# kulaginds/lzma

Measured on AMD Instinct MI355X. Metric: decompressed GiB/s (aggregate batch), higher is better.
Workload: dtype u8

## Files before the change

lzma_amd/build.py:

```python
import os
import subprocess
import sys

HERE = os.path.dirname(os.path.abspath(__file__))
CSRC = os.path.join(HERE, "csrc")
SO = os.path.join(HERE, "libxlz.so")
SOURCES = ["xlz_kernel.hip", "xlz_host.hip", "xlz_xz.hip", "xlz_7z.hip", "xlz_check_dev.hip", "xlz_filter_dev.hip", "xlz_sha256_dev.hip"]
HEADERS = ["xlz_format.h", "xlz_check.h", "xlz_check_dev.h", "xlz_check_host.h", "xlz_filter_dev.h", "xlz_sha256_dev.h", "xlz_fastpath.inc", "xlz_fastpath_pb2.inc", "xlz_fastpath_pb2_br.inc", os.path.join("..", "..", "include", "xlz.h")]
ARCH = "gfx950"


KERNEL_FILES = ["xlz_kernel.hip", "xlz_fastpath.inc", "xlz_fastpath_pb2.inc", "xlz_fastpath_pb2_br.inc", "xlz_format.h"]


def source_id(files=None):
    import hashlib
    h = hashlib.sha256()
    for f in sorted(files or (SOURCES + HEADERS)):
        with open(os.path.join(CSRC, f), "rb") as fh:
            h.update(f.encode() + b"\0" + fh.read())
    return h.hexdigest()[:12]


def _stale():
    if not os.path.exists(SO):
        return True
    t = os.path.getmtime(SO)
    deps = [os.path.join(CSRC, f) for f in SOURCES + HEADERS] + [os.path.abspath(__file__)]
    return any(os.path.getmtime(d) > t for d in deps)


def build(force=False, verbose=False, extra_flags=(), out=None):
    if out is None and os.environ.get("XLZ_SO"):
        print("lzma_amd.build: XLZ_SO is set, not building: %s" % os.environ["XLZ_SO"], file=sys.stderr)
        return os.environ["XLZ_SO"]
    if out is None and not force and not _stale():
        return SO
    hipcc = os.environ.get("HIPCC", "/opt/rocm/bin/hipcc")
    cmd = [hipcc, "--offload-arch=" + ARCH, "-O3", "-std=c++17", "-fPIC", "-shared",
           "-fgpu-rdc" if False else "-fno-gpu-rdc", "-Wall", "-Wno-unused-function",
           "-I", os.path.join(HERE, "..", "include"), '-DXLZ_BUILD_ID="%s"' % source_id(), '-DXLZ_KERNEL_ID="%s"' % source_id(KERNEL_FILES)]
    cmd += list(extra_flags)
    cmd += [os.path.join(CSRC, f) for f in SOURCES]
    cmd += ["-o", out or SO]
    if verbose:
        print(" ".join(cmd), file=sys.stderr)
    subprocess.check_call(cmd)
    return out or SO


if __name__ == "__main__":
    build(force="--force" in sys.argv, verbose=True)
    print(SO)
```

lzma_amd/csrc/xlz_host.hip:

```cpp
#include <hip/hip_runtime.h>

#include <algorithm>
#include <atomic>
#include <chrono>
#include <condition_variable>
#include <cstdio>
#include <deque>
#include <functional>
#include <memory>
#include <thread>
#include <cstdlib>
#include <cstring>
#include <mutex>
#include <new>
#include <numeric>
#include <vector>

#include "../../include/xlz.h"
#include "xlz_format.h"
#include "xlz_check.h"
#include "xlz_check_dev.h"
#include "xlz_check_host.h"
#include "xlz_sha256_dev.h"
#include "xlz_filter_dev.h"

using namespace xlz;

namespace {

constexpr uint32_t kLzmaDicMin = 1u << 12;
constexpr uint64_t kUnknownSize = ~(uint64_t)0;
constexpr uint64_t kMaxUnitBytes = 0xFFFF0000ull;
constexpr size_t kArenaAlign = 256;
constexpr size_t kStoredUnitBytes = 256 * 1024;
constexpr size_t kArenaTailPad = 1024;
constexpr size_t kOutTailPad = 64;
constexpr uint32_t kWideGrid = 32;
constexpr int XLZ_ERR_NO_MEMORY_INTERNAL = -1000;
constexpr uint64_t kSlicedCallBytes = 256ull << 20;
constexpr uint64_t kSliceBytes = 128ull << 20;
constexpr uint64_t kMaxSlices = 8;
constexpr uint32_t kCoreOverWave = 16;
static inline uint32_t head_frac_for(uint32_t slices) { return slices >= 2 ? (uint32_t)(65536ull * 3 / (2 * slices)) : 0; }

inline size_t align_up(size_t v, size_t a) { return (v + a - 1) / a * a; }

#define HIP_TRY(expr)                                                                             \
    do {                                                                                          \
        hipError_t e_ = (expr);                                                                   \
        if (e_ != hipSuccess) {                                                                   \
            if (getenv("XLZ_DEBUG"))                                                              \
                fprintf(stderr, "xlz: %s failed: %s\n", #expr, hipGetErrorString(e_));            \
            return XLZ_ERR_DEVICE;                                                                \
        }                                                                                         \
    } while (0)

}

struct xlz_reader;
struct Batcher;
static void batcher_shutdown(Batcher *bt);

struct MemPool {
    struct Blk {
        void *p;
        size_t cap;
        uint64_t gen;
        bool pinned;
    };
    std::mutex mu;
    std::vector<Blk> idle;
    std::vector<Blk> live;
    uint64_t gen = 1;
    void *take(size_t n, bool pinned)
    {
        if (n == 0) n = 1;
        {
            std::lock_guard<std::mutex> lk(mu);
            size_t best = idle.size();
            for (size_t i = 0; i < idle.size(); i++)
                if (idle[i].pinned == pinned && idle[i].cap >= n && idle[i].cap <= n + n / 2 + (1u << 16) &&
                    (best == idle.size() || idle[i].cap < idle[best].cap))
                    best = i;
            if (best != idle.size()) {
                Blk b = idle[best];
                idle.erase(idle.begin() + (long)best);
                b.gen = gen;
                live.push_back(b);
                return b.p;
            }
        }
        void *p = nullptr;
        const hipError_t e = pinned ? hipHostMalloc(&p, n, hipHostMallocDefault) : hipMalloc(&p, n);
        if (e != hipSuccess) {
            (void)hipGetLastError();
            drop_idle();
            if ((pinned ? hipHostMalloc(&p, n, hipHostMallocDefault) : hipMalloc(&p, n)) != hipSuccess) return nullptr;
        }
        std::lock_guard<std::mutex> lk(mu);
        live.push_back(Blk{p, n, gen, pinned});
        return p;
    }
    void give(void *p)
    {
        if (!p) return;
        std::lock_guard<std::mutex> lk(mu);
        for (size_t i = 0; i < live.size(); i++)
            if (live[i].p == p) {
                idle.push_back(live[i]);
                live.erase(live.begin() + (long)i);
                return;
            }
    }
    void end_of_call()
    {
        std::vector<Blk> out;
        {
            std::lock_guard<std::mutex> lk(mu);
            for (size_t i = 0; i < idle.size();)
                if (idle[i].gen + 1 < gen) {
                    out.push_back(idle[i]);
                    idle.erase(idle.begin() + (long)i);
                } else {
                    i++;
                }
            gen++;
        }
        for (const Blk &b : out) (void)(b.pinned ? hipHostFree(b.p) : hipFree(b.p));
    }
    void drop_idle()
    {
        std::vector<Blk> out;
        {
            std::lock_guard<std::mutex> lk(mu);
            out.swap(idle);
        }
        for (const Blk &b : out) (void)(b.pinned ? hipHostFree(b.p) : hipFree(b.p));
    }
    uint64_t idle_bytes()
    {
        std::lock_guard<std::mutex> lk(mu);
        uint64_t t = 0;
        for (const Blk &b : idle) t += b.cap;
        return t;
    }
};

constexpr int kEventSlots = 64;

struct HostPipe {
    static constexpr int kRing = 8;
    static constexpr size_t kRingBytes = 32u << 20;
    std::mutex mu_in;
    std::condition_variable cv_in;
    bool in_busy = false;
    std::mutex mu_out;
    uint8_t *pin_in = nullptr;
    size_t pin_in_cap = 0;
    uint8_t *ring[kRing] = {};
    hipEvent_t ring_ev[kRing] = {};
    hipStream_t copy_stream = nullptr;
    hipStream_t up_stream = nullptr;
};

struct PinLease {
    HostPipe *hp = nullptr;
    void take(HostPipe &h)
    {
        std::unique_lock<std::mutex> lk(h.mu_in);
        h.cv_in.wait(lk, [&] { return !h.in_busy; });
        h.in_busy = true;
        hp = &h;
    }
    void release()
    {
        if (!hp) return;
        {
            std::lock_guard<std::mutex> lk(hp->mu_in);
            hp->in_busy = false;
        }
        hp->cv_in.notify_one();
        hp = nullptr;
    }
    PinLease() = default;
    PinLease(const PinLease &) = delete;
    PinLease &operator=(const PinLease &) = delete;
    ~PinLease() { release(); }
};

struct xlz_ctx {
    Batcher *batcher = nullptr;
    int device = 0;
    int num_cus = 0;
    hipStream_t stream = nullptr;
    uint32_t *queue = nullptr;
    hipStream_t stream2 = nullptr;
    uint32_t *queue2 = nullptr;
    uint32_t *prio_tab = nullptr;
    hipEvent_t ev[kEventSlots] = {};
    std::mutex mu;
    HostPipe pipe;
    MemPool pool;
    xlz_call_stats last_call = {};
    bool have_last_call = false;
    uint64_t sliced_call_bytes = kSlicedCallBytes, slice_bytes = kSliceBytes;
    uint32_t max_slices = kMaxSlices;
    void *chk_tab[2] = {}, *chk_consts[2] = {};
    hipStream_t check_stream = nullptr;
    int check_mode = 0;
    xlz_check_stats last_check = {};
    xlz_sha256_stats last_sha = {};
    int filter_mode = 0;
    xlz_filter_stats last_filter = {};
};

struct StreamPlan {
    int32_t host_status = 1;
    uint64_t host_in_consumed = 0;
    uint32_t header_len = 0;
    uint32_t first_unit = 0, n_units = 0;
    uint64_t out_off = 0;
    uint64_t out_cap = 0;
    uint64_t in_off = 0;
    uint32_t in_len = 0;
    uint32_t dict_size = 0;
    bool lzma2 = false;
    bool slice = false;
    bool oversize = false;
};

struct xlz_batch {
    xlz_ctx *ctx = nullptr;
    size_t n = 0;
    std::vector<StreamPlan> plans;
    std::vector<Unit> units;
    std::vector<uint32_t> order;
    uint8_t *d_in = nullptr;
    uint8_t *d_out = nullptr;
    Unit *d_units = nullptr;
    uint32_t *d_order = nullptr;
    UnitResult *d_results = nullptr;
    size_t in_bytes = 0, out_bytes = 0;
    uint32_t max_pb = 0;
    bool compact = false;
    uint32_t max_lc_lp = 0;
    uint32_t max_lc_lp_big = 0;
    uint32_t n_normal = 0;
    uint16_t *d_scratch = nullptr;
    uint32_t scratch_stride = 0;
    uint16_t *d_mlit = nullptr;
    uint32_t mlit_stride = 0;
    hipEvent_t ev0 = nullptr, ev1 = nullptr;
    hipStream_t run_stream = nullptr;
    uint32_t *queue = nullptr;
    bool pooled = false;
    bool quiet = false;
    uint32_t call_units = 0;
    bool ran = false;
    uint64_t algo_in = 0;
    std::vector<xlz_result> final_results;
    std::vector<UnitResult> unit_results;
    bool collected = false;
    uint64_t sum_in = 0, sum_out = 0;
    std::vector<size_t> rewritten;
    std::vector<char> wants_wide;
    std::vector<uint32_t> slice_fracs;
    std::vector<hipEvent_t> slice_ev;
    uint8_t *d_states = nullptr;
    size_t state_stride = 0;
    std::vector<std::vector<SlicePiece>> slice_pieces;
    std::vector<uint64_t> slice_pack_bytes;
    SlicePiece *d_pieces = nullptr;
    uint8_t *d_pack = nullptr;
    UnitResult *d_res_snap = nullptr;
    UnitResult *pin_res = nullptr;
    uint32_t head_frac = 0;
    uint8_t *d_stage = nullptr;
    SlicePiece *d_up_pieces = nullptr;
    hipEvent_t ev_heads = nullptr, ev_tails = nullptr;
    std::function<int()> upload_tails;
    PinLease in_lease;
    uint8_t *d_chk = nullptr, *pin_chk = nullptr;
    size_t d_chk_cap = 0, pin_chk_cap = 0;
    hipEvent_t chk_ev0 = nullptr, chk_ev1 = nullptr;
    uint8_t *d_sha = nullptr, *pin_sha = nullptr;
    size_t sha_cap = 0;
    uint8_t *d_flt = nullptr, *pin_flt = nullptr;
    size_t d_flt_cap = 0, pin_flt_cap = 0;
    hipEvent_t flt_ev0 = nullptr, flt_ev1 = nullptr;
};

extern "C" const char *xlz_version(void) { return "xlz 0.1 (gfx950)"; }

#ifndef XLZ_BUILD_ID
#define XLZ_BUILD_ID "unknown"
#endif
extern "C" const char *xlz_build_id(void) { return XLZ_BUILD_ID; }
#ifndef XLZ_KERNEL_ID
#define XLZ_KERNEL_ID "unknown"
#endif
extern "C" const char *xlz_kernel_id(void) { return XLZ_KERNEL_ID; }

extern "C" const char *xlz_strerror(int st)
{
    switch (st) {
    case XLZ_OK: return "ok";
    case XLZ_OK_INPUT_EOF: return "ok (input ended; reference reports io.EOF)";
    case XLZ_ERR_RESULT: return "result error";
    case XLZ_ERR_PROPS: return "incorrect LZMA properties";
    case XLZ_ERR_HEADER_EOF: return "EOF";
    case XLZ_ERR_RC_INIT: return "rangeDec.Init: result error";
    case XLZ_ERR_UNEXPECTED_EOF: return "unexpected EOF";
    case XLZ_ERR_OUT_CAP: return "output capacity too small";
    case XLZ_ERR_BAD_ARG: return "bad argument";
    case XLZ_ERR_DEVICE: return "HIP device error";
    case XLZ_ERR_UNSUPPORTED: return "stream not supported by the GPU path";
    case XLZ_ERR_CLOSED: return "lzma: already closed";
    case XLZ_ERR_NEED_ONE_READER: return "lzma: need exactly one reader";
    case XLZ_ERR_INSUFFICIENT_PROPS: return "lzma2: not enough properties";
    case XLZ_EOF: return "EOF";
    }
    return "unknown status";
}

extern "C" int xlz_device_count(void)
{
    int n = 0;
    if (hipGetDeviceCount(&n) != hipSuccess) return 0;
    return n;
}

extern "C" int xlz_decode_prop(uint8_t d, uint8_t *lc, uint8_t *pb, uint8_t *lp)
{
    if (d >= 9 * 5 * 5) return XLZ_ERR_PROPS;
    if (lc) *lc = d % 9;
    d /= 9;
    if (pb) *pb = d / 5;
    if (lp) *lp = d % 5;
    return XLZ_OK;
}

extern "C" uint32_t xlz_decode_dict_size(const uint8_t p[4])
{
    uint32_t d = 0;
    for (int i = 0; i < 4; i++) d |= (uint32_t)p[i] << (8 * i);
    return d < kLzmaDicMin ? kLzmaDicMin : d;
}

extern "C" uint32_t xlz_decode_dict_size2(uint8_t b)
{
    const unsigned sh = (unsigned)(b / 2 + 11);
    return sh >= 32 ? 0u : (uint32_t)(2u | (b & 1u)) << sh;
}

extern "C" uint64_t xlz_decode_unpack_size(const uint8_t h[8])
{
    uint64_t u = 0;
    for (int i = 0; i < 8; i++) u |= (uint64_t)h[i] << (8 * i);
    return u;
}

namespace {

unsigned host_threads(size_t bytes)
{
    unsigned cap = 8;
    const unsigned hw = std::thread::hardware_concurrency();
    if (hw && hw < cap) cap = hw;
    const unsigned want = (unsigned)(bytes / (32u << 20)) + 1;
    return want < cap ? want : cap;
}

template <class F> void run_threads(unsigned n, F &&f)
{
    if (n <= 1) {
        f(0u);
        return;
    }
    std::vector<std::thread> th;
    th.reserve(n - 1);
    for (unsigned t = 1; t < n; t++) th.emplace_back([&f, t] { f(t); });
    f(0u);
    for (auto &x : th) x.join();
}

}

extern "C" int xlz_ctx_create(int device, xlz_ctx **out)
{
    if (!out) return XLZ_ERR_BAD_ARG;
    *out = nullptr;
    int n = 0;
    if (hipGetDeviceCount(&n) != hipSuccess || device < 0 || device >= n) return XLZ_ERR_DEVICE;
    HIP_TRY(hipSetDevice(device));
    hipDeviceProp_t prop;
    HIP_TRY(hipGetDeviceProperties(&prop, device));
    xlz_ctx *c = new (std::nothrow) xlz_ctx;
    if (!c) return XLZ_ERR_BAD_ARG;
    c->device = device;
    c->num_cus = prop.multiProcessorCount;
    if (hipStreamCreateWithFlags(&c->stream, hipStreamNonBlocking) != hipSuccess ||
        hipStreamCreateWithFlags(&c->stream2, hipStreamNonBlocking) != hipSuccess ||
        hipMalloc(&c->queue, 512) != hipSuccess || hipMalloc(&c->queue2, 512) != hipSuccess ||
        hipMalloc(&c->prio_tab, kPrioTabWords * sizeof(uint32_t)) != hipSuccess ||
        hipMemset(c->prio_tab, 0, kPrioTabWords * sizeof(uint32_t)) != hipSuccess) {
        if (c->queue) (void)hipFree(c->queue);
        if (c->queue2) (void)hipFree(c->queue2);
        if (c->stream) (void)hipStreamDestroy(c->stream);
        if (c->stream2) (void)hipStreamDestroy(c->stream2);
        if (c->prio_tab) (void)hipFree(c->prio_tab);
        delete c;
        return XLZ_ERR_DEVICE;
    }
    *out = c;
    return XLZ_OK;
}

extern "C" void xlz_ctx_destroy(xlz_ctx *c)
{
    if (!c) return;
    if (c->batcher) batcher_shutdown(c->batcher);
    (void)hipSetDevice(c->device);
    c->pool.drop_idle();
    if (c->queue) (void)hipFree(c->queue);
    if (c->queue2) (void)hipFree(c->queue2);
    if (c->prio_tab) (void)hipFree(c->prio_tab);
    for (int k = 0; k < 2; k++) {
        if (c->chk_tab[k]) (void)hipFree(c->chk_tab[k]);
        if (c->chk_consts[k]) (void)hipFree(c->chk_consts[k]);
    }
    if (c->check_stream) (void)hipStreamDestroy(c->check_stream);
    if (c->pipe.pin_in) (void)hipHostFree(c->pipe.pin_in);
    for (int i = 0; i < HostPipe::kRing; i++) {
        if (c->pipe.ring[i]) (void)hipHostFree(c->pipe.ring[i]);
        if (c->pipe.ring_ev[i]) (void)hipEventDestroy(c->pipe.ring_ev[i]);
    }
    if (c->pipe.copy_stream) (void)hipStreamDestroy(c->pipe.copy_stream);
    if (c->pipe.up_stream) (void)hipStreamDestroy(c->pipe.up_stream);
    for (hipEvent_t e : c->ev)
        if (e) (void)hipEventDestroy(e);
    if (c->stream) (void)hipStreamDestroy(c->stream);
    if (c->stream2) (void)hipStreamDestroy(c->stream2);
    delete c;
}

extern "C" int xlz_ctx_device(const xlz_ctx *c) { return c ? c->device : -1; }

extern "C" int xlz_ctx_event_record(xlz_ctx *c, int slot)
{
    if (!c || slot < 0 || slot >= kEventSlots) return XLZ_ERR_BAD_ARG;
    std::lock_guard<std::mutex> lock(c->mu);
    HIP_TRY(hipSetDevice(c->device));
    if (!c->ev[slot]) HIP_TRY(hipEventCreate(&c->ev[slot]));
    HIP_TRY(hipEventRecord(c->ev[slot], c->stream));
    return XLZ_OK;
}

extern "C" int xlz_ctx_event_elapsed_ms(xlz_ctx *c, int a, int b, float *ms)
{
    if (!c || !ms || a < 0 || a >= kEventSlots || b < 0 || b >= kEventSlots || !c->ev[a] || !c->ev[b]) return XLZ_ERR_BAD_ARG;
    HIP_TRY(hipSetDevice(c->device));
    HIP_TRY(hipEventSynchronize(c->ev[b]));
    HIP_TRY(hipEventElapsedTime(ms, c->ev[a], c->ev[b]));
    return XLZ_OK;
}

namespace {

void plan_lzma_alone(const xlz_stream_desc &s, StreamPlan &pl, Unit &u, bool &has_unit)
{
    has_unit = false;
    if (s.in_len == 0) {
        pl.host_status = XLZ_ERR_HEADER_EOF;
        pl.host_in_consumed = 0;
        return;
    }
    uint8_t lc, pb, lp;
    if (xlz_decode_prop(s.in[0], &lc, &pb, &lp) != XLZ_OK) {
        pl.host_status = XLZ_ERR_PROPS;
        pl.host_in_consumed = 1;
        return;
    }
    if (s.in_len < 13) {
        pl.host_status = XLZ_ERR_HEADER_EOF;
        pl.host_in_consumed = s.in_len;
        return;
    }
    u.dict_size = xlz_decode_dict_size(s.in + 1);
    u.unpack_size = xlz_decode_unpack_size(s.in + 5);
    u.lc = lc;
    u.lp = lp;
    u.pb = pb;
    u.kind = UNIT_LZMA1;
    pl.header_len = 13;
    has_unit = true;
}

void plan_lzma_raw(const xlz_stream_desc &s, StreamPlan &pl, Unit &u, bool &has_unit)
{
    has_unit = false;
    uint8_t lc, pb, lp;
    if (xlz_decode_prop(s.props, &lc, &pb, &lp) != XLZ_OK) {
        pl.host_status = XLZ_ERR_PROPS;
        pl.host_in_consumed = 0;
        return;
    }
    u.dict_size = s.dict_size < kLzmaDicMin ? kLzmaDicMin : s.dict_size;
    u.unpack_size = s.unpack_size;
    u.lc = lc;
    u.lp = lp;
    u.pb = pb;
    u.kind = UNIT_LZMA1;
    pl.header_len = 0;
    has_unit = true;
}

struct Lz2Unit {
    uint64_t in_start, in_len;
    uint64_t out_start, expect_out;
    bool have_reader;
};

uint64_t stored_unit_bytes()
{
#ifdef XLZ_DEV_KNOBS
    static const uint64_t v = [] {
        const char *e = getenv("XLZ_STORED_UNIT_KIB");
        if (!e) return (uint64_t)kStoredUnitBytes;
        unsigned long long k = strtoull(e, nullptr, 10);
        return (uint64_t)(k > (1u << 20) ? (1u << 20) : k) << 10;
    }();
    return v;
#else
    return kStoredUnitBytes;
#endif
}

void scan_lzma2(const uint8_t *in, size_t len, std::vector<Lz2Unit> &units, uint32_t &max_lc_lp, uint32_t *max_pb = nullptr)
{
    size_t pos = 0, unit_start = 0;
    uint64_t out = 0, unit_out = 0;
    struct Cand {
        size_t pos;
        uint64_t out;
        bool seen_lzma;
    };
    std::vector<Cand> cands;
    struct Mark {
        size_t pos;
        uint64_t out;
    };
    std::vector<Mark> marks;
    const uint64_t stored_unit = stored_unit_bytes();
    bool seen_lzma = false, unit_seen_lzma = false;
    auto cut = [&](size_t at, uint64_t at_out, bool lzma_before) {
        units.push_back({(uint64_t)unit_start, (uint64_t)(at - unit_start), unit_out, at_out - unit_out, unit_seen_lzma});
        unit_start = at;
        unit_out = at_out;
        unit_seen_lzma = lzma_before;
    };
    auto cut_at_candidates = [&](bool last_pure) {
        size_t mi = 0;
        for (size_t i = 0; i < cands.size(); i++) {
            const Cand &c = cands[i];
            if (c.pos != unit_start) cut(c.pos, c.out, c.seen_lzma);
            const size_t region_end = i + 1 < cands.size() ? cands[i + 1].pos : (size_t)-1;
            const bool pure = i + 1 < cands.size() || last_pure;
            for (; mi < marks.size() && marks[mi].pos < region_end; mi++)
                if (pure && stored_unit && marks[mi].pos > c.pos && marks[mi].out - unit_out >= stored_unit)
                    cut(marks[mi].pos, marks[mi].out, c.seen_lzma);
        }
        cands.clear();
        marks.clear();
    };
    bool ended = false;
    while (pos < len) {
        const uint8_t c = in[pos];
        if (c == 0 || (c >= 3 && c < 0x80)) {
            pos++;
            ended = true;
            break;
        }
        const bool stored = c < 3;
        const unsigned sub = c >> 5;
        const size_t hl = stored ? 3 : (sub >= 6 ? 6 : 5);
        if (pos + hl > len) break;
        uint32_t unc = ((uint32_t)in[pos + 1] << 8) | in[pos + 2];
        if (stored) {
            unc += 1;
            if (c == 1 || pos == 0)
                cands.push_back({pos, out, seen_lzma});
            else if (!cands.empty())
                marks.push_back({pos, out});
            const size_t body = std::min<size_t>(unc, len - pos - hl);
            pos += hl + body;
            out += body;
            continue;
        }
        unc = (unc | ((uint32_t)(c & 0x1F) << 16)) + 1;
        const size_t comp = (((size_t)in[pos + 3] << 8) | in[pos + 4]) + 1;
        if (sub >= 6) {
            const uint8_t props = in[pos + 5];
            if (props >= 225) break;
            max_lc_lp = std::max<uint32_t>(max_lc_lp, (props % 9) + (props / 9) % 5);
            if (max_pb) *max_pb = std::max<uint32_t>(*max_pb, props / 45u);
            if (sub == 7 && pos != 0 && pos != unit_start) {
                cut_at_candidates(true);
                if (pos != unit_start) cut(pos, out, seen_lzma);
            } else {
                cut_at_candidates(sub == 7);
            }
        }
        seen_lzma = true;
        cands.clear();
        marks.clear();
        pos += hl + std::min(comp, len - pos - hl);
        out += unc;
    }
    if (ended || pos >= len) cut_at_candidates(true);
    units.push_back({(uint64_t)unit_start, (uint64_t)(len - unit_start), unit_out, out - unit_out, unit_seen_lzma});
}

}

extern "C" int xlz_lzma2_units(const uint8_t *in, size_t len, xlz_lzma2_unit *units, size_t max_units, size_t *n_units)
{
    if ((!in && len) || !n_units || (!units && max_units)) return XLZ_ERR_BAD_ARG;
    std::vector<Lz2Unit> lu;
    uint32_t mx = 0;
    scan_lzma2(in, len, lu, mx);
    *n_units = lu.size();
    for (size_t k = 0; k < lu.size() && k < max_units; k++) {
        units[k].in_off = lu[k].in_start;
        units[k].in_len = lu[k].in_len;
        units[k].out_off = lu[k].out_start;
        units[k].out_len = lu[k].expect_out;
        units[k].have_reader = lu[k].have_reader ? 1u : 0u;
        units[k].reserved = 0;
    }
    return max_units && lu.size() > max_units ? XLZ_ERR_OUT_CAP : XLZ_OK;
}

extern "C" int xlz_batch_advice(const xlz_ctx *ctx, const xlz_stream_desc *streams, size_t n, uint32_t host_threads,
                                xlz_advice *out)
{
    if (!out || (!streams && n)) return XLZ_ERR_BAD_ARG;
    memset(out, 0, sizeof *out);
    uint64_t max_unit = 0, max_stream = 0;
    for (size_t i = 0; i < n; i++) {
        const xlz_stream_desc &s = streams[i];
        if (!s.in && s.in_len) return XLZ_ERR_BAD_ARG;
        out->in_bytes += s.in_len;
        size_t units = 0;
        if (s.format == XLZ_FMT_LZMA2_RAW) {
            std::vector<Lz2Unit> lu;
            uint32_t mx = 0;
            scan_lzma2(s.in, s.in_len, lu, mx);
            units = lu.size();
            for (const Lz2Unit &u : lu) max_unit = std::max<uint64_t>(max_unit, u.in_len);
        } else if (s.format == XLZ_FMT_LZMA_ALONE) {
            units = s.in_len > 13 ? 1 : 0;
            if (units) max_unit = std::max<uint64_t>(max_unit, s.in_len);
        } else {
            units = s.in_len ? 1 : 0;
            if (units) max_unit = std::max<uint64_t>(max_unit, s.in_len);
        }
        out->units += units;
        if (units) max_stream = std::max<uint64_t>(max_stream, s.in_len);
    }
    const uint32_t cus = ctx ? (uint32_t)ctx->num_cus : 256u;
    out->wave_slots = cus * 16u;
    if (!host_threads) host_threads = std::max(1u, std::thread::hardware_concurrency());
    out->break_even_units = kCoreOverWave * host_threads;
    out->fill = out->wave_slots ? std::min(1.0, (double)out->units / out->wave_slots) : 0.0;
    out->cpu_cost = (double)std::max<uint64_t>(max_stream, (out->in_bytes + host_threads - 1) / host_threads) / kCoreOverWave;
    out->gpu_cost = (double)std::max<uint64_t>(max_unit, out->wave_slots ? (out->in_bytes + out->wave_slots - 1) / out->wave_slots : 0);
    out->prefer_cpu = (out->units == 0 || out->cpu_cost < out->gpu_cost) ? 1 : 0;
    return XLZ_OK;
}

namespace {

template <class T> bool batch_alloc(xlz_batch *b, T **p, size_t bytes, bool pinned = false)
{
    if (b->pooled) {
        *p = static_cast<T *>(b->ctx->pool.take(bytes, pinned));
        return *p != nullptr;
    }
    return (pinned ? hipHostMalloc(reinterpret_cast<void **>(p), bytes, hipHostMallocDefault) : hipMalloc(reinterpret_cast<void **>(p), bytes)) ==
           hipSuccess;
}
void batch_release(xlz_batch *b, void *p, bool pinned = false)
{
    if (!p) return;
    if (b->pooled)
        b->ctx->pool.give(p);
    else
        (void)(pinned ? hipHostFree(p) : hipFree(p));
}

int batch_free(xlz_batch *b)
{
    if (!b) return XLZ_OK;
    if (b->ctx) (void)hipSetDevice(b->ctx->device);
    if (b->pooled && !b->quiet) (void)hipDeviceSynchronize();
    batch_release(b, b->d_in);
    batch_release(b, b->d_out);
    batch_release(b, b->d_units);
    batch_release(b, b->d_order);
    batch_release(b, b->d_results);
    batch_release(b, b->d_scratch);
    batch_release(b, b->d_mlit);
    if (b->ev0) (void)hipEventDestroy(b->ev0);
    if (b->ev1) (void)hipEventDestroy(b->ev1);
    for (hipEvent_t e : b->slice_ev)
        if (e) (void)hipEventDestroy(e);
    batch_release(b, b->d_stage);
    batch_release(b, b->d_up_pieces);
    if (b->ev_heads) (void)hipEventDestroy(b->ev_heads);
    if (b->ev_tails) (void)hipEventDestroy(b->ev_tails);
    b->in_lease.release();
    batch_release(b, b->d_states);
    batch_release(b, b->d_pieces);
    batch_release(b, b->d_pack);
    batch_release(b, b->d_res_snap);
    batch_release(b, b->pin_res, true);
    batch_release(b, b->d_chk);
    batch_release(b, b->pin_chk, true);
    if (b->chk_ev0) (void)hipEventDestroy(b->chk_ev0);
    if (b->chk_ev1) (void)hipEventDestroy(b->chk_ev1);
    batch_release(b, b->d_sha);
    batch_release(b, b->pin_sha, true);
    batch_release(b, b->d_flt);
    batch_release(b, b->pin_flt, true);
    if (b->flt_ev0) (void)hipEventDestroy(b->flt_ev0);
    if (b->flt_ev1) (void)hipEventDestroy(b->flt_ev1);
    delete b;
    return XLZ_OK;
}

int take_pin_in(PinLease &lease, HostPipe &hp, size_t bytes)
{
    lease.take(hp);
    if (hp.pin_in_cap < bytes) {
        if (hp.pin_in) (void)hipHostFree(hp.pin_in);
        hp.pin_in = nullptr;
        hp.pin_in_cap = 0;
        const size_t want = bytes + bytes / 4 + (1u << 20);
        if (hipHostMalloc(&hp.pin_in, want, hipHostMallocDefault) != hipSuccess) return XLZ_ERR_DEVICE;
        hp.pin_in_cap = want;
    }
    if (!hp.up_stream && hipStreamCreateWithFlags(&hp.up_stream, hipStreamNonBlocking) != hipSuccess) return XLZ_ERR_DEVICE;
    return XLZ_OK;
}

struct PackPiece {
    uint64_t off;
    const uint8_t *src;
    size_t len;
};

template <class At> int pack_upload(xlz_ctx *ctx, uint8_t *stage, uint8_t *dst, size_t n, uint64_t total, bool zero_gaps, At &&at)
{
    const hipStream_t up = ctx->pipe.up_stream;
    std::atomic<bool> copy_failed{false};
    auto copy = [&](uint64_t from, uint64_t to) {
        if (to > from && hipMemcpyAsync(dst + from, stage + from, (size_t)(to - from), hipMemcpyHostToDevice, up) != hipSuccess)
            copy_failed = true;
    };
    if (!n && zero_gaps) {
        memset(stage, 0, (size_t)total);
        copy(0, total);
    }
    auto end_of = [&](size_t k) {
        if (!zero_gaps) return at(k).off + at(k).len;
        return k + 1 < n ? at(k + 1).off : total;
    };
    const unsigned nth = host_threads((size_t)total);
    run_threads(nth, [&](unsigned t) {
        (void)hipSetDevice(ctx->device);
        const size_t k0 = n * t / nth, k1 = n * (t + 1) / nth;
        if (k0 >= k1) return;
        uint64_t sent = at(k0).off;
        if (zero_gaps && k0 == 0) {
            memset(stage, 0, (size_t)sent);
            sent = 0;
        }
        for (size_t k = k0; k < k1; k++) {
            const PackPiece pc = at(k);
            memcpy(stage + pc.off, pc.src, pc.len);
            const uint64_t end = end_of(k);
            if (end > pc.off + pc.len) memset(stage + pc.off + pc.len, 0, (size_t)(end - pc.off - pc.len));
            if (end - sent >= (16u << 20)) {
                copy(sent, end);
                sent = end;
            }
        }
        copy(sent, end_of(k1 - 1));
    });
    return copy_failed ? XLZ_ERR_DEVICE : XLZ_OK;
}

LaunchParams batch_params(const xlz_batch *b, bool big)
{
    LaunchParams p;
    memset(&p, 0, sizeof p);
    p.in_arena = b->d_in;
    p.out_arena = b->d_out;
    p.units = b->d_units;
    p.order = b->d_order;
    p.results = b->d_results;
    p.queue = b->queue ? b->queue : b->ctx->queue;
    p.prio_tab = b->ctx->prio_tab;
    p.call_units = b->call_units;
    if (big) {
        p.n_units = (uint32_t)b->units.size() - b->n_normal;
        p.order_base = b->n_normal;
        p.max_lc_lp = b->max_lc_lp_big;
        p.scratch = b->d_scratch;
        p.scratch_stride = b->scratch_stride;
    } else {
        p.n_units = b->n_normal;
        p.max_lc_lp = b->max_lc_lp;
        p.mlit = b->d_mlit;
        p.mlit_stride = b->mlit_stride;
        p.compact = b->compact ? 1u : 0u;
    }
    return p;
}

}

struct BatchOpts {
    uint32_t want_slices = 1;
    uint32_t head_frac = 0;
    uint32_t call_units = 0;
    bool pooled = false;
    hipStream_t run_stream = nullptr;
    uint32_t *queue = nullptr;
};
static int batch_create_ex(xlz_ctx *ctx, const xlz_stream_desc *streams, size_t n, xlz_batch **out, const BatchOpts &opts);

extern "C" int xlz_batch_create(xlz_ctx *ctx, const xlz_stream_desc *streams, size_t n, xlz_batch **out)
{
    return batch_create_ex(ctx, streams, n, out, BatchOpts{});
}

static int batch_create_ex(xlz_ctx *ctx, const xlz_stream_desc *streams, size_t n, xlz_batch **out, const BatchOpts &opts)
{
    const uint32_t want_slices = opts.want_slices, head_frac = opts.head_frac;
    if (!ctx || !out || (!streams && n)) return XLZ_ERR_BAD_ARG;
    *out = nullptr;
    for (size_t i = 0; i < n; i++) {
        if (!streams[i].in && streams[i].in_len) return XLZ_ERR_BAD_ARG;
        if ((streams[i].flags & ~XLZ_STREAM_F_LZMA2_SLICE) ||
            ((streams[i].flags & XLZ_STREAM_F_LZMA2_SLICE) && streams[i].format != XLZ_FMT_LZMA2_RAW))
            return XLZ_ERR_BAD_ARG;
        for (size_t k = 0; k < sizeof streams[i].reserved; k++)
            if (streams[i].reserved[k]) return XLZ_ERR_BAD_ARG;
    }
    HIP_TRY(hipSetDevice(ctx->device));

    xlz_batch *b = new (std::nothrow) xlz_batch;
    if (!b) return XLZ_ERR_BAD_ARG;
    b->ctx = ctx;
    b->n = n;
    b->plans.resize(n);
    b->call_units = opts.call_units;
    b->pooled = opts.pooled;
    b->run_stream = opts.run_stream;
    b->queue = opts.queue;

    auto unit_src_off_p = std::make_shared<std::vector<size_t>>();
    std::vector<size_t> &unit_src_off = *unit_src_off_p;
    size_t in_cursor = 0, out_cursor = 0;
    for (size_t i = 0; i < n; i++) {
        const xlz_stream_desc &s = streams[i];
        StreamPlan &pl = b->plans[i];
        Unit u;
        memset(&u, 0, sizeof u);
        bool has_unit = false;
        switch (s.format) {
        case XLZ_FMT_LZMA_ALONE: plan_lzma_alone(s, pl, u, has_unit); break;
        case XLZ_FMT_LZMA_RAW: plan_lzma_raw(s, pl, u, has_unit); break;
        case XLZ_FMT_LZMA2_RAW:
            u.kind = UNIT_LZMA2;
            u.dict_size = s.dict_size < kLzmaDicMin ? 8u * 1024 * 1024 : s.dict_size;
            u.unpack_size = kUnknownSize;
            pl.header_len = 0;
            pl.slice = (s.flags & XLZ_STREAM_F_LZMA2_SLICE) != 0;
            has_unit = true;
            break;
        default: pl.host_status = XLZ_ERR_BAD_ARG; break;
        }
        if (!has_unit) continue;

        if (u.kind == UNIT_LZMA2) {
            if (s.in_len > kMaxUnitBytes || s.out_cap > kMaxUnitBytes) {
                pl.host_status = XLZ_ERR_UNSUPPORTED;
                pl.oversize = !pl.slice;
                continue;
            }
            std::vector<Lz2Unit> lu;
            uint32_t mx = 0, mpb = 0;
            scan_lzma2(s.in, s.in_len, lu, mx, &mpb);
            const bool big = mx > kMaxLcLpLds;
            if (big)
                b->max_lc_lp_big = std::max(b->max_lc_lp_big, mx);
            else
                b->max_lc_lp = std::max(b->max_lc_lp, mx), b->max_pb = std::max(b->max_pb, mpb);
            pl.lzma2 = true;
            pl.in_off = in_cursor;
            pl.in_len = (uint32_t)s.in_len;
            pl.dict_size = u.dict_size;
            pl.first_unit = (uint32_t)b->units.size();
            pl.n_units = (uint32_t)lu.size();
            pl.out_off = out_cursor;
            pl.out_cap = s.out_cap;
            for (size_t k = 0; k < lu.size(); k++) {
                Unit v = u;
                const bool last = k + 1 == lu.size();
                v.in_off = in_cursor + lu[k].in_start;
                v.in_len = (uint32_t)lu[k].in_len;
                v.out_off = out_cursor + std::min<uint64_t>(lu[k].out_start, s.out_cap);
                const uint64_t room = s.out_cap > lu[k].out_start ? s.out_cap - lu[k].out_start : 0;
                v.out_cap = (uint32_t)(last ? room : std::min<uint64_t>(room, lu[k].expect_out));
                v.expect_out = (uint32_t)lu[k].expect_out;
                v.stream = (uint32_t)i;
                v.flags = (last ? UNIT_F_LAST : 0u) | (lu[k].have_reader ? UNIT_F_HAVE_READER : 0u) |
                          ((k || pl.slice) ? UNIT_F_NOT_FIRST : 0u) | (big ? UNIT_F_BIG_MODEL : 0u);
                v.lc = (uint8_t)mx;
                b->units.push_back(v);
                unit_src_off.push_back(lu[k].in_start);
            }
            b->algo_in += s.in_len;
            in_cursor += align_up(s.in_len + 16, kArenaAlign);
            out_cursor += align_up((size_t)s.out_cap + kOutTailPad, kArenaAlign);
            continue;
        }

        const size_t payload = s.in_len - pl.header_len;
        uint64_t cap = s.out_cap;
        if (u.unpack_size != kUnknownSize && u.unpack_size < cap)
            cap = u.unpack_size;
        const bool size_too_big = u.unpack_size != kUnknownSize && u.unpack_size > kMaxUnitBytes;
        if (payload > kMaxUnitBytes || cap > kMaxUnitBytes || size_too_big) {
            pl.host_status = XLZ_ERR_UNSUPPORTED;
            pl.oversize = true;
            continue;
        }
        const bool big = (uint32_t)u.lc + u.lp > kMaxLcLpLds;
        u.in_off = in_cursor;
        u.in_len = (uint32_t)payload;
        u.out_off = out_cursor;
        u.out_cap = (uint32_t)cap;
        u.stream = (uint32_t)i;
        u.flags = UNIT_F_LAST | (big ? UNIT_F_BIG_MODEL : 0u);
        pl.first_unit = (uint32_t)b->units.size();
        pl.n_units = 1;
        pl.out_off = out_cursor;
        pl.out_cap = cap;
        b->units.push_back(u);
        unit_src_off.push_back(pl.header_len);
        if (big)
            b->max_lc_lp_big = std::max(b->max_lc_lp_big, (uint32_t)u.lc + u.lp);
        else
            b->max_lc_lp = std::max(b->max_lc_lp, (uint32_t)u.lc + u.lp), b->max_pb = std::max<uint32_t>(b->max_pb, u.pb);
        b->algo_in += payload;
        in_cursor += align_up(payload + 16, kArenaAlign);
        out_cursor += align_up((size_t)cap + kOutTailPad, kArenaAlign);
    }
    b->in_bytes = in_cursor + kArenaTailPad;
    b->out_bytes = out_cursor + kArenaTailPad;

    b->order.resize(b->units.size());
    std::iota(b->order.begin(), b->order.end(), 0u);
    std::stable_sort(b->order.begin(), b->order.end(), [&](uint32_t a, uint32_t c) {
        const bool ba = b->units[a].flags & UNIT_F_BIG_MODEL, bc = b->units[c].flags & UNIT_F_BIG_MODEL;
        if (ba != bc) return !ba;
        return b->units[a].in_len > b->units[c].in_len;
    });
    for (uint32_t idx : b->order)
        if (!(b->units[idx].flags & UNIT_F_BIG_MODEL)) b->n_normal++;

    b->compact = b->max_pb <= kCompactPosBits && !getenv("XLZ_NO_COMPACT");

    const size_t nu = b->units.size();
    auto fail = [&](int st) {
        batch_free(b);
        return st;
    };
    if (!batch_alloc(b, &b->d_in, b->in_bytes)) return fail(XLZ_ERR_DEVICE);
    if (!batch_alloc(b, &b->d_out, b->out_bytes)) return fail(XLZ_ERR_DEVICE);
    if (nu) {
        if (!batch_alloc(b, &b->d_units, nu * sizeof(Unit))) return fail(XLZ_ERR_DEVICE);
        if (!batch_alloc(b, &b->d_order, nu * sizeof(uint32_t))) return fail(XLZ_ERR_DEVICE);
        if (!batch_alloc(b, &b->d_results, nu * sizeof(UnitResult))) return fail(XLZ_ERR_DEVICE);
    }
    if (hipEventCreate(&b->ev0) != hipSuccess || hipEventCreate(&b->ev1) != hipSuccess)
        return fail(XLZ_ERR_DEVICE);
    if (b->n_normal < nu) {
        b->scratch_stride = num_probs(b->max_lc_lp_big) + num_matched_probs(b->max_lc_lp_big);
        if (!batch_alloc(b, &b->d_scratch, (size_t)big_model_grid(ctx->num_cus) * b->scratch_stride * sizeof(uint16_t)))
            return fail(XLZ_ERR_DEVICE);
    }
    if (b->n_normal) {
        b->mlit_stride = num_matched_probs(b->max_lc_lp);
        const size_t slots = std::min<size_t>(b->n_normal, decode_grid(b->max_lc_lp, ctx->num_cus, ~0u, b->compact));
        if (!batch_alloc(b, &b->d_mlit, slots * b->mlit_stride * sizeof(uint16_t))) return fail(XLZ_ERR_DEVICE);
    }
    if (want_slices > 1 && b->n_normal && b->n_normal <= decode_grid(b->max_lc_lp, ctx->num_cus, b->call_units ? b->call_units : b->n_normal, b->compact)) {
        const uint32_t K0 = std::min<uint32_t>(want_slices, 63);
        for (uint32_t k = 1; k < K0; k++) b->slice_fracs.push_back((uint32_t)((uint64_t)kSliceOne * k / K0));
        if (K0 >= 4) b->slice_fracs.push_back((uint32_t)((uint64_t)kSliceOne * (2 * K0 - 1) / (2 * K0)));
        b->slice_fracs.push_back(kSliceOne);
        const uint32_t K = (uint32_t)b->slice_fracs.size();
        b->state_stride = align_up(state_bytes(b->max_lc_lp), kArenaAlign);
        if (!batch_alloc(b, &b->d_states, nu * b->state_stride)) return fail(XLZ_ERR_DEVICE);
        for (size_t k = 0; k < nu; k++)
            if (!(b->units[k].flags & UNIT_F_BIG_MODEL)) b->units[k].state = (uint64_t)(uintptr_t)(b->d_states + k * b->state_stride);
        b->slice_pieces.resize(K);
        b->slice_pack_bytes.assign(K, 0);
        size_t total_pieces = 0;
        uint64_t max_pack = 0;
        for (uint32_t k = 0; k < K; k++) {
            uint64_t cursor = 0;
            for (size_t ui = 0; ui < nu; ui++) {
                const Unit &u = b->units[ui];
                if (u.flags & UNIT_F_BIG_MODEL) continue;
                const uint32_t lo = k == 0 ? 0u : std::min(slice_bound(u.out_cap, b->slice_fracs[k - 1]), u.out_cap);
                const uint32_t hi = std::min(slice_bound(u.out_cap, b->slice_fracs[k]), u.out_cap);
                if (hi <= lo) continue;
                const uint64_t po = align_up(cursor, kArenaAlign) + ((u.out_off + lo) & (kArenaAlign - 1));
                b->slice_pieces[k].push_back(SlicePiece{u.out_off + lo, po, hi - lo, (uint32_t)ui});
                cursor = po + (hi - lo);
            }
            b->slice_pack_bytes[k] = cursor;
            max_pack = std::max(max_pack, cursor);
            total_pieces += b->slice_pieces[k].size();
        }
        b->slice_ev.assign(K, nullptr);
        for (uint32_t k = 0; k < K; k++)
            if (hipEventCreateWithFlags(&b->slice_ev[k], hipEventDisableTiming) != hipSuccess) return fail(XLZ_ERR_DEVICE);
        if (!batch_alloc(b, &b->d_pieces, std::max<size_t>(total_pieces, 1) * sizeof(SlicePiece)) ||
            !batch_alloc(b, &b->d_pack, (size_t)max_pack + kArenaAlign) ||
            !batch_alloc(b, &b->d_res_snap, (size_t)K * nu * sizeof(UnitResult)) ||
            !batch_alloc(b, &b->pin_res, (size_t)K * nu * sizeof(UnitResult), true))
            return fail(XLZ_ERR_DEVICE);
        size_t at = 0;
        for (uint32_t k = 0; k < K; k++) {
            const std::vector<SlicePiece> &pv = b->slice_pieces[k];
            if (!pv.empty() &&
                hipMemcpy(b->d_pieces + at, pv.data(), pv.size() * sizeof(SlicePiece), hipMemcpyHostToDevice) != hipSuccess)
                return fail(XLZ_ERR_DEVICE);
            at += pv.size();
        }
    }
    if (!b->slice_fracs.empty() && head_frac && head_frac < kSliceOne) {
        HostPipe &hp = ctx->pipe;
        b->head_frac = head_frac;
        auto heads = std::make_shared<std::vector<SlicePiece>>(), tails = std::make_shared<std::vector<SlicePiece>>();
        uint64_t A = 0, B = 0;
        auto place = [](std::vector<SlicePiece> &v, uint64_t &cur, uint64_t src, uint32_t len, uint32_t ui) {
            if (!len) return;
            const uint64_t po = align_up(cur, kArenaAlign) + (src & (kArenaAlign - 1));
            v.push_back(SlicePiece{src, po, len, ui});
            cur = po + len;
        };
        for (size_t ui = 0; ui < nu; ui++) {
            const Unit &u = b->units[ui];
            const uint32_t h = (u.flags & UNIT_F_BIG_MODEL) ? 0u : slice_head(u.in_len, head_frac, u.kind == UNIT_LZMA2);
            place(*heads, A, u.in_off, h, (uint32_t)ui);
            place(*tails, B, u.in_off + h, u.in_len - h, (uint32_t)ui);
        }
        A = align_up(A, kArenaAlign);
        B = align_up(B, kArenaAlign);
        if (!batch_alloc(b, &b->d_stage, A + B + kArenaAlign) ||
            !batch_alloc(b, &b->d_up_pieces, std::max<size_t>(heads->size() + tails->size(), 1) * sizeof(SlicePiece)) ||
            hipEventCreateWithFlags(&b->ev_heads, hipEventDisableTiming) != hipSuccess ||
            hipEventCreateWithFlags(&b->ev_tails, hipEventDisableTiming) != hipSuccess)
            return fail(XLZ_ERR_DEVICE);
        if ((!heads->empty() && hipMemcpy(b->d_up_pieces, heads->data(), heads->size() * sizeof(SlicePiece), hipMemcpyHostToDevice) != hipSuccess) ||
            (!tails->empty() && hipMemcpy(b->d_up_pieces + heads->size(), tails->data(), tails->size() * sizeof(SlicePiece),
                                          hipMemcpyHostToDevice) != hipSuccess))
            return fail(XLZ_ERR_DEVICE);
        if (take_pin_in(b->in_lease, hp, (size_t)(A + B)) != XLZ_OK) return fail(XLZ_ERR_DEVICE);
        auto upload_part = [b, ctx, streams, unit_src_off_p](const std::vector<SlicePiece> &pv, size_t table_at, uint64_t zone,
                                                             uint64_t zone_bytes, hipEvent_t done) -> int {
            HostPipe &hp = ctx->pipe;
            const int st = pack_upload(ctx, hp.pin_in + zone, b->d_stage + zone, pv.size(), zone_bytes, false, [&](size_t k) {
                const SlicePiece &pc = pv[k];
                const Unit &u = b->units[pc.unit];
                return PackPiece{pc.pack_off, streams[u.stream].in + (*unit_src_off_p)[pc.unit] + (pc.src_off - u.in_off), pc.len};
            });
            if (st != XLZ_OK) return st;
            if (launch_gather(b->d_up_pieces + table_at, (uint32_t)pv.size(), b->d_in, b->d_stage + zone, zone_bytes, ctx->num_cus,
                              hp.up_stream, true) != 0)
                return XLZ_ERR_DEVICE;
            return hipEventRecord(done, hp.up_stream) == hipSuccess ? XLZ_OK : XLZ_ERR_DEVICE;
        };
        if (hipMemsetAsync(b->d_in, 0, b->in_bytes, hp.up_stream) != hipSuccess) return fail(XLZ_ERR_DEVICE);
        const int st_heads = upload_part(*heads, 0, 0, A, b->ev_heads);
        if (st_heads != XLZ_OK) return fail(st_heads);
        const size_t n_heads = heads->size();
        b->upload_tails = [upload_part, tails, n_heads, A, B, b]() { return upload_part(*tails, n_heads, A, B, b->ev_tails); };
    } else {
        HostPipe &hp = ctx->pipe;
        PinLease lease;
        if (take_pin_in(lease, hp, b->in_bytes) != XLZ_OK) return fail(XLZ_ERR_DEVICE);
        const int st = pack_upload(ctx, hp.pin_in, b->d_in, nu, b->in_bytes, true, [&](size_t k) {
            const Unit &u = b->units[k];
            return PackPiece{u.in_off, streams[u.stream].in + unit_src_off[k], u.in_len};
        });
        if (hipStreamSynchronize(hp.up_stream) != hipSuccess || st != XLZ_OK) return fail(XLZ_ERR_DEVICE);
    }
    if (nu) {
        if (hipMemcpy(b->d_units, b->units.data(), nu * sizeof(Unit), hipMemcpyHostToDevice) != hipSuccess ||
            hipMemcpy(b->d_order, b->order.data(), nu * sizeof(uint32_t), hipMemcpyHostToDevice) != hipSuccess)
            return fail(XLZ_ERR_DEVICE);
    }
    *out = b;
    return XLZ_OK;
}


extern "C" int xlz_batch_run(xlz_batch *b)
{
    if (!b) return XLZ_ERR_BAD_ARG;
    xlz_ctx *ctx = b->ctx;
    std::lock_guard<std::mutex> lock(ctx->mu);
    HIP_TRY(hipSetDevice(ctx->device));
    const hipStream_t rs = b->run_stream ? b->run_stream : ctx->stream;
    uint32_t *const rq = b->queue ? b->queue : ctx->queue;
    HIP_TRY(hipMemsetAsync(rq, 0, 256, rs));
    HIP_TRY(hipEventRecord(b->ev0, rs));
    if (b->n_normal) {
        LaunchParams p = batch_params(b, false);
        if (b->slice_fracs.empty()) {
            if (launch_decode(p, ctx->num_cus, rs) != 0) return XLZ_ERR_DEVICE;
        } else {
            for (size_t k = 0; k < b->slice_fracs.size(); k++) {
                if (k) HIP_TRY(hipMemsetAsync(rq, 0, 256, rs));
                if (k == 0 && b->upload_tails) HIP_TRY(hipStreamWaitEvent(rs, b->ev_heads, 0));
                if (k == 1 && b->upload_tails) {
                    const int st = b->upload_tails();
                    b->upload_tails = nullptr;
                    if (st != XLZ_OK) return st;
                    HIP_TRY(hipStreamWaitEvent(rs, b->ev_tails, 0));
                }
                p.slice_frac = b->slice_fracs[k];
                p.slice_k = (uint32_t)k;
                p.head_frac = k == 0 ? b->head_frac : 0;
                if (launch_decode(p, ctx->num_cus, rs) != 0) return XLZ_ERR_DEVICE;
                HIP_TRY(hipMemcpyAsync(b->d_res_snap + k * b->units.size(), b->d_results, b->units.size() * sizeof(UnitResult),
                                       hipMemcpyDeviceToDevice, rs));
                HIP_TRY(hipEventRecord(b->slice_ev[k], rs));
            }
            if (b->head_frac) {
                HIP_TRY(hipEventSynchronize(b->ev_tails));
                b->in_lease.release();
                b->head_frac = 0;
            }
        }
    }
    if (b->units.size() > b->n_normal) {
        HIP_TRY(hipMemsetAsync(rq, 0, 256, rs));
        if (launch_decode(batch_params(b, true), ctx->num_cus, rs) != 0) return XLZ_ERR_DEVICE;
    }
    HIP_TRY(hipEventRecord(b->ev1, rs));
    b->ran = true;
    b->collected = false;
    return XLZ_OK;
}

extern "C" int xlz_batch_sync(xlz_batch *b)
{
    if (!b) return XLZ_ERR_BAD_ARG;
    HIP_TRY(hipSetDevice(b->ctx->device));
    HIP_TRY(hipStreamSynchronize(b->run_stream ? b->run_stream : b->ctx->stream));
    return XLZ_OK;
}

extern "C" int xlz_batch_last_kernel_ms(xlz_batch *b, float *ms)
{
    if (!b || !ms || !b->ran) return XLZ_ERR_BAD_ARG;
    HIP_TRY(hipSetDevice(b->ctx->device));
    HIP_TRY(hipEventSynchronize(b->ev1));
    HIP_TRY(hipEventElapsedTime(ms, b->ev0, b->ev1));
    return XLZ_OK;
}

namespace {

int run_units(xlz_batch *b, const std::vector<Unit> &units, std::vector<UnitResult> &res, bool big, uint32_t wide_lc_lp = 0)
{
    xlz_ctx *ctx = b->ctx;
    const size_t n = units.size();
    res.resize(n);
    if (!n) return XLZ_OK;
    Unit *d_units = nullptr;
    uint32_t *d_order = nullptr;
    UnitResult *d_res = nullptr;
    Epoch *d_epochs = nullptr;
    std::vector<uint32_t> order(n);
    std::iota(order.begin(), order.end(), 0u);
    uint32_t grid = std::min<uint32_t>((uint32_t)n, big ? big_model_grid(ctx->num_cus)
                                                        : decode_grid(b->max_lc_lp, ctx->num_cus, (uint32_t)n, b->compact));
    if (wide_lc_lp) grid = std::min(grid, kWideGrid);
    int st = XLZ_ERR_DEVICE;
    uint16_t *d_wide = nullptr;
    const uint32_t wide_stride = wide_lc_lp ? num_probs(wide_lc_lp) + num_matched_probs(wide_lc_lp) : 0;
    if (wide_lc_lp && hipMalloc(&d_wide, (size_t)grid * wide_stride * sizeof(uint16_t)) != hipSuccess) {
        (void)hipGetLastError();
        return XLZ_ERR_NO_MEMORY_INTERNAL;
    }
    if (hipMalloc(&d_units, n * sizeof(Unit)) == hipSuccess && hipMalloc(&d_order, n * sizeof(uint32_t)) == hipSuccess &&
        hipMalloc(&d_res, n * sizeof(UnitResult)) == hipSuccess &&
        hipMalloc(&d_epochs, (size_t)grid * kMaxEpochs * sizeof(Epoch)) == hipSuccess &&
        hipMemcpy(d_units, units.data(), n * sizeof(Unit), hipMemcpyHostToDevice) == hipSuccess &&
        hipMemcpy(d_order, order.data(), n * sizeof(uint32_t), hipMemcpyHostToDevice) == hipSuccess &&
        hipMemsetAsync(ctx->queue, 0, 256, ctx->stream) == hipSuccess) {
        LaunchParams p = batch_params(b, big);
        p.units = d_units;
        p.order = d_order;
        p.results = d_res;
        p.queue = ctx->queue;
        p.n_units = (uint32_t)n;
        p.order_base = 0;
        p.call_units = 0;
        p.epochs = d_epochs;
        if (wide_lc_lp) {
            p.max_lc_lp = wide_lc_lp;
            p.scratch = d_wide;
            p.scratch_stride = wide_stride;
        }
        if (launch_decode(p, ctx->num_cus, ctx->stream, wide_lc_lp ? grid : 0) == 0 && hipStreamSynchronize(ctx->stream) == hipSuccess &&
            hipMemcpy(res.data(), d_res, n * sizeof(UnitResult), hipMemcpyDeviceToHost) == hipSuccess)
            st = XLZ_OK;
    }
    if (d_units) (void)hipFree(d_units);
    if (d_order) (void)hipFree(d_order);
    if (d_res) (void)hipFree(d_res);
    if (d_epochs) (void)hipFree(d_epochs);
    if (d_wide) (void)hipFree(d_wide);
    return st;
}

void fold_streams(xlz_batch *b, std::vector<size_t> &redo)
{
    const std::vector<UnitResult> &ur = b->unit_results;
    for (size_t i = 0; i < b->n; i++) {
        const StreamPlan &pl = b->plans[i];
        xlz_result &r = b->final_results[i];
        if (pl.host_status != 1) {
            r.status = pl.host_status;
            r.in_consumed = pl.host_in_consumed;
            continue;
        }
        if (!pl.lzma2) {
            const UnitResult &u = ur[pl.first_unit];
            r.status = u.status;
            r.out_len = u.out_len;
            r.in_consumed = (uint64_t)pl.header_len + u.in_consumed;
            continue;
        }
        uint64_t out = 0, in_base = 0;
        bool settled = false;
        auto again = [&] {
            if (pl.slice) {
                r.status = XLZ_ERR_UNSUPPORTED;
                r.out_len = 0;
                r.in_consumed = 0;
            } else {
                redo.push_back(i);
            }
        };
        for (uint32_t k = 0; k < pl.n_units && !settled; k++)
            if (ur[pl.first_unit + k].aux & AUX_STALE) {
                again();
                settled = true;
            }
        for (uint32_t k = 0; k < pl.n_units && !settled; k++) {
            const Unit &un = b->units[pl.first_unit + k];
            const UnitResult &u = ur[pl.first_unit + k];
            const bool last = k + 1 == pl.n_units;
            if (u.status == ST_ERR_UNSUPPORTED && (u.aux & AUX_GROW)) b->wants_wide[i] = 1;
            if (last) {
                r.status = u.status;
                r.out_len = out + u.out_len;
                r.in_consumed = in_base + u.in_consumed;
                settled = true;
            } else if (u.status == ST_OK && !(u.aux & AUX_END_MARK) && u.out_len == un.expect_out && u.in_consumed == un.in_len) {
                out += u.out_len;
                in_base += u.in_consumed;
            } else if (u.status < 0 && u.status != ST_ERR_OUT_CAP) {
                r.status = u.status;
                r.out_len = out + u.out_len;
                r.in_consumed = in_base + u.in_consumed;
                settled = true;
            } else {
                again();
                settled = true;
            }
        }
    }
}

Unit whole_stream_unit(const xlz_batch *b, size_t i, uint32_t lc_lp, bool big)
{
    const StreamPlan &pl = b->plans[i];
    Unit u;
    memset(&u, 0, sizeof u);
    u.kind = UNIT_LZMA2;
    u.in_off = pl.in_off;
    u.in_len = pl.in_len;
    u.out_off = pl.out_off;
    u.out_cap = (uint32_t)pl.out_cap;
    u.dict_size = pl.dict_size;
    u.unpack_size = kUnknownSize;
    u.stream = (uint32_t)i;
    u.lc = (uint8_t)lc_lp;
    u.flags = UNIT_F_LAST | (big ? UNIT_F_BIG_MODEL : 0u);
    return u;
}

int rerun_streams(xlz_batch *b, const std::vector<size_t> &idx, bool big, uint32_t wide_lc_lp = 0)
{
    std::vector<Unit> units;
    for (size_t i : idx) units.push_back(whole_stream_unit(b, i, wide_lc_lp ? wide_lc_lp : b->units[b->plans[i].first_unit].lc, big));
    std::vector<UnitResult> res;
    const int st = run_units(b, units, res, big, wide_lc_lp);
    if (st != XLZ_OK) return st;
    for (size_t k = 0; k < idx.size(); k++) {
        xlz_result &r = b->final_results[idx[k]];
        r.status = res[k].status;
        r.out_len = res[k].out_len;
        r.in_consumed = res[k].in_consumed;
        b->rewritten.push_back(idx[k]);
        b->wants_wide[idx[k]] = (res[k].status == ST_ERR_UNSUPPORTED && (res[k].aux & AUX_GROW)) ? 1 : 0;
    }
    return XLZ_OK;
}

int collect(xlz_batch *b)
{
    if (b->collected) return XLZ_OK;
    xlz_ctx *ctx = b->ctx;
    std::lock_guard<std::mutex> lock(ctx->mu);
    HIP_TRY(hipSetDevice(ctx->device));
    HIP_TRY(hipEventSynchronize(b->ev1));
    std::vector<UnitResult> &ur = b->unit_results;
    ur.resize(b->units.size());
    if (!ur.empty())
        HIP_TRY(hipMemcpy(ur.data(), b->d_results, ur.size() * sizeof(UnitResult), hipMemcpyDeviceToHost));
    b->final_results.assign(b->n, xlz_result{});
    b->rewritten.clear();
    b->wants_wide.assign(b->n, 0);
    std::vector<size_t> redo;
    fold_streams(b, redo);
    for (int pass = 0; pass < 2 && !redo.empty(); pass++) {
        const bool big = pass == 1;
        std::vector<size_t> idx;
        for (size_t i : redo)
            if (((b->units[b->plans[i].first_unit].flags & UNIT_F_BIG_MODEL) != 0) == big) idx.push_back(i);
        const int st = rerun_streams(b, idx, big);
        if (st != XLZ_OK) return st;
    }
    std::vector<size_t> wide;
    for (size_t i = 0; i < b->n; i++) {
        const StreamPlan &pl = b->plans[i];
        if (pl.host_status == 1 && pl.lzma2 && !pl.slice && b->final_results[i].status == XLZ_ERR_UNSUPPORTED && b->wants_wide[i])
            wide.push_back(i);
    }
    const int st = rerun_streams(b, wide, true, kMaxLcLp);
    if (st != XLZ_OK && st != XLZ_ERR_NO_MEMORY_INTERNAL) return st;
    std::sort(b->rewritten.begin(), b->rewritten.end());
    b->rewritten.erase(std::unique(b->rewritten.begin(), b->rewritten.end()), b->rewritten.end());
    b->sum_in = b->sum_out = 0;
    for (size_t i = 0; i < b->n; i++) {
        const StreamPlan &pl = b->plans[i];
        if (pl.host_status != 1) continue;
        b->sum_out += b->final_results[i].out_len;
        b->sum_in += b->final_results[i].in_consumed - pl.header_len;
    }
    b->collected = true;
    return XLZ_OK;
}

}

extern "C" int xlz_batch_results(xlz_batch *b, xlz_result *results)
{
    if (!b || (!results && b->n) || !b->ran) return XLZ_ERR_BAD_ARG;
    int st = collect(b);
    if (st != XLZ_OK) return st;
    for (size_t i = 0; i < b->n; i++) results[i] = b->final_results[i];
    return XLZ_OK;
}

extern "C" int xlz_batch_stats(xlz_batch *b, uint64_t *in_bytes, uint64_t *out_bytes, uint64_t *units)
{
    if (!b || !b->ran) return XLZ_ERR_BAD_ARG;
    int st = collect(b);
    if (st != XLZ_OK) return st;
    if (in_bytes) *in_bytes = b->sum_in;
    if (out_bytes) *out_bytes = b->sum_out;
    if (units) *units = b->units.size();
    return XLZ_OK;
}

extern "C" int xlz_batch_unit_trace(xlz_batch *b, uint32_t *t_start, uint32_t *t_end, uint32_t *in_len, size_t cap,
                                    size_t *n_units)
{
    if (!b || !b->ran || !n_units) return XLZ_ERR_BAD_ARG;
    int st = collect(b);
    if (st != XLZ_OK) return st;
    *n_units = b->unit_results.size();
    uint32_t t0 = 0;
    bool first = true;
    for (const UnitResult &u : b->unit_results)
        if (first || (int32_t)(u.t_start - t0) < 0) {
            t0 = u.t_start;
            first = false;
        }
    for (size_t k = 0; k < b->unit_results.size() && k < cap; k++) {
        if (t_start) t_start[k] = b->unit_results[k].t_start - t0;
        if (t_end) t_end[k] = b->unit_results[k].t_end - t0;
        if (in_len) in_len[k] = b->units[k].in_len;
    }
    return XLZ_OK;
}

extern "C" int xlz_batch_launch_info(xlz_batch *b, uint32_t *workgroups, uint32_t *lds_bytes)
{
    if (!b) return XLZ_ERR_BAD_ARG;
    const uint32_t grid = std::min<uint32_t>(b->n_normal, decode_grid(b->max_lc_lp, b->ctx->num_cus, b->call_units ? b->call_units : b->n_normal, b->compact));
    if (workgroups) *workgroups = grid;
    if (lds_bytes) *lds_bytes = decode_lds_bytes(b->max_lc_lp, b->compact);
    return XLZ_OK;
}

extern "C" const char *xlz_batch_kernel_name(xlz_batch *b)
{
    if (!b) return "";
    if (!b->n_normal) return "xlz::xlz_decode_kernel_hbm_model";
    if (decode_branchy(b->max_lc_lp, b->ctx->num_cus, b->call_units ? b->call_units : b->n_normal, b->compact)) return "xlz::xlz_decode_kernel_pb2_br";
    return b->compact ? "xlz::xlz_decode_kernel_pb2" : "xlz::xlz_decode_kernel";
}

extern "C" int xlz_batch_device_output(xlz_batch *b, size_t i, void **dptr, size_t *cap)
{
    if (!b || i >= b->n || !dptr) return XLZ_ERR_BAD_ARG;
    const StreamPlan &pl = b->plans[i];
    *dptr = pl.host_status == 1 ? b->d_out + pl.out_off : nullptr;
    if (cap) *cap = pl.host_status == 1 ? (size_t)pl.out_cap : 0;
    return XLZ_OK;
}

extern "C" int xlz_batch_download(xlz_batch *b, size_t i, uint8_t *dst, size_t len)
{
    if (!b || i >= b->n || (!dst && len)) return XLZ_ERR_BAD_ARG;
    const StreamPlan &pl = b->plans[i];
    if (pl.host_status != 1 || len == 0) return XLZ_OK;
    if (len > pl.out_cap) len = (size_t)pl.out_cap;
    HIP_TRY(hipSetDevice(b->ctx->device));
    HIP_TRY(hipStreamSynchronize(b->run_stream ? b->run_stream : b->ctx->stream));
    HIP_TRY(hipMemcpy(dst, b->d_out + pl.out_off, len, hipMemcpyDeviceToHost));
    return XLZ_OK;
}

extern "C" void xlz_batch_destroy(xlz_batch *b) { batch_free(b); }

namespace xlz {
int check_launch(int width, const uint8_t *arena, const xlzchk::DevRange *ranges, uint32_t n_ranges, uint32_t total_segs,
                 const void *tab, const void *consts, uint64_t *seg_vals, uint64_t *digests, int num_cus, hipStream_t stream);
int sha256_launch(const uint8_t *arena, uint64_t arena_bytes, const xlzsha::DevRange *ranges, uint32_t n_ranges, uint32_t *digests,
                  hipStream_t stream);
}

namespace {

struct CheckHost {
    xlzchk::Consts<32> c32;
    xlzchk::Consts<64> c64;
    CheckHost()
    {
        xlzchk::build_consts<32>(c32);
        xlzchk::build_consts<64>(c64);
    }
};
const CheckHost &check_host()
{
    static const CheckHost h;
    return h;
}

int check_tables(xlz_ctx *ctx)
{
    if (ctx->chk_tab[0]) return XLZ_OK;
    const CheckHost &h = check_host();
    std::vector<uint32_t> t32(xlzchk::kTabEntries);
    std::vector<uint64_t> t64(xlzchk::kTabEntries);
    xlzchk::build_tables<32>(h.c32, t32.data());
    xlzchk::build_tables<64>(h.c64, t64.data());
    void *p[4] = {};
    const void *src[4] = {t32.data(), t64.data(), &h.c32, &h.c64};
    const size_t bytes[4] = {t32.size() * 4, t64.size() * 8, sizeof h.c32, sizeof h.c64};
    bool ok = true;
    for (int k = 0; k < 4 && ok; k++)
        ok = hipMalloc(&p[k], bytes[k]) == hipSuccess && hipMemcpy(p[k], src[k], bytes[k], hipMemcpyHostToDevice) == hipSuccess;
    if (!ok) {
        (void)hipGetLastError();
        for (void *q : p)
            if (q) (void)hipFree(q);
        return XLZ_ERR_DEVICE;
    }
    ctx->chk_tab[0] = p[0], ctx->chk_tab[1] = p[1], ctx->chk_consts[0] = p[2], ctx->chk_consts[1] = p[3];
    return XLZ_OK;
}

int check_args(const xlz_check_range *ranges, size_t n_ranges, size_t n_streams, const void *digests, bool sha_too = false)
{
    if ((!ranges || !digests) && n_ranges) return XLZ_ERR_BAD_ARG;
    for (size_t q = 0; q < n_ranges; q++)
        if (ranges[q].stream >= n_streams ||
            (ranges[q].kind != XLZ_CHECK_CRC32 && ranges[q].kind != XLZ_CHECK_CRC64 && !(sha_too && ranges[q].kind == XLZ_CHECK_SHA256)) ||
            ranges[q].reserved)
            return XLZ_ERR_BAD_ARG;
    return XLZ_OK;
}

uint64_t host_digest(uint32_t kind, const uint8_t *p, uint64_t n)
{
    return kind == XLZ_CHECK_CRC32 ? (uint64_t)xlzcheck::crc32(p, (size_t)n) : xlzcheck::crc64(p, (size_t)n);
}

int batch_checks_run(xlz_batch *b, const xlz_check_range *ranges, const size_t *idx, size_t n_idx, size_t stream_base, uint64_t *digests,
                     hipStream_t stream, const xlz_stream_desc *streams, xlz_check_stats &acc)
{
    using xlzchk::DevRange;
    if (!n_idx) return XLZ_OK;
    std::vector<DevRange> dev[2];
    std::vector<size_t> where[2];
    uint64_t segs[2] = {0, 0}, dev_bytes = 0;
    for (size_t q = 0; q < n_idx; q++) {
        const size_t ri = idx ? idx[q] : q;
        const xlz_check_range &r = ranges[ri];
        const size_t s = (size_t)(r.stream - stream_base);
        const StreamPlan &pl = b->plans[s];
        if (pl.oversize || r.kind == XLZ_CHECK_SHA256) continue;
        const bool in_arena = pl.host_status == 1;
        const uint64_t produced = in_arena ? std::min<uint64_t>(b->final_results[s].out_len, pl.out_cap) : b->final_results[s].out_len;
        const uint64_t lo = std::min(r.off, produced), hi = r.len > produced - lo ? produced : lo + r.len;
        digests[ri] = 0;
        if (hi == lo) {
            acc.empty_ranges++;
        } else if (!in_arena) {
            if (streams && streams[s].out && hi <= streams[s].out_cap) {
                digests[ri] = host_digest(r.kind, streams[s].out + lo, hi - lo);
                acc.host_ranges++, acc.host_bytes += hi - lo;
            } else {
                acc.empty_ranges++;
            }
        } else {
            const int k = r.kind == XLZ_CHECK_CRC64;
            DevRange d;
            d.off = pl.out_off + lo, d.len = hi - lo;
            const uint64_t ns = xlzchk::range_segments(d.off, d.len);
            if (d.off + d.len > b->out_bytes || segs[k] + ns > 0xFFFFFFFFull) return XLZ_ERR_UNSUPPORTED;
            d.seg_first = (uint32_t)segs[k], d.n_segs = (uint32_t)ns, d.out_index = (uint32_t)where[0].size() + (uint32_t)where[1].size(), d.reserved = 0;
            segs[k] += ns;
            dev[k].push_back(d);
            where[k].push_back(ri);
            dev_bytes += d.len;
        }
    }
    const size_t n_dev = dev[0].size() + dev[1].size();
    if (!n_dev) return XLZ_OK;
    if (n_dev > 0xFFFFFFFFull) return XLZ_ERR_UNSUPPORTED;
    xlz_ctx *ctx = b->ctx;
    std::lock_guard<std::mutex> lock(ctx->mu);
    HIP_TRY(hipSetDevice(ctx->device));
    int st = check_tables(ctx);
    if (st != XLZ_OK) return st;
    const size_t tab_bytes = n_dev * sizeof(DevRange), seg_bytes = (size_t)(segs[0] + segs[1]) * 8, dig_bytes = n_dev * 8;
    if (b->d_chk_cap < tab_bytes + seg_bytes + dig_bytes) {
        batch_release(b, b->d_chk);
        b->d_chk = nullptr, b->d_chk_cap = 0;
        const size_t want = tab_bytes + seg_bytes + dig_bytes;
        if (!batch_alloc(b, &b->d_chk, want)) return XLZ_ERR_DEVICE;
        b->d_chk_cap = want;
    }
    if (b->pin_chk_cap < tab_bytes + dig_bytes) {
        batch_release(b, b->pin_chk, true);
        b->pin_chk = nullptr, b->pin_chk_cap = 0;
        if (!batch_alloc(b, &b->pin_chk, tab_bytes + dig_bytes, true)) return XLZ_ERR_DEVICE;
        b->pin_chk_cap = tab_bytes + dig_bytes;
    }
    if (!b->chk_ev0) HIP_TRY(hipEventCreate(&b->chk_ev0));
    if (!b->chk_ev1) HIP_TRY(hipEventCreate(&b->chk_ev1));
    DevRange *h_tab = reinterpret_cast<DevRange *>(b->pin_chk);
    uint64_t *h_dig = reinterpret_cast<uint64_t *>(b->pin_chk + tab_bytes);
    if (!dev[0].empty()) memcpy(h_tab, dev[0].data(), dev[0].size() * sizeof(DevRange));
    if (!dev[1].empty()) memcpy(h_tab + dev[0].size(), dev[1].data(), dev[1].size() * sizeof(DevRange));
    DevRange *d_tab = reinterpret_cast<DevRange *>(b->d_chk);
    uint64_t *d_seg = reinterpret_cast<uint64_t *>(b->d_chk + tab_bytes);
    uint64_t *d_dig = reinterpret_cast<uint64_t *>(b->d_chk + tab_bytes + seg_bytes);
    HIP_TRY(hipMemcpyAsync(d_tab, h_tab, tab_bytes, hipMemcpyHostToDevice, stream));
    HIP_TRY(hipEventRecord(b->chk_ev0, stream));
    if (xlz::check_launch(32, b->d_out, d_tab, (uint32_t)dev[0].size(), (uint32_t)segs[0], ctx->chk_tab[0], ctx->chk_consts[0], d_seg, d_dig,
                          ctx->num_cus, stream) != 0 ||
        xlz::check_launch(64, b->d_out, d_tab + dev[0].size(), (uint32_t)dev[1].size(), (uint32_t)segs[1], ctx->chk_tab[1], ctx->chk_consts[1],
                          d_seg + segs[0], d_dig, ctx->num_cus, stream) != 0) {
        if (getenv("XLZ_DEBUG")) fprintf(stderr, "xlz: launching the check kernels failed\n");
        (void)hipStreamSynchronize(stream);
        return XLZ_ERR_DEVICE;
    }
    HIP_TRY(hipEventRecord(b->chk_ev1, stream));
    HIP_TRY(hipMemcpyAsync(h_dig, d_dig, dig_bytes, hipMemcpyDeviceToHost, stream));
    HIP_TRY(hipStreamSynchronize(stream));
    float ms = 0;
    HIP_TRY(hipEventElapsedTime(&ms, b->chk_ev0, b->chk_ev1));
    for (int k = 0; k < 2; k++)
        for (size_t j = 0; j < dev[k].size(); j++) digests[where[k][j]] = h_dig[dev[k][j].out_index];
    acc.device_ranges += n_dev, acc.device_bytes += dev_bytes, acc.kernel_ms += ms, acc.launches++;
    return XLZ_OK;
}

void sha256_plan(const uint64_t *lens, size_t n, uint32_t host_threads, double lane_rate, double host_rate, uint8_t *on_device,
                 uint64_t *thr_out)
{
    if (!host_threads) host_threads = xlzsha::kHostThreads;
    if (!(lane_rate > 0)) lane_rate = xlzsha::kLaneBytesPerS;
    if (!(host_rate > 0)) host_rate = xlzsha::kHostBytesPerSPerThread;
    std::vector<uint64_t> s(lens, lens + n);
    std::sort(s.begin(), s.end());
    double total = 0;
    for (uint64_t v : s) total += (double)v;
    double best = total / ((double)host_threads * host_rate), dev_bytes = 0;
    uint64_t thr = 0;
    for (size_t k = 1; k <= n; k++) {
        if (s[k - 1] > xlzsha::kMaxDeviceLen) break;
        dev_bytes += (double)s[k - 1];
        if (k < n && s[k] == s[k - 1]) continue;
        const double rounds = (double)((k + xlzsha::kRoundLanes - 1) / xlzsha::kRoundLanes);
        const double dev_t = (double)s[k - 1] / lane_rate * rounds, host_t = (total - dev_bytes) / ((double)host_threads * host_rate);
        const double t = std::max(dev_t, host_t);
        if (t < best) best = t, thr = s[k - 1];
    }
    for (size_t i = 0; i < n; i++) on_device[i] = thr && lens[i] <= thr;
    if (thr_out) *thr_out = thr;
}

struct ShaHostJob {
    const uint8_t *p;
    uint64_t n;
    xlz_digest *out;
};
void sha256_host_jobs(const std::vector<ShaHostJob> &jobs)
{
    if (jobs.empty()) return;
    const unsigned hw = std::thread::hardware_concurrency();
    const unsigned nth = (unsigned)std::min<size_t>(std::max(1u, std::min(hw ? hw : 1u, xlzsha::kHostThreads)), jobs.size());
    std::atomic<size_t> next{0};
    auto work = [&] {
        for (size_t i; (i = next.fetch_add(1)) < jobs.size();) xlzcheck::sha256(jobs[i].p, (size_t)jobs[i].n, jobs[i].out->b);
    };
    std::vector<std::thread> th;
    try {
        for (unsigned t = 1; t < nth; t++) th.emplace_back(work);
    } catch (...) {
    }
    work();
    for (auto &x : th) x.join();
}
void sha256_of_nothing(xlz_digest *out) { xlzcheck::sha256(out->b, 0, out->b); }
void sha_stats_add(xlz_sha256_stats &t, const xlz_sha256_stats &a)
{
    t.device_ranges += a.device_ranges, t.device_bytes += a.device_bytes, t.host_ranges += a.host_ranges, t.host_bytes += a.host_bytes;
    t.empty_ranges += a.empty_ranges, t.kernel_ms += a.kernel_ms, t.launches += a.launches;
    t.threshold = std::max(t.threshold, a.threshold);
}
void check_stats_add_sha(xlz_check_stats &t, const xlz_sha256_stats &a)
{
    t.device_ranges += a.device_ranges, t.device_bytes += a.device_bytes, t.host_ranges += a.host_ranges, t.host_bytes += a.host_bytes;
    t.empty_ranges += a.empty_ranges, t.kernel_ms += a.kernel_ms, t.launches += a.launches;
}

int batch_sha256_run(xlz_batch *b, const xlz_check_range *ranges, const size_t *idx, size_t n_idx, size_t stream_base, xlz_digest *out,
                     hipStream_t stream, const xlz_stream_desc *streams, std::vector<ShaHostJob> *later, xlz_sha256_stats &acc,
                     bool all_on_device = false)
{
    using xlzsha::DevRange;
    struct InArena {
        size_t ri;
        uint64_t off, len;
    };
    std::vector<InArena> cand;
    for (size_t q = 0; q < n_idx; q++) {
        const size_t ri = idx ? idx[q] : q;
        const xlz_check_range &r = ranges[ri];
        if (r.kind != XLZ_CHECK_SHA256) continue;
        const size_t s = (size_t)(r.stream - stream_base);
        const StreamPlan &pl = b->plans[s];
        if (pl.oversize) continue;
        const bool in_arena = pl.host_status == 1;
        const uint64_t produced = in_arena ? std::min<uint64_t>(b->final_results[s].out_len, pl.out_cap) : b->final_results[s].out_len;
        const uint64_t lo = std::min(r.off, produced), hi = r.len > produced - lo ? produced : lo + r.len;
        if (hi == lo) {
            sha256_of_nothing(&out[ri]);
            acc.empty_ranges++;
        } else if (!in_arena) {
            if (later && streams && streams[s].out && hi <= streams[s].out_cap) {
                later->push_back(ShaHostJob{streams[s].out + lo, hi - lo, &out[ri]});
                acc.host_ranges++, acc.host_bytes += hi - lo;
            } else {
                sha256_of_nothing(&out[ri]);
                acc.empty_ranges++;
            }
        } else {
            if (pl.out_off + hi > b->out_bytes) return XLZ_ERR_UNSUPPORTED;
            cand.push_back(InArena{ri, pl.out_off + lo, hi - lo});
        }
    }
    if (cand.empty()) return XLZ_OK;
    std::vector<uint64_t> lens(cand.size());
    std::vector<uint8_t> on_dev(cand.size());
    for (size_t i = 0; i < cand.size(); i++) lens[i] = cand[i].len;
    uint64_t thr = 0;
    if (all_on_device)
        std::fill(on_dev.begin(), on_dev.end(), (uint8_t)1);
    else
        sha256_plan(lens.data(), lens.size(), 0, 0, 0, on_dev.data(), &thr);
    acc.threshold = std::max(acc.threshold, thr);
    std::vector<InArena> dev, host;
    for (size_t i = 0; i < cand.size(); i++) (on_dev[i] ? dev : host).push_back(cand[i]);
    std::stable_sort(dev.begin(), dev.end(), [](const InArena &x, const InArena &y) { return x.len > y.len; });
    if (dev.size() > 0xFFFFFFFFull) return XLZ_ERR_UNSUPPORTED;
    xlz_ctx *ctx = b->ctx;
    std::vector<std::vector<uint8_t>> fetched;
    {
        std::lock_guard<std::mutex> lock(ctx->mu);
        HIP_TRY(hipSetDevice(ctx->device));
        if (!dev.empty()) {
            const size_t dig_bytes = dev.size() * 32, tab_bytes = dev.size() * sizeof(DevRange);
            if (b->sha_cap < dig_bytes + tab_bytes) {
                batch_release(b, b->d_sha);
                batch_release(b, b->pin_sha, true);
                b->d_sha = b->pin_sha = nullptr, b->sha_cap = 0;
                if (!batch_alloc(b, &b->d_sha, dig_bytes + tab_bytes) || !batch_alloc(b, &b->pin_sha, dig_bytes + tab_bytes, true))
                    return XLZ_ERR_DEVICE;
                b->sha_cap = dig_bytes + tab_bytes;
            }
            if (!b->chk_ev0) HIP_TRY(hipEventCreate(&b->chk_ev0));
            if (!b->chk_ev1) HIP_TRY(hipEventCreate(&b->chk_ev1));
            DevRange *h_tab = reinterpret_cast<DevRange *>(b->pin_sha + dig_bytes);
            for (size_t i = 0; i < dev.size(); i++)
                h_tab[i].off = dev[i].off, h_tab[i].len = dev[i].len, h_tab[i].out_index = (uint32_t)i, h_tab[i].reserved = 0;
            DevRange *d_tab = reinterpret_cast<DevRange *>(b->d_sha + dig_bytes);
            uint32_t *d_dig = reinterpret_cast<uint32_t *>(b->d_sha);
            HIP_TRY(hipMemcpyAsync(d_tab, h_tab, tab_bytes, hipMemcpyHostToDevice, stream));
            HIP_TRY(hipEventRecord(b->chk_ev0, stream));
            uint32_t launches = 0;
            for (size_t at = 0; at < dev.size(); at += xlzsha::kRoundLanes, launches++) {
                const uint32_t m = (uint32_t)std::min<size_t>(xlzsha::kRoundLanes, dev.size() - at);
                if (xlz::sha256_launch(b->d_out, b->out_bytes, d_tab + at, m, d_dig, stream) != 0) {
                    if (getenv("XLZ_DEBUG")) fprintf(stderr, "xlz: launching the SHA-256 kernel failed\n");
                    (void)hipStreamSynchronize(stream);
                    return XLZ_ERR_DEVICE;
                }
            }
            HIP_TRY(hipEventRecord(b->chk_ev1, stream));
            HIP_TRY(hipMemcpyAsync(b->pin_sha, d_dig, dig_bytes, hipMemcpyDeviceToHost, stream));
            HIP_TRY(hipStreamSynchronize(stream));
            float ms = 0;
            HIP_TRY(hipEventElapsedTime(&ms, b->chk_ev0, b->chk_ev1));
            for (size_t i = 0; i < dev.size(); i++) {
                memcpy(out[dev[i].ri].b, b->pin_sha + 32 * i, 32);
                acc.device_bytes += dev[i].len;
            }
            acc.device_ranges += dev.size(), acc.kernel_ms += ms, acc.launches += launches;
        }
        if (!later && !host.empty()) {
            fetched.resize(host.size());
            for (size_t i = 0; i < host.size(); i++) {
                fetched[i].resize((size_t)host[i].len);
                HIP_TRY(hipMemcpyAsync(fetched[i].data(), b->d_out + host[i].off, (size_t)host[i].len, hipMemcpyDeviceToHost, stream));
            }
            HIP_TRY(hipStreamSynchronize(stream));
        }
    }
    std::vector<ShaHostJob> now;
    for (size_t i = 0; i < host.size(); i++) {
        const size_t s = (size_t)(ranges[host[i].ri].stream - stream_base);
        if (later && !(streams && streams[s].out)) {
            sha256_of_nothing(&out[host[i].ri]);
            acc.empty_ranges++;
            continue;
        }
        acc.host_ranges++, acc.host_bytes += host[i].len;
        if (later)
            later->push_back(ShaHostJob{streams[s].out + (host[i].off - b->plans[s].out_off), host[i].len, &out[host[i].ri]});
        else
            now.push_back(ShaHostJob{fetched[i].data(), host[i].len, &out[host[i].ri]});
    }
    sha256_host_jobs(now);
    return XLZ_OK;
}

void crc_digest(uint64_t v, xlz_digest *out)
{
    memset(out->b, 0, sizeof out->b);
    for (int k = 0; k < 8; k++) out->b[k] = (uint8_t)(v >> (8 * k));
}

}

extern "C" int xlz_sha256_plan(const uint64_t *lens, size_t n, uint32_t host_threads, double lane_bytes_per_s,
                               double host_bytes_per_s_per_thread, uint8_t *on_device)
{
    if ((!lens || !on_device) && n) return XLZ_ERR_BAD_ARG;
    if (n) sha256_plan(lens, n, host_threads, lane_bytes_per_s, host_bytes_per_s_per_thread, on_device, nullptr);
    return XLZ_OK;
}

extern "C" int xlz_batch_digests(xlz_batch *b, const xlz_check_range *ranges, size_t n, xlz_digest *out)
{
    if (!b || !b->ran) return XLZ_ERR_BAD_ARG;
    int st = check_args(ranges, n, b->n, out, true);
    if (st != XLZ_OK) return st;
    st = collect(b);
    if (st != XLZ_OK) return st;
    xlz_check_stats acc;
    xlz_sha256_stats sha;
    memset(&acc, 0, sizeof acc);
    memset(&sha, 0, sizeof sha);
    hipStream_t stream = b->run_stream ? b->run_stream : b->ctx->stream;
    std::vector<uint64_t> crc(n);
    st = batch_checks_run(b, ranges, nullptr, n, 0, crc.data(), stream, nullptr, acc);
    if (st == XLZ_OK) st = batch_sha256_run(b, ranges, nullptr, n, 0, out, stream, nullptr, nullptr, sha);
    if (st != XLZ_OK) return st;
    for (size_t q = 0; q < n; q++)
        if (ranges[q].kind != XLZ_CHECK_SHA256) crc_digest(crc[q], &out[q]);
    check_stats_add_sha(acc, sha);
    std::lock_guard<std::mutex> lock(b->ctx->mu);
    b->ctx->last_check = acc;
    b->ctx->last_sha = sha;
    return XLZ_OK;
}

extern "C" int xlz_ctx_last_sha256_stats(xlz_ctx *ctx, xlz_sha256_stats *out)
{
    if (!ctx || !out) return XLZ_ERR_BAD_ARG;
    std::lock_guard<std::mutex> lock(ctx->mu);
    *out = ctx->last_sha;
    return XLZ_OK;
}
extern "C" int xlz_internal_batch_sha256_device(xlz_batch *b, const xlz_check_range *ranges, size_t n, xlz_digest *out, double *kernel_ms)
{
    if (!b || !b->ran || !kernel_ms) return XLZ_ERR_BAD_ARG;
    int st = check_args(ranges, n, b->n, out, true);
    if (st == XLZ_OK) st = collect(b);
    if (st != XLZ_OK) return st;
    xlz_sha256_stats sha;
    memset(&sha, 0, sizeof sha);
    st = batch_sha256_run(b, ranges, nullptr, n, 0, out, b->run_stream ? b->run_stream : b->ctx->stream, nullptr, nullptr, sha, true);
    *kernel_ms = sha.kernel_ms;
    return st;
}
extern "C" double xlz_internal_sha256_host_bench(const uint8_t *p, size_t n, size_t reps, uint32_t threads)
{
    std::vector<xlz_digest> out(reps);
    std::atomic<size_t> next{0};
    auto work = [&] {
        for (size_t i; (i = next.fetch_add(1)) < reps;) xlzcheck::sha256(p, n, out[i].b);
    };
    const auto t0 = std::chrono::steady_clock::now();
    std::vector<std::thread> th;
    for (uint32_t t = 1; t < threads; t++) th.emplace_back(work);
    work();
    for (auto &x : th) x.join();
    return std::chrono::duration<double>(std::chrono::steady_clock::now() - t0).count();
}

void xlz_internal_sha256_stats_reset(xlz_ctx *ctx)
{
    std::lock_guard<std::mutex> lock(ctx->mu);
    memset(&ctx->last_sha, 0, sizeof ctx->last_sha);
}

extern "C" int xlz_batch_checks(xlz_batch *b, const xlz_check_range *ranges, size_t n, uint64_t *digests)
{
    if (!b || !b->ran) return XLZ_ERR_BAD_ARG;
    int st = check_args(ranges, n, b->n, digests);
    if (st != XLZ_OK) return st;
    st = collect(b);
    if (st != XLZ_OK) return st;
    xlz_check_stats acc;
    memset(&acc, 0, sizeof acc);
    st = batch_checks_run(b, ranges, nullptr, n, 0, digests, b->run_stream ? b->run_stream : b->ctx->stream, nullptr, acc);
    if (st != XLZ_OK) return st;
    std::lock_guard<std::mutex> lock(b->ctx->mu);
    b->ctx->last_check = acc;
    return XLZ_OK;
}

extern "C" uint32_t xlz_crc32_combine(uint32_t a, uint32_t b, uint64_t len_b)
{
    return (uint32_t)xlzchk::combine<32>(check_host().c32, a, b, len_b);
}
extern "C" uint64_t xlz_crc64_combine(uint64_t a, uint64_t b, uint64_t len_b) { return xlzchk::combine<64>(check_host().c64, a, b, len_b); }

extern "C" int xlz_ctx_set_check_mode(xlz_ctx *ctx, int mode)
{
    if (!ctx || (mode != 0 && mode != 1 && mode != 2)) return XLZ_ERR_BAD_ARG;
    std::lock_guard<std::mutex> lock(ctx->mu);
    ctx->check_mode = mode;
    return XLZ_OK;
}
extern "C" int xlz_ctx_check_mode(const xlz_ctx *ctx) { return ctx ? ctx->check_mode : XLZ_ERR_BAD_ARG; }

extern "C" int xlz_ctx_last_check_stats(xlz_ctx *ctx, xlz_check_stats *out)
{
    if (!ctx || !out) return XLZ_ERR_BAD_ARG;
    std::lock_guard<std::mutex> lock(ctx->mu);
    *out = ctx->last_check;
    return XLZ_OK;
}

void xlz_internal_check_stats_reset(xlz_ctx *ctx)
{
    std::lock_guard<std::mutex> lock(ctx->mu);
    memset(&ctx->last_check, 0, sizeof ctx->last_check);
}
void xlz_internal_check_stats_host(xlz_ctx *ctx, uint64_t ranges, uint64_t bytes)
{
    std::lock_guard<std::mutex> lock(ctx->mu);
    ctx->last_check.host_ranges += ranges, ctx->last_check.host_bytes += bytes;
}

namespace xlz {
int filter_launch(int cls, uint8_t *arena, const xlzflt::DevStep *steps, uint32_t n_steps, uint32_t total_tiles, void *scratch,
                  void *scratch2, uint32_t total_groups, hipStream_t stream);
}

namespace {

constexpr size_t kMaxStepsPerStream = 3;

int filter_args(const xlz_filter_step *steps, size_t n_steps, size_t n_streams)
{
    if (!steps && n_steps) return XLZ_ERR_BAD_ARG;
    std::vector<uint8_t> count;
    for (size_t q = 0; q < n_steps; q++) {
        const xlz_filter_step &f = steps[q];
        if (f.stream >= n_streams || f.reserved[0] || f.reserved[1] || xlzflt::bad_step(f.id, f.param)) return XLZ_ERR_BAD_ARG;
        if (count.empty()) count.assign(n_streams, 0);
        if (++count[(size_t)f.stream] > kMaxStepsPerStream) return XLZ_ERR_BAD_ARG;
    }
    return XLZ_OK;
}

void filter_stats_add(xlz_filter_stats &t, const xlz_filter_stats &a)
{
    t.device_steps += a.device_steps, t.device_bytes += a.device_bytes, t.host_steps += a.host_steps, t.host_bytes += a.host_bytes;
    t.empty_steps += a.empty_steps, t.kernel_ms += a.kernel_ms, t.launches += a.launches;
}

int batch_filter_run(xlz_batch *b, const xlz_filter_step *steps, const size_t *idx, size_t n_idx, size_t stream_base, hipStream_t stream,
                     xlz_filter_stats &acc)
{
    using xlzflt::DevStep;
    if (!n_idx) return XLZ_OK;
    struct Round {
        std::vector<DevStep> tab[3];
        uint64_t tiles[3] = {0, 0, 0}, windows = 0, rows = 0, groups = 0;
    };
    Round rounds[kMaxStepsPerStream];
    std::vector<uint8_t> depth(b->n, 0);
    uint64_t dev_bytes = 0, dev_steps = 0;
    for (size_t q = 0; q < n_idx; q++) {
        const xlz_filter_step &f = steps[idx ? idx[q] : q];
        const size_t s = (size_t)(f.stream - stream_base);
        const StreamPlan &pl = b->plans[s];
        if (pl.oversize) continue;
        const uint64_t produced = pl.host_status == 1 ? std::min<uint64_t>(b->final_results[s].out_len, pl.out_cap) : 0;
        if (!produced) {
            acc.empty_steps++;
            continue;
        }
        if (depth[s] >= kMaxStepsPerStream || pl.out_off + produced > b->out_bytes || (pl.out_off & 15)) return XLZ_ERR_UNSUPPORTED;
        Round &R = rounds[depth[s]++];
        const int cls = f.id == XLZ_FILTER_X86 ? 1 : f.id == XLZ_FILTER_DELTA ? 2 : 0;
        DevStep d;
        d.off = pl.out_off, d.len = produced, d.id = f.id, d.param = f.param, d.aux = 0, d.aux2 = 0;
        uint64_t tiles;
        if (cls == 0) {
            tiles = (produced + xlzflt::kBcjTileBytes - 1) / xlzflt::kBcjTileBytes;
        } else if (cls == 1) {
            const uint64_t w = xlzflt::x86_windows(produced);
            tiles = (w + xlzflt::kX86TileWindows - 1) / xlzflt::kX86TileWindows;
            d.aux = R.windows, R.windows += w;
        } else {
            tiles = xlzflt::delta_chunks(produced);
            d.aux = R.rows, R.rows += tiles;
            d.aux2 = R.groups, R.groups += xlzflt::delta_groups(tiles);
        }
        if (R.tiles[cls] + tiles > 0x7FFFFFFFull) return XLZ_ERR_UNSUPPORTED;
        d.first = (uint32_t)R.tiles[cls], d.n_tiles = (uint32_t)tiles;
        R.tiles[cls] += tiles;
        R.tab[cls].push_back(d);
        dev_bytes += produced, dev_steps++;
    }
    if (!dev_steps) return XLZ_OK;
    size_t tab_bytes = 0, scratch_bytes = 0;
    for (const Round &R : rounds) {
        for (int c = 0; c < 3; c++) tab_bytes += R.tab[c].size() * sizeof(DevStep);
        scratch_bytes = std::max<size_t>(scratch_bytes, align_up((size_t)R.windows * 2, 256) + (size_t)(R.rows + R.groups) * xlzflt::kDeltaMaxDist);
    }
    xlz_ctx *ctx = b->ctx;
    std::lock_guard<std::mutex> lock(ctx->mu);
    HIP_TRY(hipSetDevice(ctx->device));
    const size_t tab_room = align_up(tab_bytes, 256);
    if (b->d_flt_cap < tab_room + scratch_bytes) {
        batch_release(b, b->d_flt);
        b->d_flt = nullptr, b->d_flt_cap = 0;
        if (!batch_alloc(b, &b->d_flt, tab_room + scratch_bytes)) return XLZ_ERR_DEVICE;
        b->d_flt_cap = tab_room + scratch_bytes;
    }
    if (b->pin_flt_cap < tab_bytes) {
        batch_release(b, b->pin_flt, true);
        b->pin_flt = nullptr, b->pin_flt_cap = 0;
        if (!batch_alloc(b, &b->pin_flt, tab_bytes, true)) return XLZ_ERR_DEVICE;
        b->pin_flt_cap = tab_bytes;
    }
    if (!b->flt_ev0) HIP_TRY(hipEventCreate(&b->flt_ev0));
    if (!b->flt_ev1) HIP_TRY(hipEventCreate(&b->flt_ev1));
    size_t at = 0;
    for (const Round &R : rounds)
        for (int c = 0; c < 3; c++)
            if (!R.tab[c].empty()) {
                memcpy(b->pin_flt + at, R.tab[c].data(), R.tab[c].size() * sizeof(DevStep));
                at += R.tab[c].size() * sizeof(DevStep);
            }
    HIP_TRY(hipMemcpyAsync(b->d_flt, b->pin_flt, tab_bytes, hipMemcpyHostToDevice, stream));
    HIP_TRY(hipEventRecord(b->flt_ev0, stream));
    uint8_t *d_scratch = b->d_flt + tab_room;
    uint32_t launches = 0;
    at = 0;
    for (const Round &R : rounds) {
        uint8_t *d_rows = d_scratch + align_up((size_t)R.windows * 2, 256);
        for (int c = 0; c < 3; c++) {
            if (R.tab[c].empty()) continue;
            const int k = xlz::filter_launch(c, b->d_out, reinterpret_cast<const DevStep *>(b->d_flt + at), (uint32_t)R.tab[c].size(),
                                             (uint32_t)R.tiles[c], c == 2 ? d_rows : d_scratch, d_rows + (size_t)R.rows * xlzflt::kDeltaMaxDist,
                                             (uint32_t)R.groups, stream);
            if (k < 0) {
                if (getenv("XLZ_DEBUG")) fprintf(stderr, "xlz: launching the filter kernels failed\n");
                (void)hipStreamSynchronize(stream);
                return XLZ_ERR_DEVICE;
            }
            launches += (uint32_t)k;
            at += R.tab[c].size() * sizeof(DevStep);
        }
    }
    HIP_TRY(hipEventRecord(b->flt_ev1, stream));
    HIP_TRY(hipStreamSynchronize(stream));
    float ms = 0;
    HIP_TRY(hipEventElapsedTime(&ms, b->flt_ev0, b->flt_ev1));
    acc.device_steps += dev_steps, acc.device_bytes += dev_bytes, acc.kernel_ms += ms, acc.launches += launches;
    return XLZ_OK;
}

}

extern "C" int xlz_filter_host(uint32_t id, uint32_t param, uint8_t *buf, size_t len)
{
    if ((!buf && len) || xlzflt::bad_step(id, param)) return XLZ_ERR_BAD_ARG;
    xlzflt::host_apply(id, param, buf, len);
    return XLZ_OK;
}

extern "C" int xlz_batch_filter(xlz_batch *b, const xlz_filter_step *steps, size_t n)
{
    if (!b || !b->ran) return XLZ_ERR_BAD_ARG;
    int st = filter_args(steps, n, b->n);
    if (st != XLZ_OK) return st;
    st = collect(b);
    if (st != XLZ_OK) return st;
    xlz_filter_stats acc;
    memset(&acc, 0, sizeof acc);
    st = batch_filter_run(b, steps, nullptr, n, 0, b->run_stream ? b->run_stream : b->ctx->stream, acc);
    if (st != XLZ_OK) return st;
    std::lock_guard<std::mutex> lock(b->ctx->mu);
    b->ctx->last_filter = acc;
    return XLZ_OK;
}

extern "C" int xlz_ctx_set_filter_mode(xlz_ctx *ctx, int mode)
{
    if (!ctx || (mode != 0 && mode != 1)) return XLZ_ERR_BAD_ARG;
    std::lock_guard<std::mutex> lock(ctx->mu);
    ctx->filter_mode = mode;
    return XLZ_OK;
}
extern "C" int xlz_ctx_filter_mode(const xlz_ctx *ctx) { return ctx ? ctx->filter_mode : XLZ_ERR_BAD_ARG; }

extern "C" int xlz_ctx_last_filter_stats(xlz_ctx *ctx, xlz_filter_stats *out)
{
    if (!ctx || !out) return XLZ_ERR_BAD_ARG;
    std::lock_guard<std::mutex> lock(ctx->mu);
    *out = ctx->last_filter;
    return XLZ_OK;
}

void xlz_internal_filter_stats_reset(xlz_ctx *ctx)
{
    std::lock_guard<std::mutex> lock(ctx->mu);
    memset(&ctx->last_filter, 0, sizeof ctx->last_filter);
}

namespace {

struct RingChunk {
    const uint8_t *src;
    size_t len;
};
template <class Before, class Src, class Scatter>
int ring_download(xlz_batch *b, size_t n, Before &&before, Src &&src, Scatter &&scatter)
{
    xlz_ctx *ctx = b->ctx;
    HostPipe &hp = ctx->pipe;
    std::lock_guard<std::mutex> out_lock(hp.mu_out);
    HIP_TRY(hipSetDevice(ctx->device));
    if (!hp.copy_stream) HIP_TRY(hipStreamCreateWithFlags(&hp.copy_stream, hipStreamNonBlocking));
    for (int r = 0; r < HostPipe::kRing; r++) {
        if (!hp.ring[r]) HIP_TRY(hipHostMalloc(&hp.ring[r], HostPipe::kRingBytes, hipHostMallocDefault));
        if (!hp.ring_ev[r]) HIP_TRY(hipEventCreateWithFlags(&hp.ring_ev[r], hipEventDisableTiming));
    }
    const unsigned nworkers = std::min<unsigned>(host_threads(b->out_bytes), HostPipe::kRing);
    std::mutex mu;
    std::condition_variable cv;
    size_t issued = 0, next_claim = 0, n_done = 0;
    std::vector<char> done(n, 0);
    bool failed = false;
    auto worker = [&] {
        (void)hipSetDevice(ctx->device);
        for (;;) {
            size_t j;
            {
                std::unique_lock<std::mutex> lk(mu);
                cv.wait(lk, [&] { return next_claim < issued || next_claim >= n || failed; });
                if (failed || next_claim >= n) return;
                j = next_claim++;
            }
            const int slot = (int)(j % HostPipe::kRing);
            const bool ok = hipEventSynchronize(hp.ring_ev[slot]) == hipSuccess;
            if (ok) scatter(j, hp.ring[slot]);
            {
                std::lock_guard<std::mutex> lk(mu);
                done[j] = 1;
                n_done++;
                if (!ok) failed = true;
            }
            cv.notify_all();
        }
    };
    std::vector<std::thread> th;
    for (unsigned t = 0; t < nworkers; t++) th.emplace_back(worker);
    int st = XLZ_OK;
    for (size_t j = 0; j <= n; j++) {
        if (!before(j, hp.copy_stream)) {
            st = XLZ_ERR_DEVICE;
            break;
        }
        if (j == n) break;
        const int slot = (int)(j % HostPipe::kRing);
        if (j >= (size_t)HostPipe::kRing) {
            std::unique_lock<std::mutex> lk(mu);
            cv.wait(lk, [&] { return done[j - HostPipe::kRing] || failed; });
            if (failed) break;
        }
        const RingChunk c = src(j);
        if (hipMemcpyAsync(hp.ring[slot], c.src, c.len, hipMemcpyDeviceToHost, hp.copy_stream) != hipSuccess ||
            hipEventRecord(hp.ring_ev[slot], hp.copy_stream) != hipSuccess) {
            st = XLZ_ERR_DEVICE;
            break;
        }
        {
            std::lock_guard<std::mutex> lk(mu);
            issued = j + 1;
        }
        cv.notify_all();
    }
    {
        std::unique_lock<std::mutex> lk(mu);
        if (st != XLZ_OK) failed = true;
        if (!failed) cv.wait(lk, [&] { return n_done == n || failed; });
        if (failed) st = XLZ_ERR_DEVICE;
        next_claim = std::max(next_claim, n);
    }
    cv.notify_all();
    for (auto &x : th) x.join();
    if (hipStreamSynchronize(hp.copy_stream) != hipSuccess) st = XLZ_ERR_DEVICE;
    return st;
}

int download_all(xlz_batch *b, const xlz_stream_desc *streams, const xlz_result *results, const std::vector<size_t> *only = nullptr)
{
    struct Piece {
        uint64_t dev_off;
        uint8_t *dst;
        size_t len;
    };
    struct Chunk {
        uint64_t dev_off = 0;
        size_t len = 0;
        std::vector<Piece> pieces;
    };
    std::vector<Chunk> chunks;
    const size_t n_take = only ? only->size() : b->n;
    for (size_t t = 0; t < n_take; t++) {
        const size_t i = only ? (*only)[t] : t;
        const StreamPlan &pl = b->plans[i];
        size_t len = (size_t)results[i].out_len;
        if (pl.host_status != 1 || len == 0) continue;
        if (len > pl.out_cap) len = (size_t)pl.out_cap;
        uint64_t off = pl.out_off;
        uint8_t *dst = streams[i].out;
        while (len) {
            if (chunks.empty() || off + 1 > chunks.back().dev_off + HostPipe::kRingBytes || off < chunks.back().dev_off) {
                chunks.emplace_back();
                chunks.back().dev_off = off;
            }
            Chunk &c = chunks.back();
            const size_t room = (size_t)(c.dev_off + HostPipe::kRingBytes - off);
            const size_t take = len < room ? len : room;
            c.pieces.push_back({off, dst, take});
            c.len = (size_t)(off + take - c.dev_off);
            off += take;
            dst += take;
            len -= take;
        }
    }
    if (chunks.empty()) return XLZ_OK;
    return ring_download(
        b, chunks.size(),
        [&](size_t j, hipStream_t) { return j > 0 || hipEventSynchronize(b->ev1) == hipSuccess; },
        [&](size_t j) { return RingChunk{b->d_out + chunks[j].dev_off, chunks[j].len}; },
        [&](size_t j, const uint8_t *ring) {
            for (const Piece &pc : chunks[j].pieces) memcpy(pc.dst, ring + (pc.dev_off - chunks[j].dev_off), pc.len);
        });
}

struct SlotClock {
    bool any = false;
    uint32_t ref = 0;
    int64_t first = 0, last = 0;
    uint64_t busy = 0;
    void add(const UnitResult &u)
    {
        if (!any) ref = u.t_start, first = 0, last = 0, any = true;
        const int64_t a = (int32_t)(u.t_start - ref), e = (int32_t)(u.t_end - ref);
        first = std::min(first, a);
        last = std::max(last, e);
        busy += (uint32_t)(u.t_end - u.t_start);
    }
    double span_ms() const { return any ? (double)(last - first) / 1e5 : 0.0; }
    double occupancy(uint32_t slots) const { return any && slots && last > first ? (double)busy / ((double)slots * (double)(last - first)) : 0.0; }
};

bool dev_late_results()
{
#ifdef XLZ_DEV_KNOBS
    static const bool v = [] {
        const char *e = getenv("XLZ_DEV_LATE_RESULTS");
        return e && strcmp(e, "1") == 0;
    }();
    return v;
#else
    return false;
#endif
}

int download_sliced(xlz_batch *b, const xlz_stream_desc *streams, std::vector<double> *per_slice, std::vector<size_t> &gaps)
{
    xlz_ctx *ctx = b->ctx;
    const size_t K = b->slice_fracs.size(), nu = b->units.size();
    struct Chunk {
        uint32_t k;
        uint64_t off;
        size_t len;
    };
    std::vector<Chunk> chunks;
    for (size_t k = 0; k < K; k++)
        for (uint64_t off = 0; off < b->slice_pack_bytes[k]; off += HostPipe::kRingBytes)
            chunks.push_back({(uint32_t)k, off, (size_t)std::min<uint64_t>(HostPipe::kRingBytes, b->slice_pack_bytes[k] - off)});

    size_t next_k = 0, piece_base = 0;
    const bool late = dev_late_results();
    auto before = [&](size_t j, hipStream_t cs) {
        for (const size_t upto = j < chunks.size() ? chunks[j].k : K - 1; next_k <= upto; next_k++) {
            const size_t k = next_k;
            if (hipStreamWaitEvent(cs, b->slice_ev[k], 0) != hipSuccess ||
                launch_gather(b->d_pieces + piece_base, (uint32_t)b->slice_pieces[k].size(), b->d_out, b->d_pack,
                              b->slice_pack_bytes[k], ctx->num_cus, cs) != 0 ||
                (late && k + 1 < K && hipStreamWaitEvent(cs, b->slice_ev[k + 1], 0) != hipSuccess) ||
                hipMemcpyAsync(b->pin_res + k * nu, b->d_res_snap + k * nu, nu * sizeof(UnitResult), hipMemcpyDeviceToHost, cs) != hipSuccess)
                return false;
            piece_base += b->slice_pieces[k].size();
        }
        return true;
    };
    auto scatter = [&](size_t j, const uint8_t *ring) {
        const Chunk &c = chunks[j];
        const std::vector<SlicePiece> &pv = b->slice_pieces[c.k];
        const UnitResult *res = b->pin_res + (size_t)c.k * nu;
        size_t lo = 0, hi = pv.size();
        while (hi - lo > 1) {
            const size_t mid = (lo + hi) / 2;
            if (pv[mid].pack_off <= c.off)
                lo = mid;
            else
                hi = mid;
        }
        for (size_t i = lo; i < pv.size() && pv[i].pack_off < c.off + c.len; i++) {
            const SlicePiece &pc = pv[i];
            const Unit &u = b->units[pc.unit];
            const uint64_t lo_in_unit = pc.src_off - u.out_off;
            const uint64_t got = res[pc.unit].out_len;
            const uint64_t valid = got > lo_in_unit ? std::min<uint64_t>(got - lo_in_unit, pc.len) : 0;
            const uint64_t a = std::max<uint64_t>(pc.pack_off, c.off), e = std::min<uint64_t>(pc.pack_off + valid, c.off + c.len);
            if (e <= a) continue;
            uint8_t *dst = streams[u.stream].out + (u.out_off - b->plans[u.stream].out_off) + lo_in_unit + (a - pc.pack_off);
            memcpy(dst, ring + (a - c.off), (size_t)(e - a));
        }
    };
    int st = ring_download(
        b, chunks.size(), before, [&](size_t j) { return RingChunk{b->d_pack + chunks[j].off, chunks[j].len}; }, scatter);
    gaps.clear();
    for (size_t ui = 0; ui < nu && st == XLZ_OK && K > 1; ui++) {
        const Unit &u = b->units[ui];
        if (u.flags & UNIT_F_BIG_MODEL) {
            if (gaps.empty() || gaps.back() != u.stream) gaps.push_back(u.stream);
            continue;
        }
        const uint64_t fin = b->pin_res[(K - 1) * nu + ui].out_len;
        for (size_t k = 0; k + 1 < K; k++) {
            const uint64_t hi = std::min(slice_bound(u.out_cap, b->slice_fracs[k]), u.out_cap);
            if (b->pin_res[k * nu + ui].out_len < std::min<uint64_t>(hi, fin)) {
                if (gaps.empty() || gaps.back() != u.stream) gaps.push_back(u.stream);
                break;
            }
        }
    }
    if (st == XLZ_OK && per_slice) {
        uint32_t slots = 0;
        (void)xlz_batch_launch_info(b, &slots, nullptr);
        per_slice->assign(K, 0.0);
        for (size_t k = 0; k < K; k++) {
            const UnitResult *res = b->pin_res + k * nu, *prev = k ? res - nu : nullptr;
            SlotClock launch;
            for (size_t ui = 0; ui < nu; ui++)
                if (!(b->units[ui].flags & UNIT_F_BIG_MODEL) &&
                    !(prev && prev[ui].t_start == res[ui].t_start && prev[ui].t_end == res[ui].t_end))
                    launch.add(res[ui]);
            (*per_slice)[k] = launch.occupancy(slots);
        }
    }
    return st;
}

}

static int decode_oversize(xlz_ctx *ctx, const xlz_stream_desc *streams, xlz_result *results, const std::vector<size_t> &idx);

extern "C" int xlz_ctx_set_slicing(xlz_ctx *ctx, uint64_t min_call_bytes, uint64_t slice_bytes, uint32_t max_slices)
{
    if (!ctx) return XLZ_ERR_BAD_ARG;
    std::lock_guard<std::mutex> lock(ctx->mu);
    ctx->sliced_call_bytes = min_call_bytes ? min_call_bytes : kSlicedCallBytes;
    ctx->slice_bytes = slice_bytes ? slice_bytes : kSliceBytes;
    ctx->max_slices = max_slices ? std::min<uint32_t>(max_slices, 63) : (uint32_t)kMaxSlices;
    return XLZ_OK;
}

extern "C" int xlz_ctx_trim(xlz_ctx *ctx, uint64_t *released)
{
    if (!ctx) return XLZ_ERR_BAD_ARG;
    HIP_TRY(hipSetDevice(ctx->device));
    if (released) *released = ctx->pool.idle_bytes();
    ctx->pool.drop_idle();
    return XLZ_OK;
}

extern "C" int xlz_ctx_last_call_stats(xlz_ctx *ctx, xlz_call_stats *out)
{
    if (!ctx || !out) return XLZ_ERR_BAD_ARG;
    std::lock_guard<std::mutex> lock(ctx->mu);
    if (!ctx->have_last_call) return XLZ_ERR_BAD_ARG;
    *out = ctx->last_call;
    return XLZ_OK;
}

static void plan_sub_batches(const xlz_stream_desc *streams, size_t n, std::vector<size_t> &cuts, bool *rounds)
{
    cuts.assign(1, 0);
    *rounds = false;
    uint64_t total = 0;
    for (size_t i = 0; i < n; i++) total += streams[i].out_cap;
    const size_t k_round = 4096;
    if (n > 6144 && total / n >= (256u << 10)) {
        *rounds = true;
        for (size_t at = k_round; at < n; at += k_round) cuts.push_back(at);
        cuts.push_back(n);
        return;
    }
    const size_t n_sub = std::min<size_t>(std::min<size_t>(8, n / k_round), (size_t)(total >> 29));
    if (n_sub >= 2) {
        const double whole = (double)total / ((double)(n_sub - 1) + 0.5);
        std::vector<double> bounds;
        double acc_b = whole / 4;
        bounds.push_back(acc_b);
        for (size_t k = 0; k + 1 < n_sub; k++) bounds.push_back(acc_b += whole);
        uint64_t acc = 0;
        size_t next = 0;
        for (size_t i = 0; i < n && next < bounds.size(); i++) {
            acc += streams[i].out_cap;
            const bool small = next == 0;
            const size_t least = small ? k_round / 8 : k_round / 2;
            if ((double)acc >= bounds[next] && i + 1 - cuts.back() >= least && n - (i + 1) >= k_round / 8) {
                cuts.push_back(i + 1);
                next++;
            }
        }
    }
    cuts.push_back(n);
}

extern "C" int xlz_decode_batch_plan(const xlz_stream_desc *streams, size_t n, size_t *cuts, size_t max_cuts, size_t *n_cuts, int *mode)
{
    if ((!streams && n) || !n_cuts || (!cuts && max_cuts)) return XLZ_ERR_BAD_ARG;
    std::vector<size_t> c;
    bool rounds = false;
    plan_sub_batches(streams, n, c, &rounds);
    *n_cuts = c.size();
    for (size_t k = 0; k < c.size() && k < max_cuts; k++) cuts[k] = c[k];
    if (mode) *mode = c.size() <= 2 ? 0 : rounds ? 2 : 1;
    return max_cuts && c.size() > max_cuts ? XLZ_ERR_OUT_CAP : XLZ_OK;
}

static int decode_batch_impl(xlz_ctx *ctx, const xlz_stream_desc *streams, size_t n, xlz_result *results, const xlz_filter_step *steps,
                             size_t n_steps, const xlz_check_range *ranges, size_t n_ranges, uint64_t *digests, bool accumulate,
                             xlz_digest *xd = nullptr)
{
    if (!ctx || (!streams && n) || (!results && n)) return XLZ_ERR_BAD_ARG;
    for (size_t i = 0; i < n; i++)
        if (!streams[i].out && streams[i].out_cap) return XLZ_ERR_BAD_ARG;
    if (check_args(ranges, n_ranges, n, xd ? (const void *)xd : (const void *)digests, xd != nullptr) != XLZ_OK) return XLZ_ERR_BAD_ARG;
    std::vector<uint64_t> crc_of(xd ? n_ranges : 0);
    if (xd) digests = crc_of.data();
    bool has_sha = false;
    for (size_t q = 0; q < n_ranges && xd; q++) has_sha |= ranges[q].kind == XLZ_CHECK_SHA256;
    std::vector<ShaHostJob> sha_later;
    xlz_sha256_stats sha;
    memset(&sha, 0, sizeof sha);
    if (filter_args(steps, n_steps, n) != XLZ_OK) return XLZ_ERR_BAD_ARG;
    for (size_t q = 0; q < n_steps; q++)
        if (streams[steps[q].stream].flags & XLZ_STREAM_F_LZMA2_SLICE) return XLZ_ERR_BAD_ARG;
    const char *dbg = getenv("XLZ_DEBUG");
    const auto t0 = std::chrono::steady_clock::now();
    auto now_ms = [&] { return std::chrono::duration<double, std::milli>(std::chrono::steady_clock::now() - t0).count(); };
    std::vector<size_t> cuts;
    bool rounds_mode = false;
    plan_sub_batches(streams, n, cuts, &rounds_mode);
    const size_t S = cuts.size() - 1;
    xlz_call_stats cs;
    memset(&cs, 0, sizeof cs);
    cs.streams = n;
    cs.sub_batches = (uint32_t)S;

    uint64_t sliced_call_bytes, slice_bytes, max_slices;
    {
        std::lock_guard<std::mutex> lock(ctx->mu);
        sliced_call_bytes = ctx->sliced_call_bytes, slice_bytes = ctx->slice_bytes, max_slices = ctx->max_slices;
    }
    std::vector<std::vector<size_t>> sub_steps(n_steps ? S : 0);
    for (size_t q = 0; q < n_steps; q++)
        sub_steps[(size_t)(std::upper_bound(cuts.begin(), cuts.end(), (size_t)steps[q].stream) - cuts.begin()) - 1].push_back(q);
    xlz_filter_stats flt;
    memset(&flt, 0, sizeof flt);
    auto slices_for = [&](size_t k) -> uint32_t {
        if (S > 1 && !rounds_mode) return 1;
        if (n_steps && !sub_steps[k].empty()) return 1;
        uint64_t total = 0;
        for (size_t i = cuts[k]; i < cuts[k + 1]; i++) total += streams[i].out_cap;
        return total >= sliced_call_bytes ? (uint32_t)std::max<uint64_t>(1, std::min<uint64_t>(max_slices, total / slice_bytes)) : 1u;
    };

    std::vector<std::vector<size_t>> sub_ranges(n_ranges ? S : 0);
    xlz_check_stats chk;
    memset(&chk, 0, sizeof chk);
    if (n_ranges || n_steps) {
        for (size_t q = 0; q < n_ranges; q++)
            sub_ranges[(size_t)(std::upper_bound(cuts.begin(), cuts.end(), (size_t)ranges[q].stream) - cuts.begin()) - 1].push_back(q);
        std::lock_guard<std::mutex> lock(ctx->mu);
        if (hipSetDevice(ctx->device) != hipSuccess ||
            (!ctx->check_stream && hipStreamCreateWithFlags(&ctx->check_stream, hipStreamNonBlocking) != hipSuccess))
            return XLZ_ERR_DEVICE;
    }

    std::vector<xlz_batch *> sub(S, nullptr);
    std::mutex mu;
    std::condition_variable cv;
    std::vector<int> created(S, 0), launched(S, 0), decoded(S, 0);
    int st_up = XLZ_OK, st_down = XLZ_OK;
    bool abort_all = false;
    const bool threaded = S > 1;
    double t_first_up = 0, t_decoded = 0, occ_busy = 0, occ_span = 0;
    SlotClock clock;

    auto uploader = [&] {
        for (size_t k = 0; k < S; k++) {
            {
                std::lock_guard<std::mutex> lk(mu);
                if (abort_all) return;
            }
            xlz_batch *b = nullptr;
            BatchOpts o;
            o.want_slices = slices_for(k);
            o.head_frac = k == 0 ? head_frac_for(o.want_slices) : 0;
            o.call_units = (S > 1 && !rounds_mode) ? (uint32_t)std::min<size_t>(n, 0xFFFFFFFFu) : 0u;
            o.pooled = true;
            if (S > 1 && !rounds_mode && k % 2) o.run_stream = ctx->stream2, o.queue = ctx->queue2;
            const int st = batch_create_ex(ctx, streams + cuts[k], cuts[k + 1] - cuts[k], &b, o);
            if (dbg) fprintf(stderr, "xlz_decode_batch: sub-batch %zu uploaded at %.1f ms\n", k, now_ms());
            {
                std::lock_guard<std::mutex> lk(mu);
                sub[k] = b;
                created[k] = st == XLZ_OK ? 1 : -1;
                if (st != XLZ_OK) st_up = st, abort_all = true;
                if (k == 0) t_first_up = now_ms();
            }
            cv.notify_all();
            if (st != XLZ_OK) return;
        }
    };
    int st = XLZ_OK;
    auto collect_one = [&](size_t k) {
        int e = xlz_batch_results(sub[k], results + cuts[k]);
        if (e == XLZ_OK) {
            uint32_t slots = 0;
            (void)xlz_batch_launch_info(sub[k], &slots, nullptr);
            cs.units += sub[k]->unit_results.size();
            cs.wave_slots = std::max(cs.wave_slots, slots);
            if (sub[k]->slice_fracs.empty())
                for (const UnitResult &u : sub[k]->unit_results) clock.add(u);
        }
        if (dbg) fprintf(stderr, "xlz_decode_batch: sub-batch %zu decoded at %.1f ms\n", k, now_ms());
        if (e == XLZ_OK && n_steps && !sub_steps[k].empty()) {
            e = batch_filter_run(sub[k], steps, sub_steps[k].data(), sub_steps[k].size(), cuts[k], ctx->check_stream, flt);
            if (dbg) fprintf(stderr, "xlz_decode_batch: sub-batch %zu filtered at %.1f ms\n", k, now_ms());
        }
        {
            std::lock_guard<std::mutex> lk(mu);
            decoded[k] = e == XLZ_OK ? 1 : -1;
            if (e != XLZ_OK) abort_all = true;
            t_decoded = now_ms();
        }
        cv.notify_all();
        if (e == XLZ_OK && n_ranges && !sub_ranges[k].empty()) {
            e = batch_checks_run(sub[k], ranges, sub_ranges[k].data(), sub_ranges[k].size(), cuts[k], digests, ctx->check_stream,
                                 streams + cuts[k], chk);
            if (e == XLZ_OK && has_sha)
                e = batch_sha256_run(sub[k], ranges, sub_ranges[k].data(), sub_ranges[k].size(), cuts[k], xd, ctx->check_stream,
                                     streams + cuts[k], &sha_later, sha);
            if (dbg) fprintf(stderr, "xlz_decode_batch: sub-batch %zu checked at %.1f ms\n", k, now_ms());
            if (e != XLZ_OK) {
                {
                    std::lock_guard<std::mutex> lk(mu);
                    abort_all = true;
                }
                cv.notify_all();
            }
        }
        return e;
    };
    auto await_decoded = [&](size_t k) {
        if (!threaded) {
            if (decoded[k] == 0) {
                const int e = collect_one(k);
                if (e != XLZ_OK) st_down = e;
            }
            return decoded[k] == 1;
        }
        std::unique_lock<std::mutex> lk(mu);
        cv.wait(lk, [&] { return decoded[k] != 0 || abort_all; });
        return decoded[k] == 1;
    };
    auto downloader = [&] {
        for (size_t k = 0; k < S; k++) {
            int e = XLZ_OK;
            if (threaded) {
                std::unique_lock<std::mutex> lk(mu);
                cv.wait(lk, [&] { return launched[k] != 0 || abort_all; });
                if (launched[k] != 1) return;
            }
            xlz_batch *b = sub[k];
            if (!b->slice_fracs.empty()) {
                std::vector<double> occ;
                std::vector<size_t> again;
                e = download_sliced(b, streams + cuts[k], &occ, again);
                if (dbg)
                    fprintf(stderr, "xlz_decode_batch: sub-batch %zu: %zu slices downloaded at %.1f ms, %zu streams with gaps\n", k,
                            b->slice_fracs.size(), now_ms(), again.size());
                if (e == XLZ_OK && !await_decoded(k)) return;
                if (e == XLZ_OK) {
                    again.insert(again.end(), b->rewritten.begin(), b->rewritten.end());
                    std::sort(again.begin(), again.end());
                    again.erase(std::unique(again.begin(), again.end()), again.end());
                    if (!again.empty()) e = download_all(b, streams + cuts[k], results + cuts[k], &again);
                }
                std::lock_guard<std::mutex> lk(mu);
                if (e == XLZ_OK) cs.refetched += (uint32_t)again.size();
                cs.slices = std::max<uint32_t>(cs.slices, (uint32_t)b->slice_fracs.size());
                for (double o : occ) occ_busy += o * 1.0, occ_span += 1.0;
            } else {
                if (!await_decoded(k)) return;
                e = download_all(b, streams + cuts[k], results + cuts[k]);
            }
            if (dbg) fprintf(stderr, "xlz_decode_batch: sub-batch %zu downloaded at %.1f ms\n", k, now_ms());
            if (e != XLZ_OK) {
                std::lock_guard<std::mutex> lk(mu);
                st_down = e;
                abort_all = true;
                cv.notify_all();
                return;
            }
        }
    };
    std::thread th_up, th_down;
    if (threaded) {
        try {
            th_up = std::thread(uploader);
            th_down = std::thread(downloader);
        } catch (...) {
            {
                std::lock_guard<std::mutex> lk(mu);
                abort_all = true;
            }
            cv.notify_all();
            if (th_up.joinable()) th_up.join();
            for (xlz_batch *b : sub) xlz_batch_destroy(b);
            return XLZ_ERR_DEVICE;
        }
    }
    double sliced_kernel_ms = -1;
    if (!threaded) {
        uploader();
        st = st_up;
        if (st == XLZ_OK) st = xlz_batch_run(sub[0]);
        if (st == XLZ_OK) {
            launched[0] = 1;
            downloader();
            st = st_down;
            float ms = 0;
            if (st == XLZ_OK && !sub[0]->slice_fracs.empty() && xlz_batch_last_kernel_ms(sub[0], &ms) == XLZ_OK) sliced_kernel_ms = ms;
        }
    } else {
        for (size_t k = 0; k < S && st == XLZ_OK; k++) {
            {
                std::unique_lock<std::mutex> lk(mu);
                cv.wait(lk, [&] { return created[k] != 0 || abort_all; });
                if (created[k] != 1) break;
            }
            st = xlz_batch_run(sub[k]);
            {
                std::lock_guard<std::mutex> lk(mu);
                launched[k] = st == XLZ_OK ? 1 : -1;
                if (st != XLZ_OK) abort_all = true;
            }
            cv.notify_all();
            if (st == XLZ_OK && k > 0) st = collect_one(k - 1);
        }
        bool all_launched;
        {
            std::lock_guard<std::mutex> lk(mu);
            all_launched = created[S - 1] == 1 && launched[S - 1] == 1 && !abort_all;
        }
        if (st == XLZ_OK && all_launched) st = collect_one(S - 1);
        {
            std::lock_guard<std::mutex> lk(mu);
            if (st != XLZ_OK) abort_all = true;
        }
        cv.notify_all();
        th_up.join();
        th_down.join();
        if (st == XLZ_OK) st = st_up != XLZ_OK ? st_up : st_down;
    }
    const double t_end = now_ms();
    cs.upload_ms = t_first_up;
    cs.decode_ms = t_decoded - t_first_up;
    cs.download_ms = t_end - t_decoded;
    if (sliced_kernel_ms >= 0) {
        cs.decode_ms = sliced_kernel_ms;
        cs.download_ms = std::max(0.0, t_end - t_first_up - sliced_kernel_ms);
    }
    cs.total_ms = t_end;
    cs.kernel_span_ms = sliced_kernel_ms >= 0 ? sliced_kernel_ms : clock.span_ms();
    cs.slot_occupancy = occ_span > 0 ? occ_busy / occ_span : clock.occupancy(cs.wave_slots);
    {
        std::lock_guard<std::mutex> lock(ctx->mu);
        ctx->last_call = cs;
        ctx->have_last_call = st == XLZ_OK;
    }
    std::vector<size_t> big;
    for (size_t k = 0; k < S && st == XLZ_OK; k++)
        for (size_t i = 0; i < sub[k]->n; i++)
            if (sub[k]->plans[i].oversize) big.push_back(cuts[k] + i);
    for (xlz_batch *b : sub) {
        if (b && st == XLZ_OK) b->quiet = true;
        xlz_batch_destroy(b);
    }
    ctx->pool.end_of_call();
    if (st == XLZ_OK && !big.empty()) st = decode_oversize(ctx, streams, results, big);
    if (st == XLZ_OK && n_steps) {
        for (size_t q = 0; q < n_steps && !big.empty(); q++) {
            const xlz_filter_step &f = steps[q];
            if (!std::binary_search(big.begin(), big.end(), (size_t)f.stream)) continue;
            const uint64_t produced = std::min<uint64_t>(results[f.stream].out_len, streams[f.stream].out_cap);
            if (produced)
                xlzflt::host_apply(f.id, f.param, streams[f.stream].out, produced), flt.host_steps++, flt.host_bytes += produced;
            else
                flt.empty_steps++;
        }
        std::lock_guard<std::mutex> lock(ctx->mu);
        if (accumulate)
            filter_stats_add(ctx->last_filter, flt);
        else
            ctx->last_filter = flt;
    }
    if (st == XLZ_OK && n_ranges) {
        for (size_t q = 0; q < n_ranges && !big.empty(); q++) {
            const xlz_check_range &r = ranges[q];
            if (!std::binary_search(big.begin(), big.end(), (size_t)r.stream)) continue;
            const uint64_t produced = std::min<uint64_t>(results[r.stream].out_len, streams[r.stream].out_cap);
            const uint64_t lo = std::min(r.off, produced), hi = r.len > produced - lo ? produced : lo + r.len;
            if (r.kind == XLZ_CHECK_SHA256) {
                if (hi > lo)
                    sha_later.push_back(ShaHostJob{streams[r.stream].out + lo, hi - lo, &xd[q]}), sha.host_ranges++, sha.host_bytes += hi - lo;
                else
                    sha256_of_nothing(&xd[q]), sha.empty_ranges++;
                continue;
            }
            digests[q] = hi > lo ? host_digest(r.kind, streams[r.stream].out + lo, hi - lo) : 0;
            if (hi > lo)
                chk.host_ranges++, chk.host_bytes += hi - lo;
            else
                chk.empty_ranges++;
        }
        sha256_host_jobs(sha_later);
        for (size_t q = 0; q < n_ranges && xd; q++)
            if (ranges[q].kind != XLZ_CHECK_SHA256) crc_digest(digests[q], &xd[q]);
        check_stats_add_sha(chk, sha);
        std::lock_guard<std::mutex> lock(ctx->mu);
        if (xd && accumulate)
            sha_stats_add(ctx->last_sha, sha);
        else if (xd)
            ctx->last_sha = sha;
        if (accumulate) {
            xlz_check_stats &t = ctx->last_check;
            t.device_ranges += chk.device_ranges, t.device_bytes += chk.device_bytes, t.host_ranges += chk.host_ranges;
            t.host_bytes += chk.host_bytes, t.empty_ranges += chk.empty_ranges, t.kernel_ms += chk.kernel_ms, t.launches += chk.launches;
        } else {
            ctx->last_check = chk;
        }
    }
    return st;
}

extern "C" int xlz_decode_batch(xlz_ctx *ctx, const xlz_stream_desc *streams, size_t n, xlz_result *results)
{
    return decode_batch_impl(ctx, streams, n, results, nullptr, 0, nullptr, 0, nullptr, false);
}

extern "C" int xlz_decode_batch_checked(xlz_ctx *ctx, const xlz_stream_desc *streams, size_t n, xlz_result *results,
                                        const xlz_check_range *ranges, size_t n_ranges, uint64_t *digests)
{
    return decode_batch_impl(ctx, streams, n, results, nullptr, 0, ranges, n_ranges, digests, false);
}

extern "C" int xlz_decode_batch_filtered(xlz_ctx *ctx, const xlz_stream_desc *streams, size_t n, xlz_result *results,
                                         const xlz_filter_step *steps, size_t n_steps, const xlz_check_range *ranges, size_t n_ranges,
                                         uint64_t *digests)
{
    if (!ctx && xlz_device_count() == 0) return XLZ_ERR_DEVICE;
    return decode_batch_impl(ctx, streams, n, results, steps, n_steps, ranges, n_ranges, digests, false);
}

int xlz_internal_decode_batch_filtered(xlz_ctx *ctx, const xlz_stream_desc *streams, size_t n, xlz_result *results,
                                       const xlz_filter_step *steps, size_t n_steps, const xlz_check_range *ranges, size_t n_ranges,
                                       uint64_t *digests, int accumulate)
{
    return decode_batch_impl(ctx, streams, n, results, steps, n_steps, ranges, n_ranges, digests, accumulate != 0);
}

extern "C" int xlz_decode_batch_digests(xlz_ctx *ctx, const xlz_stream_desc *streams, size_t n, xlz_result *results,
                                        const xlz_filter_step *steps, size_t n_steps, const xlz_check_range *ranges, size_t n_ranges,
                                        xlz_digest *out)
{
    if (!ctx) return XLZ_ERR_BAD_ARG;
    return decode_batch_impl(ctx, streams, n, results, steps, n_steps, ranges, n_ranges, nullptr, false, out);
}

int xlz_internal_decode_batch_digests(xlz_ctx *ctx, const xlz_stream_desc *streams, size_t n, xlz_result *results,
                                      const xlz_filter_step *steps, size_t n_steps, const xlz_check_range *ranges, size_t n_ranges,
                                      xlz_digest *out, int accumulate)
{
    return decode_batch_impl(ctx, streams, n, results, steps, n_steps, ranges, n_ranges, nullptr, accumulate != 0, out);
}

int xlz_internal_decode_batch_checked(xlz_ctx *ctx, const xlz_stream_desc *streams, size_t n, xlz_result *results,
                                      const xlz_check_range *ranges, size_t n_ranges, uint64_t *digests, int accumulate)
{
    return decode_batch_impl(ctx, streams, n, results, nullptr, 0, ranges, n_ranges, digests, accumulate != 0);
}

namespace {

struct MultiItem {
    size_t stream;
    uint64_t in_off, in_len;
    uint64_t out_off, out_len;
    bool whole, first, last;
    xlz_result res;
};

constexpr uint64_t kMultiMinSplitBytes = 64u << 10;

void multi_split(const xlz_stream_desc &s, size_t stream, size_t pieces, std::vector<MultiItem> &items)
{
    std::vector<Lz2Unit> lu;
    uint32_t mx = 0;
    if (pieces >= 2 && s.in_len <= kMaxUnitBytes && s.out_cap <= kMaxUnitBytes) scan_lzma2(s.in, s.in_len, lu, mx);
    uint64_t announced = 0;
    for (const Lz2Unit &u : lu) announced += u.expect_out;
    if (lu.size() < 2 || announced > s.out_cap) {
        MultiItem it{stream, 0, s.in_len, 0, s.out_cap, true, true, true, xlz_result{}};
        items.push_back(it);
        return;
    }
    pieces = std::min(pieces, lu.size());
    size_t k = 0;
    for (size_t p = 0; p < pieces; p++) {
        const size_t k0 = k;
        const uint64_t until = (uint64_t)s.in_len * (p + 1) / pieces;
        k++;
        while (k < lu.size() && (p + 1 == pieces || lu[k].in_start + lu[k].in_len <= until) && lu.size() - k > pieces - p - 1) k++;
        if (p + 1 == pieces) k = lu.size();
        MultiItem it;
        it.stream = stream;
        it.in_off = lu[k0].in_start;
        it.in_len = (k == lu.size() ? (uint64_t)s.in_len : lu[k].in_start) - it.in_off;
        it.out_off = lu[k0].out_start;
        it.out_len = (k == lu.size() ? announced : lu[k].out_start) - it.out_off;
        it.whole = false;
        it.first = k0 == 0;
        it.last = k == lu.size();
        it.res = xlz_result{};
        items.push_back(it);
    }
}

}

namespace {

void multi_plan(size_t n_ctx, const xlz_stream_desc *streams, size_t n, std::vector<MultiItem> &items,
                std::vector<std::vector<size_t>> &shard)
{
    uint64_t total_in = 0;
    for (size_t i = 0; i < n; i++) total_in += streams[i].in_len;
    const uint64_t share = std::max<uint64_t>(1, total_in / n_ctx);
    items.clear();
    items.reserve(n + 4 * n_ctx);
    for (size_t i = 0; i < n; i++) {
        const xlz_stream_desc &s = streams[i];
        size_t pieces = 1;
        if (n_ctx > 1 && s.format == XLZ_FMT_LZMA2_RAW && !(s.flags & XLZ_STREAM_F_LZMA2_SLICE) && s.in_len >= kMultiMinSplitBytes &&
            s.in_len > share / 4)
            pieces = (size_t)std::min<uint64_t>(4 * n_ctx, (s.in_len + share / 4 - 1) / std::max<uint64_t>(1, share / 4));
        multi_split(s, i, pieces, items);
    }
    std::vector<size_t> order(items.size());
    std::iota(order.begin(), order.end(), (size_t)0);
    std::stable_sort(order.begin(), order.end(), [&](size_t a, size_t b) { return items[a].in_len > items[b].in_len; });
    shard.assign(n_ctx, {});
    std::vector<uint64_t> load(n_ctx, 0);
    for (size_t i : order) {
        size_t k = 0;
        for (size_t c = 1; c < n_ctx; c++)
            if (load[c] < load[k]) k = c;
        shard[k].push_back(i);
        load[k] += items[i].in_len + 1;
    }
    for (auto &idx : shard) std::sort(idx.begin(), idx.end());
}

}

extern "C" int xlz_decode_batch_multi_plan(size_t n_ctx, const xlz_stream_desc *streams, size_t n, xlz_multi_item *out,
                                           size_t max_items, size_t *n_items)
{
    if (!n_ctx || (!streams && n) || !n_items || (!out && max_items)) return XLZ_ERR_BAD_ARG;
    for (size_t i = 0; i < n; i++)
        if (!streams[i].in && streams[i].in_len) return XLZ_ERR_BAD_ARG;
    std::vector<MultiItem> items;
    std::vector<std::vector<size_t>> shard;
    multi_plan(n_ctx, streams, n, items, shard);
    *n_items = items.size();
    for (size_t c = 0; c < n_ctx; c++)
        for (size_t k : shard[c]) {
            if (k >= max_items) continue;
            const MultiItem &it = items[k];
            out[k].stream = it.stream;
            out[k].context = (uint32_t)c;
            out[k].flags = (it.whole ? 1u : 0u) | (it.first ? 2u : 0u) | (it.last ? 4u : 0u);
            out[k].in_off = it.in_off;
            out[k].in_len = it.in_len;
            out[k].out_off = it.out_off;
            out[k].out_len = it.out_len;
        }
    return max_items && items.size() > max_items ? XLZ_ERR_OUT_CAP : XLZ_OK;
}

extern "C" int xlz_decode_batch_multi(xlz_ctx *const *ctxs, size_t n_ctx, const xlz_stream_desc *streams, size_t n,
                                      xlz_result *results)
{
    if (!ctxs || n_ctx == 0 || (!streams && n) || (!results && n)) return XLZ_ERR_BAD_ARG;
    for (size_t c = 0; c < n_ctx; c++)
        if (!ctxs[c]) return XLZ_ERR_BAD_ARG;
    for (size_t i = 0; i < n; i++)
        if ((!streams[i].in && streams[i].in_len) || (!streams[i].out && streams[i].out_cap)) return XLZ_ERR_BAD_ARG;
    if (n_ctx == 1 || n == 0) return xlz_decode_batch(ctxs[0], streams, n, results);
    std::vector<MultiItem> items;
    std::vector<std::vector<size_t>> shard;
    multi_plan(n_ctx, streams, n, items, shard);
    std::vector<int> st(n_ctx, XLZ_OK);
    auto work = [&](size_t c) {
        std::vector<size_t> &idx = shard[c];
        if (idx.empty()) return;
        std::vector<xlz_stream_desc> d(idx.size());
        std::vector<xlz_result> r(idx.size());
        for (size_t k = 0; k < idx.size(); k++) {
            const MultiItem &it = items[idx[k]];
            d[k] = streams[it.stream];
            if (!it.whole) {
                d[k].in += it.in_off;
                d[k].in_len = (size_t)it.in_len;
                d[k].out += it.out_off;
                d[k].out_cap = it.last ? (size_t)(streams[it.stream].out_cap - it.out_off) : (size_t)it.out_len;
                if (!it.first) d[k].flags |= XLZ_STREAM_F_LZMA2_SLICE;
            }
        }
        st[c] = xlz_decode_batch(ctxs[c], d.data(), d.size(), r.data());
        if (st[c] == XLZ_OK)
            for (size_t k = 0; k < idx.size(); k++) items[idx[k]].res = r[k];
    };
    std::vector<std::thread> th;
    for (size_t c = 1; c < n_ctx; c++) th.emplace_back(work, c);
    work(0);
    for (auto &x : th) x.join();
    for (size_t c = 0; c < n_ctx; c++)
        if (st[c] != XLZ_OK) return st[c];
    std::vector<size_t> again;
    for (size_t k = 0; k < items.size();) {
        const size_t i = items[k].stream;
        if (items[k].whole) {
            results[i] = items[k].res;
            k++;
            continue;
        }
        bool clean = true;
        xlz_result sum{};
        size_t e = k;
        for (; e < items.size() && items[e].stream == i; e++) {
            const MultiItem &it = items[e];
            if (it.last)
                clean = clean && it.res.status == XLZ_OK;
            else
                clean = clean && it.res.status == XLZ_ERR_UNEXPECTED_EOF && it.res.out_len == it.out_len &&
                        it.res.in_consumed == it.in_len;
            sum.out_len += it.res.out_len;
            if (it.last) {
                sum.in_consumed = it.in_off + it.res.in_consumed;
                sum.status = it.res.status;
            }
        }
        if (clean)
            results[i] = sum;
        else
            again.push_back(i);
        k = e;
    }
    if (!again.empty()) {
        std::vector<xlz_stream_desc> d(again.size());
        std::vector<xlz_result> r(again.size());
        for (size_t k = 0; k < again.size(); k++) d[k] = streams[again[k]];
        const int s2 = xlz_decode_batch(ctxs[0], d.data(), d.size(), r.data());
        if (s2 != XLZ_OK) return s2;
        for (size_t k = 0; k < again.size(); k++) results[again[k]] = r[k];
    }
    return XLZ_OK;
}

struct Session {
    uint8_t *d_ctl = nullptr;
    uint8_t *d_win = nullptr;
    uint8_t *d_shadow = nullptr;
    size_t win_cap = 0, win_max = 0;
    size_t off_state = 0, off_in = 0, in_buf = 0;
    Unit unit;
    uint32_t model_lc_lp = 0;
    uint32_t pos = 0;
    uint32_t rebase = 0;
    uint64_t in_skip = 0;
    uint64_t in_loaded = 0;
    uint64_t consumed = 0;
    bool started = false;
    size_t payload_off = 0;
    uint64_t left = kUnknownSize;
};

struct xlz_reader {
    xlz_ctx *ctx = nullptr;
    xlz_stream_desc desc;
    std::vector<uint8_t> in;
    const uint8_t *src = nullptr;
    size_t src_len = 0;
    std::vector<uint8_t> chunk;
    size_t rd = 0;
    bool finished = false;
    bool closed = false;
    bool is_closer = false;
    int32_t status = XLZ_OK;
    int call_status = XLZ_OK;
    int step_status = XLZ_OK;
    uint64_t delivered = 0;
    Session *ss = nullptr;
    bool whole = false;
    bool refill_pending = false;
    uint64_t n_refills = 0, n_whole = 0, n_shadow = 0;
    bool pending_reset = false, pending_reopen = false;
    bool streaming = false, in_eof = false, need_input = false;
    bool input_fresh = true;
    uint64_t in_base = 0;
    std::vector<uint64_t> par_in, par_out;
    size_t par_next = 0;
    bool par = false, par_tried = false;
    uint64_t n_par = 0;
};

struct Batcher {
    xlz_ctx *ctx = nullptr;
    uint32_t window_us = 500, max_streams = 4096;
    std::mutex mu;
    std::condition_variable cv_work, cv_done;
    std::deque<xlz_reader *> pending;
    bool stop = false;
    uint64_t n_batches = 0, n_streams = 0;
    std::thread th;
};

namespace {

constexpr size_t kChunk = 1u << 20;
constexpr size_t kWinSlack = 65536 + 1024;
constexpr size_t kInBuf = 4u << 20;
constexpr size_t kCtlHead = 256;

xlz_reader *reader_new(xlz_ctx *ctx, const uint8_t *in, size_t in_len)
{
    xlz_reader *r = new (std::nothrow) xlz_reader;
    if (!r) return nullptr;
    r->ctx = ctx;
    r->in.assign(in, in + in_len);
    r->src = r->in.data();
    r->src_len = r->in.size();
    memset(&r->desc, 0, sizeof r->desc);
    return r;
}

int check_rc_init(const uint8_t *p, size_t n)
{
    if (n == 0) return XLZ_ERR_HEADER_EOF;
    if (p[0] != 0) return XLZ_ERR_RC_INIT;
    if (n < 5) return XLZ_ERR_HEADER_EOF;
    return XLZ_OK;
}

void session_free(Session *ss)
{
    if (!ss) return;
    if (ss->d_ctl) (void)hipFree(ss->d_ctl);
    if (ss->d_win) (void)hipFree(ss->d_win);
    if (ss->d_shadow) (void)hipFree(ss->d_shadow);
    delete ss;
}

int session_open(xlz_reader *r)
{
    Session *ss = new (std::nothrow) Session;
    if (!ss) return XLZ_ERR_DEVICE;
    Unit &u = ss->unit;
    memset(&u, 0, sizeof u);
    uint64_t known = kUnknownSize;
    if (r->desc.format == XLZ_FMT_LZMA2_RAW) {
        std::vector<Lz2Unit> lu;
        uint32_t mx = 0;
        scan_lzma2(r->src, r->src_len, lu, mx);
        u.kind = UNIT_LZMA2;
        u.dict_size = r->desc.dict_size < kLzmaDicMin ? 8u * 1024 * 1024 : r->desc.dict_size;
        u.unpack_size = kUnknownSize;
        if (r->streaming && mx < 4) mx = 4;
        u.lc = (uint8_t)mx;
        ss->model_lc_lp = mx;
    } else {
        xlz_stream_desc d = r->desc;
        d.in = r->src;
        d.in_len = r->src_len;
        StreamPlan pl;
        bool has = false;
        if (r->desc.format == XLZ_FMT_LZMA_ALONE)
            plan_lzma_alone(d, pl, u, has);
        else
            plan_lzma_raw(d, pl, u, has);
        if (!has) {
            delete ss;
            return XLZ_ERR_BAD_ARG;
        }
        ss->payload_off = pl.header_len;
        ss->model_lc_lp = (uint32_t)u.lc + u.lp;
        known = u.unpack_size;
    }
    if (ss->model_lc_lp > kMaxLcLp) {
        delete ss;
        return XLZ_ERR_UNSUPPORTED;
    }
    u.flags = UNIT_F_LAST;
    ss->win_max = 2 * (size_t)u.dict_size + kChunk + kWinSlack;
    if (known != kUnknownSize && known + kWinSlack < ss->win_max) ss->win_max = (size_t)known + kWinSlack;
    if (ss->win_max > kMaxUnitBytes) ss->win_max = (size_t)kMaxUnitBytes;
    ss->win_cap = std::min<size_t>(ss->win_max, 2 * kChunk + kWinSlack);
    ss->left = known;
    ss->in_buf = r->streaming ? kInBuf : std::min<size_t>(kInBuf, align_up(r->src_len - ss->payload_off + 16, 256) + kArenaTailPad);
    ss->off_state = kCtlHead;
    ss->off_in = align_up(ss->off_state + state_bytes(ss->model_lc_lp), 256);
    if (hipMalloc(&ss->d_ctl, ss->off_in + ss->in_buf) != hipSuccess || hipMalloc(&ss->d_win, ss->win_cap) != hipSuccess) {
        session_free(ss);
        return XLZ_ERR_DEVICE;
    }
    const uint32_t zero = 0;
    if (hipMemcpy(ss->d_ctl + 128, &zero, 4, hipMemcpyHostToDevice) != hipSuccess) {
        session_free(ss);
        return XLZ_ERR_DEVICE;
    }
    if (u.kind == UNIT_LZMA2) {
        const uint64_t none = 0;
        if (hipMemcpy(ss->d_ctl + ss->off_state + (size_t)kStateShadowWord * 4, &none, 8, hipMemcpyHostToDevice) != hipSuccess) {
            session_free(ss);
            return XLZ_ERR_DEVICE;
        }
    }
    r->ss = ss;
    return XLZ_OK;
}

int session_prepare(xlz_reader *r, hipStream_t stream)
{
    Session *ss = r->ss;
    Unit &u = ss->unit;
    const size_t need = ss->left == kUnknownSize ? kChunk : (size_t)std::min<uint64_t>(kChunk, ss->left);
    if ((size_t)ss->pos + need + kWinSlack > ss->win_cap) {
        const size_t keep = std::min<size_t>(ss->pos, u.dict_size);
        if (ss->win_cap < ss->win_max) {
            size_t want = std::min(ss->win_max, std::max(ss->win_cap * 2, (size_t)ss->pos + need + kWinSlack));
            uint8_t *nw = nullptr;
            if (hipMalloc(&nw, want) != hipSuccess) return XLZ_ERR_DEVICE;
            if (hipMemcpyAsync(nw, ss->d_win, ss->pos, hipMemcpyDeviceToDevice, stream) != hipSuccess ||
                hipStreamSynchronize(stream) != hipSuccess) {
                (void)hipFree(nw);
                return XLZ_ERR_DEVICE;
            }
            (void)hipFree(ss->d_win);
            ss->d_win = nw;
            ss->win_cap = want;
        }
        if ((size_t)ss->pos + need + kWinSlack > ss->win_cap) {
            if ((size_t)ss->pos - keep < keep) return XLZ_ERR_UNSUPPORTED;
            if (hipMemcpyAsync(ss->d_win, ss->d_win + (ss->pos - keep), keep, hipMemcpyDeviceToDevice, stream) != hipSuccess)
                return XLZ_ERR_DEVICE;
            ss->rebase += (uint32_t)(ss->pos - keep);
            ss->pos = (uint32_t)keep;
        }
    }
    const uint64_t total = r->in_base + r->src_len - ss->payload_off;
    const bool more_coming = r->streaming && !r->in_eof;
    const uint64_t margin = u.kind == UNIT_LZMA2 ? 70000 : 4096;
    if (!ss->started || (ss->in_loaded < total && ss->in_loaded - ss->consumed < margin)) {
        ss->in_skip = ss->consumed & ~(uint64_t)255;
        const uint64_t end = std::min<uint64_t>(total, ss->in_skip + ss->in_buf - kArenaTailPad);
        if (hipMemcpyAsync(ss->d_ctl + ss->off_in, r->src + (ss->payload_off + ss->in_skip - r->in_base), (size_t)(end - ss->in_skip),
                           hipMemcpyHostToDevice, stream) != hipSuccess ||
            hipMemsetAsync(ss->d_ctl + ss->off_in + (end - ss->in_skip), 0, kArenaTailPad, stream) != hipSuccess ||
            hipStreamSynchronize(stream) != hipSuccess)
            return XLZ_ERR_DEVICE;
        ss->in_loaded = end;
    }
    u.in_off = (uint64_t)(ss->d_ctl + ss->off_in);
    u.in_len = (uint32_t)(ss->in_loaded - ss->in_skip);
    u.in_skip = (uint32_t)ss->in_skip;
    u.out_off = (uint64_t)ss->d_win;
    u.out_cap = (uint32_t)(ss->win_cap - kOutTailPad);
    u.pause_at = ss->pos + (uint32_t)kChunk;
    u.rebase = ss->rebase;
    u.state = (uint64_t)(ss->d_ctl + ss->off_state);
    u.flags = UNIT_F_LAST | (ss->started ? UNIT_F_RESUME : 0u) |
              ((ss->in_loaded < total || more_coming) ? UNIT_F_MORE_INPUT : 0u);
    if (ss->started && r->pending_reset) u.flags |= UNIT_F_RESET_MODEL;
    if (ss->started && r->pending_reopen) u.flags |= UNIT_F_REOPEN;
    return XLZ_OK;
}

int session_grow_model(xlz_reader *r, uint32_t need, hipStream_t stream)
{
    Session *ss = r->ss;
    if (need > kMaxLcLp) return XLZ_ERR_UNSUPPORTED;
    const size_t new_off_in = align_up(ss->off_state + state_bytes(need), 256);
    uint8_t *nc = nullptr;
    if (hipMalloc(&nc, new_off_in + ss->in_buf) != hipSuccess) return XLZ_ERR_DEVICE;
    if (hipMemcpyAsync(nc, ss->d_ctl, ss->off_state + kStateWords * 4, hipMemcpyDeviceToDevice, stream) != hipSuccess ||
        hipMemcpyAsync(nc + new_off_in, ss->d_ctl + ss->off_in, ss->in_buf, hipMemcpyDeviceToDevice, stream) != hipSuccess ||
        hipStreamSynchronize(stream) != hipSuccess) {
        (void)hipFree(nc);
        return XLZ_ERR_DEVICE;
    }
    (void)hipFree(ss->d_ctl);
    ss->d_ctl = nc;
    ss->off_in = new_off_in;
    ss->model_lc_lp = need;
    ss->unit.lc = (uint8_t)need;
    return XLZ_OK;
}

int session_make_shadow(xlz_reader *r)
{
    Session *ss = r->ss;
    if (!ss->d_shadow) {
        const size_t n = ss->unit.dict_size;
        uint8_t *img = nullptr;
        if (hipMalloc(&img, n) != hipSuccess) return XLZ_ERR_DEVICE;
        if (hipMemset(img, 0, n) != hipSuccess) {
            (void)hipFree(img);
            return XLZ_ERR_DEVICE;
        }
        ss->d_shadow = img;
        r->n_shadow++;
    }
    const uint64_t addr = (uint64_t)ss->d_shadow;
    if (hipMemcpy(ss->d_ctl + ss->off_state + (size_t)kStateShadowWord * 4, &addr, 8, hipMemcpyHostToDevice) != hipSuccess)
        return XLZ_ERR_DEVICE;
    return XLZ_OK;
}

int sessions_launch(xlz_ctx *ctx, const std::vector<xlz_reader *> &rs, bool big);

int sessions_step(xlz_ctx *ctx, const std::vector<xlz_reader *> &all)
{
    if (all.empty()) return XLZ_OK;
    std::lock_guard<std::mutex> lock(ctx->mu);
    for (xlz_reader *r : all) r->step_status = XLZ_ERR_DEVICE;
    HIP_TRY(hipSetDevice(ctx->device));
    std::vector<xlz_reader *> normal, bigs;
    for (xlz_reader *r : all) {
        int st = session_prepare(r, ctx->stream);
        if (st == XLZ_ERR_UNSUPPORTED) {
            r->finished = true;
            r->status = XLZ_ERR_UNSUPPORTED;
            r->chunk.clear();
            r->rd = 0;
            continue;
        }
        if (st != XLZ_OK) {
            for (xlz_reader *q : all) q->step_status = st;
            return st;
        }
        (r->ss->model_lc_lp > kMaxLcLpLds ? bigs : normal).push_back(r);
    }
    for (xlz_reader *r : all) r->step_status = XLZ_OK;
    const int st_normal = normal.empty() ? XLZ_OK : sessions_launch(ctx, normal, false);
    const int st_big = bigs.empty() ? XLZ_OK : sessions_launch(ctx, bigs, true);
    for (xlz_reader *r : normal) r->step_status = st_normal;
    for (xlz_reader *r : bigs) r->step_status = st_big;
    return st_normal != XLZ_OK ? st_normal : st_big;
}

int sessions_launch(xlz_ctx *ctx, const std::vector<xlz_reader *> &rs, bool big)
{
    const size_t n = rs.size();
    uint32_t max_lc_lp = 0;
    std::vector<Unit> units(n);
    for (size_t i = 0; i < n; i++) {
        units[i] = rs[i]->ss->unit;
        if (big) units[i].flags |= UNIT_F_BIG_MODEL;
        max_lc_lp = std::max(max_lc_lp, rs[i]->ss->model_lc_lp);
    }
    Unit *d_units = nullptr;
    uint32_t *d_order = nullptr;
    UnitResult *d_res = nullptr;
    uint8_t *scratch = nullptr;
    if (n == 1) {
        d_units = reinterpret_cast<Unit *>(rs[0]->ss->d_ctl);
        d_order = reinterpret_cast<uint32_t *>(rs[0]->ss->d_ctl + 128);
        d_res = reinterpret_cast<UnitResult *>(rs[0]->ss->d_ctl + 160);
    } else {
        const size_t o_order = align_up(n * sizeof(Unit), 256), o_res = o_order + align_up(n * 4, 256);
        HIP_TRY(hipMalloc(&scratch, o_res + n * sizeof(UnitResult)));
        d_units = reinterpret_cast<Unit *>(scratch);
        d_order = reinterpret_cast<uint32_t *>(scratch + o_order);
        d_res = reinterpret_cast<UnitResult *>(scratch + o_res);
        std::vector<uint32_t> order(n);
        std::iota(order.begin(), order.end(), 0u);
        if (hipMemcpyAsync(d_order, order.data(), n * 4, hipMemcpyHostToDevice, ctx->stream) != hipSuccess ||
            hipStreamSynchronize(ctx->stream) != hipSuccess) {
            (void)hipFree(scratch);
            return XLZ_ERR_DEVICE;
        }
    }
    uint16_t *d_mlit = nullptr;
    uint16_t *d_big = nullptr;
    uint32_t big_stride = 0;
    if (big) {
        big_stride = num_probs(max_lc_lp) + num_matched_probs(max_lc_lp);
        const size_t grid = std::min<size_t>(n, big_model_grid(ctx->num_cus));
        if (hipMalloc(&d_big, grid * big_stride * sizeof(uint16_t)) != hipSuccess) {
            if (scratch) (void)hipFree(scratch);
            return XLZ_ERR_DEVICE;
        }
    }
    int st = XLZ_ERR_DEVICE;
    std::vector<UnitResult> res(n);
    if (hipMemcpyAsync(d_units, units.data(), n * sizeof(Unit), hipMemcpyHostToDevice, ctx->stream) == hipSuccess &&
        hipMemsetAsync(ctx->queue, 0, 256, ctx->stream) == hipSuccess) {
        LaunchParams p;
        memset(&p, 0, sizeof p);
        p.in_arena = nullptr;
        p.out_arena = nullptr;
        p.units = d_units;
        p.order = d_order;
        p.results = d_res;
        p.queue = ctx->queue;
        p.n_units = (uint32_t)n;
        p.max_lc_lp = max_lc_lp;
        p.mlit = d_mlit;
        p.mlit_stride = 0;
        p.scratch = d_big;
        p.scratch_stride = big_stride;
        p.prio_tab = ctx->prio_tab;
        if (launch_decode(p, ctx->num_cus, ctx->stream) == 0 &&
            hipMemcpyAsync(res.data(), d_res, n * sizeof(UnitResult), hipMemcpyDeviceToHost, ctx->stream) == hipSuccess &&
            hipStreamSynchronize(ctx->stream) == hipSuccess)
            st = XLZ_OK;
    }
    if (st == XLZ_OK) {
        for (size_t i = 0; i < n; i++) {
            xlz_reader *r = rs[i];
            Session *ss = r->ss;
            const UnitResult &u = res[i];
            const uint32_t new_pos = (uint32_t)u.out_len;
            ss->started = true;
            ss->rebase = 0;
            r->pending_reset = r->pending_reopen = false;
            ss->consumed = ss->in_skip + (uint32_t)((uint32_t)u.in_consumed - (uint32_t)ss->in_skip);
            r->n_refills++;
            if (u.status == ST_PAUSED && (u.aux & AUX_GROW)) {
                const int g = session_grow_model(r, (u.aux & AUX_GROW_MASK) >> AUX_GROW_SHIFT, ctx->stream);
                if (g == XLZ_ERR_DEVICE) st = XLZ_ERR_DEVICE;
                if (g == XLZ_ERR_UNSUPPORTED) {
                    r->finished = true;
                    r->status = XLZ_ERR_UNSUPPORTED;
                    r->chunk.clear();
                    r->rd = 0;
                    continue;
                }
            }
            if (u.status == ST_PAUSED && (u.aux & AUX_SHADOW) && session_make_shadow(r) != XLZ_OK) st = XLZ_ERR_DEVICE;
            if (((u.aux & AUX_STALE) || u.status == ST_ERR_UNSUPPORTED) && r->streaming) {
                r->finished = true;
                r->status = XLZ_ERR_UNSUPPORTED;
                r->chunk.clear();
                r->rd = 0;
                continue;
            }
            if ((u.aux & AUX_STALE) || u.status == ST_ERR_UNSUPPORTED) {
                r->whole = true;
                continue;
            }
            const size_t fresh = new_pos > ss->pos ? new_pos - ss->pos : 0;
            r->chunk.resize(fresh);
            r->rd = 0;
            if (fresh && hipMemcpyAsync(r->chunk.data(), ss->d_win + ss->pos, fresh, hipMemcpyDeviceToHost, ctx->stream) !=
                             hipSuccess)
                st = XLZ_ERR_DEVICE;
            ss->pos = new_pos;
            r->delivered += fresh;
            if (ss->left != kUnknownSize) ss->left -= std::min<uint64_t>(ss->left, fresh);
            if (u.status != ST_PAUSED) {
                r->finished = true;
                r->status = u.status;
            } else if ((u.aux & AUX_NEED_INPUT) && r->streaming && !r->in_eof &&
                       ss->in_loaded >= r->in_base + r->src_len - ss->payload_off) {
                r->need_input = true;
            }
        }
        if (hipStreamSynchronize(ctx->stream) != hipSuccess) st = XLZ_ERR_DEVICE;
    }
    if (scratch) (void)hipFree(scratch);
    if (d_big) (void)hipFree(d_big);
    return st;
}

int reader_whole(xlz_reader *r)
{
    r->n_whole++;
    if (r->src_len > kMaxUnitBytes || r->delivered > kMaxUnitBytes) {
        r->finished = true;
        r->status = XLZ_ERR_UNSUPPORTED;
        return XLZ_OK;
    }
    uint64_t cap = 0;
    bool known = false;
    if (r->desc.format == XLZ_FMT_LZMA_ALONE) {
        uint64_t u = xlz_decode_unpack_size(r->src + 5);
        if (u != kUnknownSize) known = true, cap = u;
    } else if (r->desc.format == XLZ_FMT_LZMA_RAW && r->desc.unpack_size != kUnknownSize) {
        known = true;
        cap = r->desc.unpack_size;
    }
    if (!known) cap = std::max<uint64_t>(1u << 16, std::max<uint64_t>((uint64_t)r->src_len * 6, r->delivered * 2));
    std::vector<uint8_t> out;
    for (;;) {
        if (cap > kMaxUnitBytes) cap = kMaxUnitBytes;
        out.resize((size_t)cap);
        xlz_stream_desc d = r->desc;
        d.in = r->src;
        d.in_len = r->src_len;
        d.out = out.data();
        d.out_cap = out.size();
        xlz_result res;
        int st = xlz_decode_batch(r->ctx, &d, 1, &res);
        if (st != XLZ_OK) return st;
        if (res.status == XLZ_ERR_OUT_CAP && !known && cap < kMaxUnitBytes) {
            cap *= 4;
            continue;
        }
        const size_t skip = (size_t)std::min<uint64_t>(r->delivered, res.out_len);
        r->chunk.assign(out.begin() + skip, out.begin() + (size_t)res.out_len);
        r->rd = 0;
        r->delivered = res.out_len;
        r->finished = true;
        r->status = res.status;
        return XLZ_OK;
    }
}

void batcher_loop(Batcher *bt)
{
    std::unique_lock<std::mutex> lk(bt->mu);
    for (;;) {
        bt->cv_work.wait(lk, [&] { return bt->stop || !bt->pending.empty(); });
        if (bt->stop && bt->pending.empty()) return;
        bt->cv_work.wait_for(lk, std::chrono::microseconds(bt->window_us),
                             [&] { return bt->stop || bt->pending.size() >= bt->max_streams; });
        std::vector<xlz_reader *> work;
        while (!bt->pending.empty() && work.size() < bt->max_streams) {
            work.push_back(bt->pending.front());
            bt->pending.pop_front();
        }
        lk.unlock();
        (void)sessions_step(bt->ctx, work);
        lk.lock();
        bt->n_batches++;
        bt->n_streams += work.size();
        for (xlz_reader *r : work) {
            if (r->step_status != XLZ_OK) r->call_status = r->step_status;
            r->refill_pending = false;
        }
        bt->cv_done.notify_all();
    }
}

constexpr uint64_t kParBytes = 64u << 20;

bool reader_parallel_plan(xlz_reader *r)
{
    r->par_tried = true;
    std::vector<Lz2Unit> lu;
    uint32_t mx = 0;
    scan_lzma2(r->src, r->src_len, lu, mx);
    if (lu.size() < 8 || mx > kMaxLcLpLds) return false;
    r->par_in.assign(1, 0);
    r->par_out.assign(1, 0);
    for (const Lz2Unit &u : lu) {
        if (u.in_start != r->par_in.back() || u.out_start != r->par_out.back()) return false;
        r->par_in.push_back(u.in_start + (uint64_t)u.in_len);
        r->par_out.push_back(u.out_start + u.expect_out);
    }
    return r->par_in.back() == r->src_len;
}

int reader_parallel_step(xlz_reader *r)
{
    const size_t nunits = r->par_in.size() - 1;
    const size_t k0 = r->par_next;
    size_t k1 = k0 + 1;
    while (k1 < nunits && r->par_out[k1 + 1] - r->par_out[k0] <= kParBytes) k1++;
    const bool last = k1 == nunits;
    const uint64_t want_out = r->par_out[k1] - r->par_out[k0], in_len = r->par_in[k1] - r->par_in[k0];
    if (want_out > kMaxUnitBytes || in_len > kMaxUnitBytes) {
        r->par = false;
        return XLZ_OK;
    }
    std::vector<uint8_t> out((size_t)want_out + (last ? 65536 : 0) + 1);
    xlz_stream_desc d = r->desc;
    d.in = r->src + r->par_in[k0];
    d.in_len = (size_t)in_len;
    d.out = out.data();
    d.out_cap = out.size() - 1;
    xlz_result res;
    int st = xlz_decode_batch(r->ctx, &d, 1, &res);
    if (st != XLZ_OK) return st;
    r->n_par++;
    const bool clean = last ? (res.status >= 0 && res.out_len == want_out)
                            : (res.status == XLZ_ERR_UNEXPECTED_EOF && res.out_len == want_out && res.in_consumed == in_len);
    if (!clean && !(last && k0 == 0)) {
        r->par = false;
        r->whole = true;
        return XLZ_OK;
    }
    out.resize((size_t)res.out_len);
    r->chunk.swap(out);
    r->rd = 0;
    r->delivered += res.out_len;
    r->par_next = k1;
    if (last) {
        r->finished = true;
        r->status = res.status;
    }
    return XLZ_OK;
}

int reader_refill(xlz_reader *r)
{
    r->input_fresh = false;
    if (r->desc.format == XLZ_FMT_LZMA2_RAW && !r->streaming && !r->whole && !r->ss && !r->par_tried)
        r->par = reader_parallel_plan(r);
    if (r->par) {
        int st = reader_parallel_step(r);
        if (st != XLZ_OK || r->par) return st;
        if (r->whole && !r->finished) return reader_whole(r);
        if (r->delivered) {
            r->whole = true;
            return reader_whole(r);
        }
    }
    if (!r->ss && !r->whole) {
        int st = XLZ_OK;
        {
            std::lock_guard<std::mutex> lock(r->ctx->mu);
            HIP_TRY(hipSetDevice(r->ctx->device));
            st = session_open(r);
        }
        if (st == XLZ_ERR_UNSUPPORTED)
            r->whole = true;
        else if (st != XLZ_OK)
            return st;
    }
    if (r->whole && r->streaming && !r->in_eof && !r->finished) {
        r->need_input = true;
        return XLZ_OK;
    }
    if (!r->whole) {
        Batcher *bt = r->ctx->batcher;
        if (bt) {
            std::unique_lock<std::mutex> lk(bt->mu);
            r->refill_pending = true;
            bt->pending.push_back(r);
            bt->cv_work.notify_one();
            bt->cv_done.wait(lk, [&] { return !r->refill_pending; });
            if (r->call_status != XLZ_OK) return r->call_status;
        } else {
            std::vector<xlz_reader *> one{r};
            int st = sessions_step(r->ctx, one);
            if (st != XLZ_OK) return st;
        }
    }
    if (r->whole && !r->finished) return reader_whole(r);
    return XLZ_OK;
}

void reader_release_device(xlz_reader *r)
{
    if (!r->ss) return;
    std::lock_guard<std::mutex> lock(r->ctx->mu);
    (void)hipSetDevice(r->ctx->device);
    session_free(r->ss);
    r->ss = nullptr;
}

}

static int decode_oversize(xlz_ctx *ctx, const xlz_stream_desc *streams, xlz_result *results, const std::vector<size_t> &idx)
{
    std::vector<xlz_reader> rs(idx.size());
    std::vector<uint64_t> produced(idx.size(), 0);
    std::vector<xlz_reader *> active;
    int st = XLZ_OK;
    for (size_t k = 0; k < idx.size(); k++) {
        xlz_reader &r = rs[k];
        r.ctx = ctx;
        r.desc = streams[idx[k]];
        r.src = streams[idx[k]].in;
        r.src_len = streams[idx[k]].in_len;
        int so;
        {
            std::lock_guard<std::mutex> lock(ctx->mu);
            HIP_TRY(hipSetDevice(ctx->device));
            so = session_open(&r);
        }
        if (so == XLZ_OK)
            active.push_back(&r);
        else if (so == XLZ_ERR_DEVICE)
            st = so;
        else
            results[idx[k]].status = XLZ_ERR_UNSUPPORTED;
    }
    while (st == XLZ_OK && !active.empty()) {
        st = sessions_step(ctx, active);
        if (st != XLZ_OK) break;
        std::vector<xlz_reader *> next;
        for (xlz_reader *r : active) {
            const size_t k = (size_t)(r - rs.data());
            const xlz_stream_desc &d = streams[idx[k]];
            xlz_result &res = results[idx[k]];
            if (r->whole) {
                res.status = XLZ_ERR_UNSUPPORTED;
                res.out_len = produced[k];
                continue;
            }
            const size_t room = d.out_cap > produced[k] ? (size_t)(d.out_cap - produced[k]) : 0;
            const size_t take = std::min(room, r->chunk.size());
            if (take) memcpy(d.out + produced[k], r->chunk.data(), take);
            const bool overflow = take < r->chunk.size();
            produced[k] += take;
            r->chunk.clear();
            if (overflow || r->finished) {
                res.status = overflow ? XLZ_ERR_OUT_CAP : r->status;
                res.out_len = produced[k];
                res.in_consumed = r->ss->payload_off + r->ss->consumed;
                res.reserved = 0;
                continue;
            }
            next.push_back(r);
        }
        active.swap(next);
    }
    for (xlz_reader &r : rs) reader_release_device(&r);
    return st;
}

extern "C" xlz_reader *xlz_new_reader1(xlz_ctx *ctx, const uint8_t *in, size_t in_len, int *err)
{
    int e = XLZ_OK;
    xlz_reader *r = nullptr;
    if (!ctx || (!in && in_len)) {
        e = XLZ_ERR_BAD_ARG;
    } else if (in_len == 0) {
        e = XLZ_ERR_HEADER_EOF;
    } else if (xlz_decode_prop(in[0], nullptr, nullptr, nullptr) != XLZ_OK) {
        e = XLZ_ERR_PROPS;
    } else if (in_len < 13) {
        e = XLZ_ERR_HEADER_EOF;
    } else if ((e = check_rc_init(in + 13, in_len - 13)) == XLZ_OK) {
        r = reader_new(ctx, in, in_len);
        if (!r)
            e = XLZ_ERR_BAD_ARG;
        else
            r->desc.format = XLZ_FMT_LZMA_ALONE;
    }
    if (err) *err = e;
    return r;
}

extern "C" xlz_reader *xlz_new_reader2(xlz_ctx *ctx, const uint8_t *in, size_t in_len, int dict_size, int *err)
{
    int e = XLZ_OK;
    xlz_reader *r = nullptr;
    if (!ctx || (!in && in_len)) {
        e = XLZ_ERR_BAD_ARG;
    } else if (in_len == 0) {
        e = XLZ_ERR_UNEXPECTED_EOF;
    } else {
        const uint8_t c = in[0];
        const bool lzma_chunk = c >= 0x80;
        const size_t hl = c == 0 || (c >= 3 && c < 0x80) ? 1 : (c < 3 ? 3 : ((c >> 5) >= 6 ? 6 : 5));
        if (in_len < hl) {
            e = XLZ_ERR_UNEXPECTED_EOF;
        } else if (lzma_chunk) {
            const uint8_t props = hl == 6 ? in[5] : 0;
            if (xlz_decode_prop(props, nullptr, nullptr, nullptr) != XLZ_OK) {
                e = XLZ_ERR_PROPS;
            } else {
                size_t comp = (((size_t)in[3] << 8) | in[4]) + 1;
                size_t avail = std::min(comp, in_len - hl);
                e = check_rc_init(in + hl, avail);
            }
        }
        if (e == XLZ_OK) {
            r = reader_new(ctx, in, in_len);
            if (!r) {
                e = XLZ_ERR_BAD_ARG;
            } else {
                r->desc.format = XLZ_FMT_LZMA2_RAW;
                r->desc.dict_size = (uint32_t)dict_size;
            }
        }
    }
    if (err) *err = e;
    return r;
}

extern "C" xlz_reader *xlz_new_lzma_decompressor_for_sevenzip(xlz_ctx *ctx, const uint8_t *props, size_t props_len,
                                                              uint64_t unpack_size, const uint8_t *const *readers,
                                                              const size_t *reader_lens, size_t n_readers, int *err)
{
    int e = XLZ_OK;
    xlz_reader *r = nullptr;
    if (n_readers != 1) {
        e = XLZ_ERR_NEED_ONE_READER;
    } else if (!ctx || !props || props_len < 5 || !readers || !reader_lens || (!readers[0] && reader_lens[0])) {
        e = XLZ_ERR_BAD_ARG;
    } else if (xlz_decode_prop(props[0], nullptr, nullptr, nullptr) != XLZ_OK) {
        e = XLZ_ERR_PROPS;
    } else {
        e = check_rc_init(readers[0], reader_lens[0]);
        if (e == XLZ_OK) {
            r = reader_new(ctx, readers[0], reader_lens[0]);
            if (!r) {
                e = XLZ_ERR_BAD_ARG;
            } else {
                r->desc.format = XLZ_FMT_LZMA_RAW;
                r->desc.props = props[0];
                r->desc.dict_size = xlz_decode_dict_size(props + 1);
                r->desc.unpack_size = unpack_size;
                r->is_closer = true;
            }
        }
    }
    if (err) *err = e;
    return r;
}

extern "C" xlz_reader *xlz_new_lzma2_decompressor_for_sevenzip(xlz_ctx *ctx, const uint8_t *props, size_t props_len,
                                                               uint64_t unpack_size, const uint8_t *const *readers,
                                                               const size_t *reader_lens, size_t n_readers, int *err)
{
    (void)unpack_size;
    int e = XLZ_OK;
    xlz_reader *r = nullptr;
    if (n_readers != 1) {
        e = XLZ_ERR_NEED_ONE_READER;
    } else if (props_len != 1) {
        e = XLZ_ERR_INSUFFICIENT_PROPS;
    } else if (!ctx || !props || !readers || !reader_lens) {
        e = XLZ_ERR_BAD_ARG;
    } else {
        r = xlz_new_reader2(ctx, readers[0], reader_lens[0], (int)xlz_decode_dict_size2(props[0]), &e);
        if (r) r->is_closer = true;
    }
    if (err) *err = e;
    return r;
}

extern "C" long xlz_reader_read(xlz_reader *r, uint8_t *p, size_t n, int *err)
{
    int e = XLZ_OK;
    long got = 0;
    if (!r || (!p && n)) {
        e = XLZ_ERR_BAD_ARG;
    } else if (r->closed) {
        e = XLZ_ERR_CLOSED;
    } else {
        for (;;) {
            const size_t left = r->chunk.size() - r->rd;
            const size_t k = std::min(left, n - (size_t)got);
            if (k) memcpy(p + got, r->chunk.data() + r->rd, k);
            r->rd += k;
            got += (long)k;
            if ((size_t)got == n) break;
            if (r->finished) {
                e = r->status >= 0 ? XLZ_EOF : r->status;
                break;
            }
            if (r->need_input) {
                e = XLZ_NEED_INPUT;
                break;
            }
            if ((e = reader_refill(r)) != XLZ_OK) break;
        }
        if (n == 0 && r->finished && r->rd == r->chunk.size()) e = r->status >= 0 ? XLZ_EOF : r->status;
    }
    if (err) *err = e;
    return got;
}

extern "C" int xlz_reader_close(xlz_reader *r)
{
    if (!r) return XLZ_ERR_BAD_ARG;
    if (r->closed) return XLZ_ERR_CLOSED;
    r->closed = true;
    reader_release_device(r);
    r->in.clear();
    r->in.shrink_to_fit();
    r->chunk.clear();
    r->chunk.shrink_to_fit();
    return XLZ_OK;
}

extern "C" void xlz_reader_free(xlz_reader *r)
{
    if (!r) return;
    reader_release_device(r);
    delete r;
}

extern "C" int xlz_reader_reset(xlz_reader *r)
{
    if (!r) return XLZ_ERR_BAD_ARG;
    if (r->closed) return XLZ_ERR_CLOSED;
    if (r->desc.format == XLZ_FMT_LZMA2_RAW || r->whole) return XLZ_ERR_UNSUPPORTED;
    r->pending_reset = true;
    r->finished = false;
    return XLZ_OK;
}

extern "C" int xlz_reader_reopen(xlz_reader *r, const uint8_t *in, size_t in_len, uint64_t unpack_size)
{
    if (!r || (!in && in_len)) return XLZ_ERR_BAD_ARG;
    if (r->closed) return XLZ_ERR_CLOSED;
    if (r->desc.format == XLZ_FMT_LZMA2_RAW || r->whole) return XLZ_ERR_UNSUPPORTED;
    r->streaming = false;
    r->in_eof = false;
    r->input_fresh = true;
    r->in_base = 0;
    r->need_input = false;
    if (!r->ss) {
        std::lock_guard<std::mutex> lock(r->ctx->mu);
        HIP_TRY(hipSetDevice(r->ctx->device));
        int st = session_open(r);
        if (st != XLZ_OK) return st;
    }
    const int e = check_rc_init(in, in_len);
    r->in.assign(in, in + in_len);
    r->src = r->in.data();
    r->src_len = r->in.size();
    Session *ss = r->ss;
    ss->payload_off = 0;
    ss->in_skip = ss->in_loaded = ss->consumed = 0;
    ss->unit.unpack_size = unpack_size;
    ss->win_max = 2 * (size_t)ss->unit.dict_size + kChunk + kWinSlack;
    ss->left = kUnknownSize;
    if (ss->in_buf < kInBuf) {
        uint8_t *nc = nullptr;
        std::lock_guard<std::mutex> lock(r->ctx->mu);
        HIP_TRY(hipSetDevice(r->ctx->device));
        HIP_TRY(hipMalloc(&nc, ss->off_in + kInBuf));
        if (hipMemcpy(nc, ss->d_ctl, ss->off_in, hipMemcpyDeviceToDevice) != hipSuccess) {
            (void)hipFree(nc);
            return XLZ_ERR_DEVICE;
        }
        (void)hipFree(ss->d_ctl);
        ss->d_ctl = nc;
        ss->in_buf = kInBuf;
    }
    if (ss->started) {
        r->pending_reopen = true;
    } else {
        ss->unit.kind = UNIT_LZMA1;
    }
    r->finished = false;
    r->status = XLZ_OK;
    return e == XLZ_ERR_RC_INIT ? XLZ_ERR_RESULT : e;
}

extern "C" int xlz_reader_expect_more(xlz_reader *r)
{
    if (!r) return XLZ_ERR_BAD_ARG;
    if (r->closed) return XLZ_ERR_CLOSED;
    if (!r->input_fresh || r->whole) return XLZ_ERR_BAD_ARG;
    r->streaming = true;
    r->in_eof = false;
    return XLZ_OK;
}

extern "C" int xlz_reader_feed(xlz_reader *r, const uint8_t *data, size_t n)
{
    if (!r || (!data && n)) return XLZ_ERR_BAD_ARG;
    if (r->closed) return XLZ_ERR_CLOSED;
    if (!r->streaming || r->in_eof) return XLZ_ERR_BAD_ARG;
    if (r->ss) {
        const uint64_t keep_from = r->ss->payload_off + (r->ss->consumed & ~(uint64_t)255);
        if (keep_from > r->in_base) {
            const size_t drop = (size_t)std::min<uint64_t>(keep_from - r->in_base, r->in.size());
            r->in.erase(r->in.begin(), r->in.begin() + drop);
            r->in_base += drop;
        }
    }
    r->in.insert(r->in.end(), data, data + n);
    r->src = r->in.data();
    r->src_len = r->in.size();
    r->need_input = false;
    return XLZ_OK;
}

extern "C" int xlz_reader_feed_eof(xlz_reader *r)
{
    if (!r) return XLZ_ERR_BAD_ARG;
    if (r->closed) return XLZ_ERR_CLOSED;
    if (!r->streaming) return XLZ_ERR_BAD_ARG;
    r->in_eof = true;
    r->need_input = false;
    return XLZ_OK;
}

extern "C" int xlz_reader_memory(const xlz_reader *r, uint64_t *window_bytes, uint64_t *image_bytes)
{
    if (!r) return XLZ_ERR_BAD_ARG;
    if (window_bytes) *window_bytes = r->ss ? r->ss->win_cap : 0;
    if (image_bytes) *image_bytes = (r->ss && r->ss->d_shadow) ? r->ss->unit.dict_size : 0;
    return XLZ_OK;
}

extern "C" int xlz_reader_stats(const xlz_reader *r, uint64_t *refills, uint64_t *whole_decodes, uint64_t *in_uploaded)
{
    if (!r) return XLZ_ERR_BAD_ARG;
    if (refills) *refills = r->n_refills + r->n_par;
    if (whole_decodes) *whole_decodes = r->n_whole;
    if (in_uploaded) *in_uploaded = r->ss ? r->ss->in_loaded : 0;
    return XLZ_OK;
}

static void batcher_shutdown(Batcher *bt)
{
    {
        std::lock_guard<std::mutex> lk(bt->mu);
        bt->stop = true;
        bt->cv_work.notify_all();
    }
    bt->th.join();
    delete bt;
}

extern "C" int xlz_ctx_enable_batching(xlz_ctx *ctx, uint32_t window_us, uint32_t max_streams)
{
    if (!ctx || ctx->batcher) return XLZ_ERR_BAD_ARG;
    Batcher *bt = new (std::nothrow) Batcher;
    if (!bt) return XLZ_ERR_BAD_ARG;
    bt->ctx = ctx;
    bt->window_us = window_us;
    bt->max_streams = max_streams ? max_streams : 1;
    bt->th = std::thread(batcher_loop, bt);
    ctx->batcher = bt;
    return XLZ_OK;
}

extern "C" int xlz_ctx_batching_stats(xlz_ctx *ctx, uint64_t *batches, uint64_t *streams)
{
    if (!ctx || !ctx->batcher) return XLZ_ERR_BAD_ARG;
    std::lock_guard<std::mutex> lk(ctx->batcher->mu);
    if (batches) *batches = ctx->batcher->n_batches;
    if (streams) *streams = ctx->batcher->n_streams;
    return XLZ_OK;
}
```

Measured before the change: 17.69.

## Replace monolithic pinned staging with chunked pinned ring pinned by background helper

Swaps the single large pinned input staging buffer and the fixed 8-slot output ring for a shared chunked PinRing of 32 MiB chunks, split between upload and download. A background helper thread pins the chunks ahead of time so large hipHostMalloc calls leave the call path. Uploads now stream through per-chunk writers that recycle chunks via events instead of holding one lease for the whole input. It adds locking, event reclaim waits and a persistent thread, and it caps pinned memory, which may throttle uploads when chunks are all in flight.

```diff
diff --git a/lzma_amd/build.py b/lzma_amd/build.py
--- a/lzma_amd/build.py
+++ b/lzma_amd/build.py
@@ -6,7 +6,7 @@
 CSRC = os.path.join(HERE, "csrc")
 SO = os.path.join(HERE, "libxlz.so")
 SOURCES = ["xlz_kernel.hip", "xlz_host.hip", "xlz_xz.hip", "xlz_7z.hip", "xlz_check_dev.hip", "xlz_filter_dev.hip", "xlz_sha256_dev.hip"]
-HEADERS = ["xlz_format.h", "xlz_check.h", "xlz_check_dev.h", "xlz_check_host.h", "xlz_filter_dev.h", "xlz_sha256_dev.h", "xlz_fastpath.inc", "xlz_fastpath_pb2.inc", "xlz_fastpath_pb2_br.inc", os.path.join("..", "..", "include", "xlz.h")]
+HEADERS = ["xlz_format.h", "xlz_check.h", "xlz_check_dev.h", "xlz_check_host.h", "xlz_filter_dev.h", "xlz_sha256_dev.h", "xlz_pinring.h", "xlz_fastpath.inc", "xlz_fastpath_pb2.inc", "xlz_fastpath_pb2_br.inc", os.path.join("..", "..", "include", "xlz.h")]
 ARCH = "gfx950"
 
 
diff --git a/lzma_amd/csrc/xlz_host.hip b/lzma_amd/csrc/xlz_host.hip
--- a/lzma_amd/csrc/xlz_host.hip
+++ b/lzma_amd/csrc/xlz_host.hip
@@ -23,6 +23,7 @@
 #include "xlz_check_host.h"
 #include "xlz_sha256_dev.h"
 #include "xlz_filter_dev.h"
+#include "xlz_pinring.h"
 
 using namespace xlz;
 
@@ -72,6 +73,7 @@
     std::vector<Blk> idle;
     std::vector<Blk> live;
     uint64_t gen = 1;
+    std::atomic<uint64_t> *pin_alloc_max = nullptr;
     void *take(size_t n, bool pinned)
     {
         if (n == 0) n = 1;
@@ -91,6 +93,7 @@
             }
         }
         void *p = nullptr;
+        if (pinned && pin_alloc_max && pin_alloc_max->load() < n) pin_alloc_max->store(n);
         const hipError_t e = pinned ? hipHostMalloc(&p, n, hipHostMallocDefault) : hipMalloc(&p, n);
         if (e != hipSuccess) {
             (void)hipGetLastError();
@@ -144,23 +147,38 @@
         for (const Blk &b : idle) t += b.cap;
         return t;
     }
+    uint64_t pinned_bytes()
+    {
+        std::lock_guard<std::mutex> lk(mu);
+        uint64_t t = 0;
+        for (const Blk &b : idle) t += b.pinned ? b.cap : 0;
+        for (const Blk &b : live) t += b.pinned ? b.cap : 0;
+        return t;
+    }
 };
 
 constexpr int kEventSlots = 64;
 
 struct HostPipe {
-    static constexpr int kRing = 8;
-    static constexpr size_t kRingBytes = 32u << 20;
+    static constexpr size_t kChunkBytes = 32u << 20;
+    static constexpr int kChunks = 20;
+    static int out_share(int chunks) { return std::max(1, chunks * 2 / 5); }
+    size_t chunk_bytes = kChunkBytes;
+    int n_in = kChunks - out_share(kChunks), n_out = out_share(kChunks);
     std::mutex mu_in;
     std::condition_variable cv_in;
     bool in_busy = false;
     std::mutex mu_out;
-    uint8_t *pin_in = nullptr;
-    size_t pin_in_cap = 0;
-    uint8_t *ring[kRing] = {};
-    hipEvent_t ring_ev[kRing] = {};
+    std::mutex mu_setup;
+    bool ready = false, helper_started = false;
+    xlzpin::PinRing in_ring, out_ring;
+    std::vector<hipEvent_t> in_ev, out_ev;
+    std::thread helper;
+    std::atomic<uint64_t> call_alloc_max{0};
     hipStream_t copy_stream = nullptr;
     hipStream_t up_stream = nullptr;
+    size_t piece_round = 4096;
+    unsigned piece_shift = 29;
 };
 
 struct PinLease {
@@ -273,13 +291,12 @@
     SlicePiece *d_pieces = nullptr;
     uint8_t *d_pack = nullptr;
     UnitResult *d_res_snap = nullptr;
-    UnitResult *pin_res = nullptr;
+    std::vector<UnitResult> res_host;
     uint32_t head_frac = 0;
     uint8_t *d_stage = nullptr;
     SlicePiece *d_up_pieces = nullptr;
     hipEvent_t ev_heads = nullptr, ev_tails = nullptr;
     std::function<int()> upload_tails;
-    PinLease in_lease;
     uint8_t *d_chk = nullptr, *pin_chk = nullptr;
     size_t d_chk_cap = 0, pin_chk_cap = 0;
     hipEvent_t chk_ev0 = nullptr, chk_ev1 = nullptr;
@@ -382,6 +399,72 @@
     for (unsigned t = 1; t < n; t++) th.emplace_back([&f, t] { f(t); });
     f(0u);
     for (auto &x : th) x.join();
+}
+
+int pipe_setup(xlz_ctx *c)
+{
+    HostPipe &hp = c->pipe;
+    std::lock_guard<std::mutex> lk(hp.mu_setup);
+    if (hp.ready) return XLZ_OK;
+    HIP_TRY(hipSetDevice(c->device));
+    if (!hp.up_stream) HIP_TRY(hipStreamCreateWithFlags(&hp.up_stream, hipStreamNonBlocking));
+    if (!hp.copy_stream) HIP_TRY(hipStreamCreateWithFlags(&hp.copy_stream, hipStreamNonBlocking));
+    hp.in_ev.resize((size_t)hp.n_in, nullptr);
+    hp.out_ev.resize((size_t)hp.n_out, nullptr);
+    for (hipEvent_t &e : hp.in_ev)
+        if (!e) HIP_TRY(hipEventCreateWithFlags(&e, hipEventDisableTiming));
+    for (hipEvent_t &e : hp.out_ev)
+        if (!e) HIP_TRY(hipEventCreateWithFlags(&e, hipEventDisableTiming));
+    xlzpin::Callbacks cb;
+    cb.alloc = [](size_t n) -> void * {
+        void *p = nullptr;
+        if (hipHostMalloc(&p, n, hipHostMallocDefault) != hipSuccess) {
+            (void)hipGetLastError();
+            return nullptr;
+        }
+        return p;
+    };
+    cb.release = [](void *p) { (void)hipHostFree(p); };
+    cb.done = [&hp](int i) { return hipEventQuery(hp.in_ev[(size_t)i]) == hipSuccess; };
+    cb.wait = [&hp](int i) { return hipEventSynchronize(hp.in_ev[(size_t)i]) == hipSuccess; };
+    xlzpin::Callbacks cb_out = cb;
+    cb_out.done = [](int) { return true; };
+    cb_out.wait = [](int) { return true; };
+    if (!hp.in_ring.configure(hp.chunk_bytes, hp.n_in, cb) || !hp.out_ring.configure(hp.chunk_bytes, hp.n_out, cb_out)) return XLZ_ERR_DEVICE;
+    hp.ready = true;
+    return XLZ_OK;
+}
+
+int pipe_acquire(HostPipe &hp, xlzpin::PinRing &ring, uint8_t **p)
+{
+    void *q = nullptr;
+    size_t pinned_here = 0;
+    const int i = ring.acquire(&q, &pinned_here);
+    if (pinned_here > hp.call_alloc_max.load()) hp.call_alloc_max.store(pinned_here);
+    *p = static_cast<uint8_t *>(q);
+    return i;
+}
+
+void pipe_start_helper(xlz_ctx *c)
+{
+    HostPipe &hp = c->pipe;
+    if (pipe_setup(c) != XLZ_OK) return;
+    std::lock_guard<std::mutex> lk(hp.mu_setup);
+    if (hp.helper_started) return;
+    hp.helper_started = true;
+    try {
+        hp.helper = std::thread([c] {
+            HostPipe &hp = c->pipe;
+            if (hipSetDevice(c->device) != hipSuccess) return;
+            bool in = true, out = true;
+            for (int k = 0; k < 4 && in; k++) in = hp.in_ring.pin_next();
+            while (in || out) {
+                if (out) out = hp.out_ring.pin_next();
+                if (in) in = hp.in_ring.pin_next();
+            }
+        });
+    } catch (...) {
+    }
 }
 
 }
@@ -412,6 +495,7 @@
         delete c;
         return XLZ_ERR_DEVICE;
     }
+    c->pool.pin_alloc_max = &c->pipe.call_alloc_max;
     *out = c;
     return XLZ_OK;
 }
@@ -430,11 +514,15 @@
         if (c->chk_consts[k]) (void)hipFree(c->chk_consts[k]);
     }
     if (c->check_stream) (void)hipStreamDestroy(c->check_stream);
-    if (c->pipe.pin_in) (void)hipHostFree(c->pipe.pin_in);
-    for (int i = 0; i < HostPipe::kRing; i++) {
-        if (c->pipe.ring[i]) (void)hipHostFree(c->pipe.ring[i]);
-        if (c->pipe.ring_ev[i]) (void)hipEventDestroy(c->pipe.ring_ev[i]);
-    }
+    c->pipe.in_ring.shutdown();
+    c->pipe.out_ring.shutdown();
+    if (c->pipe.helper.joinable()) c->pipe.helper.join();
+    c->pipe.in_ring.free_all();
+    c->pipe.out_ring.free_all();
+    for (hipEvent_t e : c->pipe.in_ev)
+        if (e) (void)hipEventDestroy(e);
+    for (hipEvent_t e : c->pipe.out_ev)
+        if (e) (void)hipEventDestroy(e);
     if (c->pipe.copy_stream) (void)hipStreamDestroy(c->pipe.copy_stream);
     if (c->pipe.up_stream) (void)hipStreamDestroy(c->pipe.up_stream);
     for (hipEvent_t e : c->ev)
@@ -719,12 +807,10 @@
     batch_release(b, b->d_up_pieces);
     if (b->ev_heads) (void)hipEventDestroy(b->ev_heads);
     if (b->ev_tails) (void)hipEventDestroy(b->ev_tails);
-    b->in_lease.release();
     batch_release(b, b->d_states);
     batch_release(b, b->d_pieces);
     batch_release(b, b->d_pack);
     batch_release(b, b->d_res_snap);
-    batch_release(b, b->pin_res, true);
     batch_release(b, b->d_chk);
     batch_release(b, b->pin_chk, true);
     if (b->chk_ev0) (void)hipEventDestroy(b->chk_ev0);
@@ -739,38 +825,75 @@
     return XLZ_OK;
 }
 
-int take_pin_in(PinLease &lease, HostPipe &hp, size_t bytes)
-{
-    lease.take(hp);
-    if (hp.pin_in_cap < bytes) {
-        if (hp.pin_in) (void)hipHostFree(hp.pin_in);
-        hp.pin_in = nullptr;
-        hp.pin_in_cap = 0;
-        const size_t want = bytes + bytes / 4 + (1u << 20);
-        if (hipHostMalloc(&hp.pin_in, want, hipHostMallocDefault) != hipSuccess) return XLZ_ERR_DEVICE;
-        hp.pin_in_cap = want;
-    }
-    if (!hp.up_stream && hipStreamCreateWithFlags(&hp.up_stream, hipStreamNonBlocking) != hipSuccess) return XLZ_ERR_DEVICE;
-    return XLZ_OK;
-}
-
 struct PackPiece {
     uint64_t off;
     const uint8_t *src;
     size_t len;
 };
 
-template <class At> int pack_upload(xlz_ctx *ctx, uint8_t *stage, uint8_t *dst, size_t n, uint64_t total, bool zero_gaps, At &&at)
-{
-    const hipStream_t up = ctx->pipe.up_stream;
-    std::atomic<bool> copy_failed{false};
-    auto copy = [&](uint64_t from, uint64_t to) {
-        if (to > from && hipMemcpyAsync(dst + from, stage + from, (size_t)(to - from), hipMemcpyHostToDevice, up) != hipSuccess)
-            copy_failed = true;
-    };
+struct ChunkWriter {
+    HostPipe &hp;
+    uint8_t *dst;
+    int idx = -1;
+    uint8_t *p = nullptr;
+    uint64_t base = 0, sent = 0, cur = 0;
+    bool ok = true;
+    ChunkWriter(HostPipe &h, uint8_t *d) : hp(h), dst(d) {}
+    void flush()
+    {
+        if (cur > sent && hipMemcpyAsync(dst + sent, p + (sent - base), (size_t)(cur - sent), hipMemcpyHostToDevice, hp.up_stream) != hipSuccess)
+            ok = false;
+        sent = cur;
+    }
+    void finish()
+    {
+        if (idx < 0) return;
+        flush();
+        if (hipEventRecord(hp.in_ev[(size_t)idx], hp.up_stream) != hipSuccess) ok = false;
+        hp.in_ring.submit(idx);
+        idx = -1;
+    }
+    void put(uint64_t off, const uint8_t *src , size_t len)
+    {
+        const uint64_t C = hp.chunk_bytes;
+        while (len && ok) {
+            if (idx >= 0 && off >= base + C) finish();
+            if (idx < 0) {
+                idx = pipe_acquire(hp, hp.in_ring, &p);
+                if (idx < 0) {
+                    ok = false;
+                    return;
+                }
+                base = sent = cur = off;
+            }
+            const size_t take = (size_t)std::min<uint64_t>(len, base + C - off);
+            if (src)
+                memcpy(p + (off - base), src, take), src += take;
+            else
+                memset(p + (off - base), 0, take);
+            off += take;
+            len -= take;
+            cur = off;
+            if (cur == base + C)
+                finish();
+            else if (cur - sent >= (16u << 20))
+                flush();
+        }
+    }
+};
+
+template <class At> int pack_upload(xlz_ctx *ctx, uint8_t *dst, size_t n, uint64_t total, bool zero_gaps, At &&at)
+{
+    if (pipe_setup(ctx) != XLZ_OK) return XLZ_ERR_DEVICE;
+    HostPipe &hp = ctx->pipe;
+    PinLease lease;
+    lease.take(hp);
+    std::atomic<bool> failed{false};
     if (!n && zero_gaps) {
-        memset(stage, 0, (size_t)total);
-        copy(0, total);
+        ChunkWriter w(hp, dst);
+        w.put(0, nullptr, (size_t)total);
+        w.finish();
+        if (!w.ok) failed = true;
     }
     auto end_of = [&](size_t k) {
         if (!zero_gaps) return at(k).off + at(k).len;
@@ -781,24 +904,18 @@
         (void)hipSetDevice(ctx->device);
         const size_t k0 = n * t / nth, k1 = n * (t + 1) / nth;
         if (k0 >= k1) return;
-        uint64_t sent = at(k0).off;
-        if (zero_gaps && k0 == 0) {
-            memset(stage, 0, (size_t)sent);
-            sent = 0;
-        }
-        for (size_t k = k0; k < k1; k++) {
+        ChunkWriter w(hp, dst);
+        if (zero_gaps && k0 == 0) w.put(0, nullptr, (size_t)at(k0).off);
+        for (size_t k = k0; k < k1 && w.ok; k++) {
             const PackPiece pc = at(k);
-            memcpy(stage + pc.off, pc.src, pc.len);
+            w.put(pc.off, pc.src, pc.len);
             const uint64_t end = end_of(k);
-            if (end > pc.off + pc.len) memset(stage + pc.off + pc.len, 0, (size_t)(end - pc.off - pc.len));
-            if (end - sent >= (16u << 20)) {
-                copy(sent, end);
-                sent = end;
-            }
-        }
-        copy(sent, end_of(k1 - 1));
+            if (end > pc.off + pc.len) w.put(pc.off + pc.len, nullptr, (size_t)(end - pc.off - pc.len));
+        }
+        w.finish();
+        if (!w.ok) failed = true;
     });
-    return copy_failed ? XLZ_ERR_DEVICE : XLZ_OK;
+    return failed ? XLZ_ERR_DEVICE : XLZ_OK;
 }
 
 LaunchParams batch_params(const xlz_batch *b, bool big)
@@ -1044,9 +1161,9 @@
             if (hipEventCreateWithFlags(&b->slice_ev[k], hipEventDisableTiming) != hipSuccess) return fail(XLZ_ERR_DEVICE);
         if (!batch_alloc(b, &b->d_pieces, std::max<size_t>(total_pieces, 1) * sizeof(SlicePiece)) ||
             !batch_alloc(b, &b->d_pack, (size_t)max_pack + kArenaAlign) ||
-            !batch_alloc(b, &b->d_res_snap, (size_t)K * nu * sizeof(UnitResult)) ||
-            !batch_alloc(b, &b->pin_res, (size_t)K * nu * sizeof(UnitResult), true))
+            !batch_alloc(b, &b->d_res_snap, (size_t)K * nu * sizeof(UnitResult)))
             return fail(XLZ_ERR_DEVICE);
+        b->res_host.assign((size_t)K * nu, UnitResult{});
         size_t at = 0;
         for (uint32_t k = 0; k < K; k++) {
             const std::vector<SlicePiece> &pv = b->slice_pieces[k];
@@ -1084,11 +1201,11 @@
             (!tails->empty() && hipMemcpy(b->d_up_pieces + heads->size(), tails->data(), tails->size() * sizeof(SlicePiece),
                                           hipMemcpyHostToDevice) != hipSuccess))
             return fail(XLZ_ERR_DEVICE);
-        if (take_pin_in(b->in_lease, hp, (size_t)(A + B)) != XLZ_OK) return fail(XLZ_ERR_DEVICE);
+        if (pipe_setup(ctx) != XLZ_OK) return fail(XLZ_ERR_DEVICE);
         auto upload_part = [b, ctx, streams, unit_src_off_p](const std::vector<SlicePiece> &pv, size_t table_at, uint64_t zone,
                                                              uint64_t zone_bytes, hipEvent_t done) -> int {
             HostPipe &hp = ctx->pipe;
-            const int st = pack_upload(ctx, hp.pin_in + zone, b->d_stage + zone, pv.size(), zone_bytes, false, [&](size_t k) {
+            const int st = pack_upload(ctx, b->d_stage + zone, pv.size(), zone_bytes, false, [&](size_t k) {
                 const SlicePiece &pc = pv[k];
                 const Unit &u = b->units[pc.unit];
                 return PackPiece{pc.pack_off, streams[u.stream].in + (*unit_src_off_p)[pc.unit] + (pc.src_off - u.in_off), pc.len};
@@ -1105,14 +1222,11 @@
         const size_t n_heads = heads->size();
         b->upload_tails = [upload_part, tails, n_heads, A, B, b]() { return upload_part(*tails, n_heads, A, B, b->ev_tails); };
     } else {
-        HostPipe &hp = ctx->pipe;
-        PinLease lease;
-        if (take_pin_in(lease, hp, b->in_bytes) != XLZ_OK) return fail(XLZ_ERR_DEVICE);
-        const int st = pack_upload(ctx, hp.pin_in, b->d_in, nu, b->in_bytes, true, [&](size_t k) {
+        const int st = pack_upload(ctx, b->d_in, nu, b->in_bytes, true, [&](size_t k) {
             const Unit &u = b->units[k];
             return PackPiece{u.in_off, streams[u.stream].in + unit_src_off[k], u.in_len};
         });
-        if (hipStreamSynchronize(hp.up_stream) != hipSuccess || st != XLZ_OK) return fail(XLZ_ERR_DEVICE);
+        if (st != XLZ_OK || hipStreamSynchronize(ctx->pipe.up_stream) != hipSuccess) return fail(XLZ_ERR_DEVICE);
     }
     if (nu) {
         if (hipMemcpy(b->d_units, b->units.data(), nu * sizeof(Unit), hipMemcpyHostToDevice) != hipSuccess ||
@@ -1156,11 +1270,7 @@
                                        hipMemcpyDeviceToDevice, rs));
                 HIP_TRY(hipEventRecord(b->slice_ev[k], rs));
             }
-            if (b->head_frac) {
-                HIP_TRY(hipEventSynchronize(b->ev_tails));
-                b->in_lease.release();
-                b->head_frac = 0;
-            }
+            b->head_frac = 0;
         }
     }
     if (b->units.size() > b->n_normal) {
@@ -2126,23 +2236,21 @@
     const uint8_t *src;
     size_t len;
 };
-template <class Before, class Src, class Scatter>
-int ring_download(xlz_batch *b, size_t n, Before &&before, Src &&src, Scatter &&scatter)
+template <class Before, class Src, class Scatter, class Dep>
+int ring_download(xlz_batch *b, size_t n, Before &&before, Src &&src, Scatter &&scatter, Dep &&dep)
 {
     xlz_ctx *ctx = b->ctx;
     HostPipe &hp = ctx->pipe;
+    if (pipe_setup(ctx) != XLZ_OK) return XLZ_ERR_DEVICE;
     std::lock_guard<std::mutex> out_lock(hp.mu_out);
     HIP_TRY(hipSetDevice(ctx->device));
-    if (!hp.copy_stream) HIP_TRY(hipStreamCreateWithFlags(&hp.copy_stream, hipStreamNonBlocking));
-    for (int r = 0; r < HostPipe::kRing; r++) {
-        if (!hp.ring[r]) HIP_TRY(hipHostMalloc(&hp.ring[r], HostPipe::kRingBytes, hipHostMallocDefault));
-        if (!hp.ring_ev[r]) HIP_TRY(hipEventCreateWithFlags(&hp.ring_ev[r], hipEventDisableTiming));
-    }
-    const unsigned nworkers = std::min<unsigned>(host_threads(b->out_bytes), HostPipe::kRing);
+    const unsigned nworkers = std::min<unsigned>(host_threads(b->out_bytes), (unsigned)hp.n_out);
     std::mutex mu;
     std::condition_variable cv;
     size_t issued = 0, next_claim = 0, n_done = 0;
     std::vector<char> done(n, 0);
+    std::vector<int> slot_of(n, -1);
+    std::vector<uint8_t *> mem_of(n, nullptr);
     bool failed = false;
     auto worker = [&] {
         (void)hipSetDevice(ctx->device);
@@ -2154,11 +2262,24 @@
                 if (failed || next_claim >= n) return;
                 j = next_claim++;
             }
-            const int slot = (int)(j % HostPipe::kRing);
-            const bool ok = hipEventSynchronize(hp.ring_ev[slot]) == hipSuccess;
-            if (ok) scatter(j, hp.ring[slot]);
+            const int slot = slot_of[j];
+            bool ok = hipEventSynchronize(hp.out_ev[(size_t)slot]) == hipSuccess;
+            if (ok) {
+                const std::pair<size_t, size_t> d = dep(j);
+                std::unique_lock<std::mutex> lk(mu);
+                cv.wait(lk, [&] {
+                    if (failed) return true;
+                    for (size_t i = d.first; i < d.second; i++)
+                        if (!done[i]) return false;
+                    return true;
+                });
+                ok = !failed;
+            }
+            if (ok) scatter(j, mem_of[j]);
+            hp.out_ring.release(slot);
             {
                 std::lock_guard<std::mutex> lk(mu);
+                slot_of[j] = -1;
                 done[j] = 1;
                 n_done++;
                 if (!ok) failed = true;
@@ -2175,20 +2296,29 @@
             break;
         }
         if (j == n) break;
-        const int slot = (int)(j % HostPipe::kRing);
-        if (j >= (size_t)HostPipe::kRing) {
-            std::unique_lock<std::mutex> lk(mu);
-            cv.wait(lk, [&] { return done[j - HostPipe::kRing] || failed; });
-            if (failed) break;
-        }
-        const RingChunk c = src(j);
-        if (hipMemcpyAsync(hp.ring[slot], c.src, c.len, hipMemcpyDeviceToHost, hp.copy_stream) != hipSuccess ||
-            hipEventRecord(hp.ring_ev[slot], hp.copy_stream) != hipSuccess) {
+        uint8_t *mem = nullptr;
+        const int slot = pipe_acquire(hp, hp.out_ring, &mem);
+        if (slot < 0) {
             st = XLZ_ERR_DEVICE;
             break;
         }
+        const RingChunk c = src(j);
+        bool stop;
         {
             std::lock_guard<std::mutex> lk(mu);
+            stop = failed;
+        }
+        if (stop || hipMemcpyAsync(mem, c.src, c.len, hipMemcpyDeviceToHost, hp.copy_stream) != hipSuccess ||
+            hipEventRecord(hp.out_ev[(size_t)slot], hp.copy_stream) != hipSuccess) {
+            (void)hipStreamSynchronize(hp.copy_stream);
+            hp.out_ring.release(slot);
+            st = XLZ_ERR_DEVICE;
+            break;
+        }
+        {
+            std::lock_guard<std::mutex> lk(mu);
+            slot_of[j] = slot;
+            mem_of[j] = mem;
             issued = j + 1;
         }
         cv.notify_all();
@@ -2203,6 +2333,8 @@
     cv.notify_all();
     for (auto &x : th) x.join();
     if (hipStreamSynchronize(hp.copy_stream) != hipSuccess) st = XLZ_ERR_DEVICE;
+    for (size_t j = 0; j < n; j++)
+        if (slot_of[j] >= 0) hp.out_ring.release(slot_of[j]);
     return st;
 }
 
@@ -2219,6 +2351,8 @@
         std::vector<Piece> pieces;
     };
     std::vector<Chunk> chunks;
+    if (pipe_setup(b->ctx) != XLZ_OK) return XLZ_ERR_DEVICE;
+    const uint64_t ring_bytes = b->ctx->pipe.chunk_bytes;
     const size_t n_take = only ? only->size() : b->n;
     for (size_t t = 0; t < n_take; t++) {
         const size_t i = only ? (*only)[t] : t;
@@ -2229,12 +2363,12 @@
         uint64_t off = pl.out_off;
         uint8_t *dst = streams[i].out;
         while (len) {
-            if (chunks.empty() || off + 1 > chunks.back().dev_off + HostPipe::kRingBytes || off < chunks.back().dev_off) {
+            if (chunks.empty() || off + 1 > chunks.back().dev_off + ring_bytes || off < chunks.back().dev_off) {
                 chunks.emplace_back();
                 chunks.back().dev_off = off;
             }
             Chunk &c = chunks.back();
-            const size_t room = (size_t)(c.dev_off + HostPipe::kRingBytes - off);
+            const size_t room = (size_t)(c.dev_off + ring_bytes - off);
             const size_t take = len < room ? len : room;
             c.pieces.push_back({off, dst, take});
             c.len = (size_t)(off + take - c.dev_off);
@@ -2250,7 +2384,8 @@
         [&](size_t j) { return RingChunk{b->d_out + chunks[j].dev_off, chunks[j].len}; },
         [&](size_t j, const uint8_t *ring) {
             for (const Piece &pc : chunks[j].pieces) memcpy(pc.dst, ring + (pc.dev_off - chunks[j].dev_off), pc.len);
-        });
+        },
+        [](size_t) { return std::pair<size_t, size_t>(0, 0); });
 }
 
 struct SlotClock {
@@ -2289,13 +2424,22 @@
     const size_t K = b->slice_fracs.size(), nu = b->units.size();
     struct Chunk {
         uint32_t k;
+        bool results;
         uint64_t off;
         size_t len;
     };
     std::vector<Chunk> chunks;
-    for (size_t k = 0; k < K; k++)
-        for (uint64_t off = 0; off < b->slice_pack_bytes[k]; off += HostPipe::kRingBytes)
-            chunks.push_back({(uint32_t)k, off, (size_t)std::min<uint64_t>(HostPipe::kRingBytes, b->slice_pack_bytes[k] - off)});
+    if (pipe_setup(ctx) != XLZ_OK) return XLZ_ERR_DEVICE;
+    const uint64_t ring_bytes = ctx->pipe.chunk_bytes;
+    std::vector<std::pair<size_t, size_t>> res_chunks(K);
+    for (size_t k = 0; k < K; k++) {
+        res_chunks[k].first = chunks.size();
+        for (uint64_t off = 0; off < nu * sizeof(UnitResult); off += ring_bytes)
+            chunks.push_back({(uint32_t)k, true, off, (size_t)std::min<uint64_t>(ring_bytes, nu * sizeof(UnitResult) - off)});
+        res_chunks[k].second = chunks.size();
+        for (uint64_t off = 0; off < b->slice_pack_bytes[k]; off += ring_bytes)
+            chunks.push_back({(uint32_t)k, false, off, (size_t)std::min<uint64_t>(ring_bytes, b->slice_pack_bytes[k] - off)});
+    }
 
     size_t next_k = 0, piece_base = 0;
     const bool late = dev_late_results();
@@ -2305,8 +2449,7 @@
             if (hipStreamWaitEvent(cs, b->slice_ev[k], 0) != hipSuccess ||
                 launch_gather(b->d_pieces + piece_base, (uint32_t)b->slice_pieces[k].size(), b->d_out, b->d_pack,
                               b->slice_pack_bytes[k], ctx->num_cus, cs) != 0 ||
-                (late && k + 1 < K && hipStreamWaitEvent(cs, b->slice_ev[k + 1], 0) != hipSuccess) ||
-                hipMemcpyAsync(b->pin_res + k * nu, b->d_res_snap + k * nu, nu * sizeof(UnitResult), hipMemcpyDeviceToHost, cs) != hipSuccess)
+                (late && k + 1 < K && hipStreamWaitEvent(cs, b->slice_ev[k + 1], 0) != hipSuccess))
                 return false;
             piece_base += b->slice_pieces[k].size();
         }
@@ -2314,8 +2457,12 @@
     };
     auto scatter = [&](size_t j, const uint8_t *ring) {
         const Chunk &c = chunks[j];
+        if (c.results) {
+            memcpy(reinterpret_cast<uint8_t *>(b->res_host.data() + (size_t)c.k * nu) + c.off, ring, c.len);
+            return;
+        }
         const std::vector<SlicePiece> &pv = b->slice_pieces[c.k];
-        const UnitResult *res = b->pin_res + (size_t)c.k * nu;
+        const UnitResult *res = b->res_host.data() + (size_t)c.k * nu;
         size_t lo = 0, hi = pv.size();
         while (hi - lo > 1) {
             const size_t mid = (lo + hi) / 2;
@@ -2337,7 +2484,13 @@
         }
     };
     int st = ring_download(
-        b, chunks.size(), before, [&](size_t j) { return RingChunk{b->d_pack + chunks[j].off, chunks[j].len}; }, scatter);
+        b, chunks.size(), before,
+        [&](size_t j) {
+            const Chunk &c = chunks[j];
+            if (c.results) return RingChunk{reinterpret_cast<const uint8_t *>(b->d_res_snap + (size_t)c.k * nu) + c.off, c.len};
+            return RingChunk{b->d_pack + c.off, c.len};
+        },
+        scatter, [&](size_t j) { return chunks[j].results ? std::pair<size_t, size_t>(0, 0) : res_chunks[chunks[j].k]; });
     gaps.clear();
     for (size_t ui = 0; ui < nu && st == XLZ_OK && K > 1; ui++) {
         const Unit &u = b->units[ui];
@@ -2345,10 +2498,10 @@
             if (gaps.empty() || gaps.back() != u.stream) gaps.push_back(u.stream);
             continue;
         }
-        const uint64_t fin = b->pin_res[(K - 1) * nu + ui].out_len;
+        const uint64_t fin = b->res_host[(K - 1) * nu + ui].out_len;
         for (size_t k = 0; k + 1 < K; k++) {
             const uint64_t hi = std::min(slice_bound(u.out_cap, b->slice_fracs[k]), u.out_cap);
-            if (b->pin_res[k * nu + ui].out_len < std::min<uint64_t>(hi, fin)) {
+            if (b->res_host[k * nu + ui].out_len < std::min<uint64_t>(hi, fin)) {
                 if (gaps.empty() || gaps.back() != u.stream) gaps.push_back(u.stream);
                 break;
             }
@@ -2359,7 +2512,7 @@
         (void)xlz_batch_launch_info(b, &slots, nullptr);
         per_slice->assign(K, 0.0);
         for (size_t k = 0; k < K; k++) {
-            const UnitResult *res = b->pin_res + k * nu, *prev = k ? res - nu : nullptr;
+            const UnitResult *res = b->res_host.data() + k * nu, *prev = k ? res - nu : nullptr;
             SlotClock launch;
             for (size_t ui = 0; ui < nu; ui++)
                 if (!(b->units[ui].flags & UNIT_F_BIG_MODEL) &&
@@ -2394,6 +2547,38 @@
     return XLZ_OK;
 }
 
+#ifdef XLZ_DEV_KNOBS
+extern "C" int xlz_dev_set_pin_ring(xlz_ctx *ctx, uint64_t chunk_bytes, uint32_t chunks)
+{
+    if (!ctx || chunk_bytes < 4096 || chunk_bytes % 4096 || chunks < 2 || chunks > 1024) return XLZ_ERR_BAD_ARG;
+    HostPipe &hp = ctx->pipe;
+    std::lock_guard<std::mutex> lk(hp.mu_setup);
+    if (hp.ready) return XLZ_ERR_BAD_ARG;
+    hp.chunk_bytes = (size_t)chunk_bytes;
+    hp.n_out = HostPipe::out_share((int)chunks);
+    hp.n_in = (int)chunks - hp.n_out;
+    return XLZ_OK;
+}
+extern "C" int xlz_dev_set_pieces(xlz_ctx *ctx, uint32_t round_streams, uint32_t piece_shift)
+{
+    if (!ctx || piece_shift > 40) return XLZ_ERR_BAD_ARG;
+    std::lock_guard<std::mutex> lock(ctx->mu);
+    ctx->pipe.piece_round = round_streams ? round_streams : 4096;
+    ctx->pipe.piece_shift = piece_shift ? piece_shift : 29;
+    return XLZ_OK;
+}
+extern "C" int xlz_dev_pin_stats(xlz_ctx *ctx, uint64_t *largest, uint64_t *held, uint64_t *chunk_bytes, uint32_t *chunks)
+{
+    if (!ctx) return XLZ_ERR_BAD_ARG;
+    HostPipe &hp = ctx->pipe;
+    if (largest) *largest = hp.call_alloc_max.load();
+    if (held) *held = hp.in_ring.pinned_bytes() + hp.out_ring.pinned_bytes() + ctx->pool.pinned_bytes();
+    if (chunk_bytes) *chunk_bytes = hp.chunk_bytes;
+    if (chunks) *chunks = (uint32_t)(hp.n_in + hp.n_out);
+    return XLZ_OK;
+}
+#endif
+
 extern "C" int xlz_ctx_last_call_stats(xlz_ctx *ctx, xlz_call_stats *out)
 {
     if (!ctx || !out) return XLZ_ERR_BAD_ARG;
@@ -2403,20 +2588,20 @@
     return XLZ_OK;
 }
 
-static void plan_sub_batches(const xlz_stream_desc *streams, size_t n, std::vector<size_t> &cuts, bool *rounds)
+static void plan_sub_batches(const xlz_stream_desc *streams, size_t n, std::vector<size_t> &cuts, bool *rounds, size_t k_round = 4096,
+                             unsigned piece_shift = 29)
 {
     cuts.assign(1, 0);
     *rounds = false;
     uint64_t total = 0;
     for (size_t i = 0; i < n; i++) total += streams[i].out_cap;
-    const size_t k_round = 4096;
     if (n > 6144 && total / n >= (256u << 10)) {
         *rounds = true;
         for (size_t at = k_round; at < n; at += k_round) cuts.push_back(at);
         cuts.push_back(n);
         return;
     }
-    const size_t n_sub = std::min<size_t>(std::min<size_t>(8, n / k_round), (size_t)(total >> 29));
+    const size_t n_sub = std::min<size_t>(std::min<size_t>(8, n / k_round), (size_t)(total >> piece_shift));
     if (n_sub >= 2) {
         const double whole = (double)total / ((double)(n_sub - 1) + 0.5);
         std::vector<double> bounds;
@@ -2471,9 +2656,11 @@
     const char *dbg = getenv("XLZ_DEBUG");
     const auto t0 = std::chrono::steady_clock::now();
     auto now_ms = [&] { return std::chrono::duration<double, std::milli>(std::chrono::steady_clock::now() - t0).count(); };
+    pipe_start_helper(ctx);
+    ctx->pipe.call_alloc_max = 0;
     std::vector<size_t> cuts;
     bool rounds_mode = false;
-    plan_sub_batches(streams, n, cuts, &rounds_mode);
+    plan_sub_batches(streams, n, cuts, &rounds_mode, ctx->pipe.piece_round, ctx->pipe.piece_shift);
     const size_t S = cuts.size() - 1;
     xlz_call_stats cs;
     memset(&cs, 0, sizeof cs);
diff --git a/lzma_amd/csrc/xlz_pinring.h b/lzma_amd/csrc/xlz_pinring.h
--- /dev/null
+++ b/lzma_amd/csrc/xlz_pinring.h
@@ -0,0 +1,204 @@
+#pragma once
+
+#include <condition_variable>
+#include <cstddef>
+#include <cstdint>
+#include <functional>
+#include <mutex>
+#include <vector>
+
+namespace xlzpin {
+
+struct Callbacks {
+    std::function<void *(size_t)> alloc;
+    std::function<void(void *)> release;
+    std::function<bool(int)> done;
+    std::function<bool(int)> wait;
+};
+
+class PinRing {
+public:
+    PinRing() = default;
+    PinRing(const PinRing &) = delete;
+    PinRing &operator=(const PinRing &) = delete;
+
+    bool configure(size_t chunk_bytes, int n_chunks, Callbacks cb)
+    {
+        std::lock_guard<std::mutex> lk(mu_);
+        if (pinned_ || pinning_ || chunk_bytes == 0 || n_chunks <= 0) return false;
+        chunk_bytes_ = chunk_bytes;
+        cb_ = std::move(cb);
+        chunks_.assign((size_t)n_chunks, Chunk{});
+        return true;
+    }
+    size_t chunk_bytes() const { return chunk_bytes_; }
+    int chunks() const { return (int)chunks_.size(); }
+
+    bool pin_next()
+    {
+        int i;
+        {
+            std::lock_guard<std::mutex> lk(mu_);
+            if (down_ || failed_) return false;
+            i = first_in(UNPINNED);
+            if (i < 0) return false;
+            chunks_[(size_t)i].state = PINNING;
+            pinning_++;
+        }
+        return pin(i, FREE);
+    }
+
+    int acquire(void **p, size_t *call_path_alloc = nullptr)
+    {
+        if (call_path_alloc) *call_path_alloc = 0;
+        std::unique_lock<std::mutex> lk(mu_);
+        for (;;) {
+            if (down_ || failed_ || chunks_.empty()) return -1;
+            int i = oldest_in(FREE);
+            if (i >= 0) return hold(i, p);
+            const int fl = oldest_in(IN_FLIGHT);
+            if (fl >= 0) {
+                chunks_[(size_t)fl].state = RECLAIMING;
+                lk.unlock();
+                bool over = cb_.done(fl), ok = true;
+                lk.lock();
+                if (!over && !(first_in(UNPINNED) >= 0 && pinning_ == 0)) {
+                    lk.unlock();
+                    ok = cb_.wait(fl);
+                    lk.lock();
+                    over = true;
+                }
+                if (over) {
+                    chunks_[(size_t)fl].state = FREE;
+                    if (!ok) failed_ = true;
+                    if (!ok || down_) {
+                        cv_.notify_all();
+                        return -1;
+                    }
+                    return hold(fl, p);
+                }
+                chunks_[(size_t)fl].state = IN_FLIGHT;
+                cv_.notify_all();
+            }
+            i = first_in(UNPINNED);
+            if (i >= 0) {
+                chunks_[(size_t)i].state = PINNING;
+                pinning_++;
+                lk.unlock();
+                const bool ok = pin(i, HELD);
+                lk.lock();
+                if (!ok) return -1;
+                if (call_path_alloc) *call_path_alloc = chunk_bytes_;
+                if (p) *p = chunks_[(size_t)i].p;
+                return i;
+            }
+            cv_.wait(lk);
+        }
+    }
+
+    void submit(int i) { set(i, IN_FLIGHT); }
+    void release(int i) { set(i, FREE); }
+
+    void shutdown()
+    {
+        {
+            std::lock_guard<std::mutex> lk(mu_);
+            down_ = true;
+        }
+        cv_.notify_all();
+    }
+    void free_all()
+    {
+        std::lock_guard<std::mutex> lk(mu_);
+        for (Chunk &c : chunks_) {
+            if (c.p) cb_.release(c.p);
+            c = Chunk{};
+        }
+        pinned_ = 0;
+    }
+
+    size_t pinned_bytes()
+    {
+        std::lock_guard<std::mutex> lk(mu_);
+        return (size_t)pinned_ * chunk_bytes_;
+    }
+    int pinned_chunks()
+    {
+        std::lock_guard<std::mutex> lk(mu_);
+        return pinned_;
+    }
+    bool failed()
+    {
+        std::lock_guard<std::mutex> lk(mu_);
+        return failed_;
+    }
+
+private:
+    enum State : uint8_t { UNPINNED, PINNING, FREE, HELD, IN_FLIGHT, RECLAIMING };
+    struct Chunk {
+        void *p = nullptr;
+        State state = UNPINNED;
+        uint64_t since = 0;
+    };
+    std::mutex mu_;
+    std::condition_variable cv_;
+    std::vector<Chunk> chunks_;
+    Callbacks cb_;
+    size_t chunk_bytes_ = 0;
+    uint64_t tick_ = 0;
+    int pinned_ = 0, pinning_ = 0;
+    bool down_ = false, failed_ = false;
+
+    int first_in(State s) const
+    {
+        for (size_t i = 0; i < chunks_.size(); i++)
+            if (chunks_[i].state == s) return (int)i;
+        return -1;
+    }
+    int oldest_in(State s) const
+    {
+        int best = -1;
+        for (size_t i = 0; i < chunks_.size(); i++)
+            if (chunks_[i].state == s && (best < 0 || chunks_[i].since < chunks_[(size_t)best].since)) best = (int)i;
+        return best;
+    }
+    int hold(int i, void **p)
+    {
+        chunks_[(size_t)i].state = HELD;
+        chunks_[(size_t)i].since = ++tick_;
+        if (p) *p = chunks_[(size_t)i].p;
+        return i;
+    }
+    void set(int i, State s)
+    {
+        {
+            std::lock_guard<std::mutex> lk(mu_);
+            if (i < 0 || (size_t)i >= chunks_.size()) return;
+            chunks_[(size_t)i].state = s;
+            chunks_[(size_t)i].since = ++tick_;
+        }
+        cv_.notify_all();
+    }
+    bool pin(int i, State then)
+    {
+        void *q = cb_.alloc(chunk_bytes_);
+        {
+            std::lock_guard<std::mutex> lk(mu_);
+            pinning_--;
+            Chunk &c = chunks_[(size_t)i];
+            if (q) {
+                c.p = q;
+                c.state = then;
+                c.since = ++tick_;
+                pinned_++;
+            } else {
+                c.state = UNPINNED;
+                failed_ = true;
+            }
+        }
+        cv_.notify_all();
+        return q != nullptr;
+    }
+};
+
+}
```

After: 17.65. Within noise of the previous version (-0.3%).
